# rapidsai/cugraph-gnn

Hardware: AMD Instinct MI355X
Metric: sampled-edges/sec (sample+renumber+feature-gather+SAGEConv fwd), ogbn-products-like fan-out [25, 10] (higher is better)
Workload: dtype int64 ids (int32 timed as a variant) + f32 features (SAGE lin_l/lin_r product: bf16x3-split MFMA, f32 accumulate); 1 GPU; ogbn-products-like RMAT: V=2449029, E=118462496 directed (CSR row_ptr i64 / col i64 replicated per GPU), feat fp32 [V,100], batch 1024/GPU, fan-out [25, 10], 2-layer SAGEConv(mean) 100-256-47 fwd, step = 8 call groups of 188 mini-batches; parallelism=dp1 (seeds sharded, no data-path collective)

## Files before the change

### cugraph-gnn_amd/csrc/wg_common.hpp

```cpp
#pragma once
#include <hip/hip_runtime.h>

#include <cstdarg>
#include <cstdint>
#include <cstdio>
#include <stdexcept>
#include <vector>
#include <mutex>
#include <string>
#include <unordered_map>

#include "wgamd_ops.h"
#include "wgamd_tensor.h"
#include "wgamd_types.h"

struct wholememory_tensor_ {
  void* storage_ptr;
  wholememory_tensor_description_t desc;
  wholememory_tensor_* root;
  wholememory_handle_t handle;
  bool owns_handle = false;
  uint64_t handle_serial = 0;
};

extern "C" uint64_t wgamd_handle_serial(wholememory_handle_t h);
extern "C" wholememory_error_code_t wgamd_free_if_serial(wholememory_handle_t h, uint64_t serial);

namespace wgamd {

struct hip_error : std::runtime_error {
  using std::runtime_error::runtime_error;
};
struct logic_error : std::runtime_error {
  using std::runtime_error::runtime_error;
};
struct invalid_input : std::runtime_error {
  using std::runtime_error::runtime_error;
};
struct comm_error : std::runtime_error {
  using std::runtime_error::runtime_error;
};

inline std::string fmt(const char* f, ...)
{
  char buf[1024];
  va_list ap;
  va_start(ap, f);
  vsnprintf(buf, sizeof(buf), f, ap);
  va_end(ap);
  return buf;
}

#define WG_HIP_CHECK(expr)                                                                   \
  do {                                                                                       \
    hipError_t e__ = (expr);                                                                 \
    if (e__ != hipSuccess) {                                                                 \
      throw ::wgamd::hip_error(::wgamd::fmt("%s:%d HIP error %d (%s) in %s", __FILE__,       \
                                            __LINE__, (int)e__, hipGetErrorString(e__), #expr)); \
    }                                                                                        \
  } while (0)

#define WG_EXPECTS(cond, ...)                                                              \
  do {                                                                                     \
    if (!(cond)) throw ::wgamd::logic_error(::wgamd::fmt(__VA_ARGS__));                    \
  } while (0)

#define WG_REQUIRE_INPUT(cond, ...)                                                        \
  do {                                                                                     \
    if (!(cond)) throw ::wgamd::invalid_input(::wgamd::fmt(__VA_ARGS__));                  \
  } while (0)

template <typename F>
inline wholememory_error_code_t guarded(const char* op, F&& body)
{
  try {
    body();
  } catch (const invalid_input& e) {
    fprintf(stderr, "[wholegraph_amd] %s: invalid input: %s\n", op, e.what());
    return WHOLEMEMORY_INVALID_INPUT;
  } catch (const logic_error& e) {
    fprintf(stderr, "[wholegraph_amd] %s: logic error: %s\n", op, e.what());
    return WHOLEMEMORY_LOGIC_ERROR;
  } catch (const hip_error& e) {
    fprintf(stderr, "[wholegraph_amd] %s: device error: %s\n", op, e.what());
    return WHOLEMEMORY_CUDA_ERROR;
  } catch (const comm_error& e) {
    fprintf(stderr, "[wholegraph_amd] %s: communication error: %s\n", op, e.what());
    return WHOLEMEMORY_COMMUNICATION_ERROR;
  } catch (const std::bad_alloc&) {
    fprintf(stderr, "[wholegraph_amd] %s: out of memory\n", op);
    return WHOLEMEMORY_OUT_OF_MEMORY;
  } catch (...) {
    fprintf(stderr, "[wholegraph_amd] %s: unknown error\n", op);
    return WHOLEMEMORY_UNKNOW_ERROR;
// ... 52 lines not shown
  wholememory_env_func_t* env_;
  void* ctx_ = nullptr;
  void* ptr_ = nullptr;
};

class temp_arena {
 public:
  explicit temp_arena(wholememory_env_func_t* env) : buf_(env) {}
  size_t add(size_t bytes)
  {
    const size_t off = total_;
    total_ += (bytes + 255) / 256 * 256;
    return off;
  }
  void commit() { base_ = static_cast<char*>(buf_.bytes((int64_t)(total_ ? total_ : 1))); }
  template <typename T>
  T* at(size_t off) const
  {
    return reinterpret_cast<T*>(base_ + off);
  }

 private:
  temp_buffer buf_;
  size_t total_ = 0;
  char* base_   = nullptr;
};

inline void* output_alloc(wholememory_env_func_t* env, void* memory_context, int64_t elt_count,
                          wholememory_dtype_t dtype)
{
  wholememory_tensor_description_t d;
  wholememory_initialize_tensor_desc(&d);
  d.dim        = 1;
  d.sizes[0]   = elt_count;
  d.strides[0] = 1;
  d.dtype      = dtype;
  void* p = env->output_fns.malloc_fn(&d, WHOLEMEMORY_MA_DEVICE, memory_context,
                                      env->output_fns.global_context);
  if (elt_count > 0 && p == nullptr) throw std::bad_alloc();
  return p;
}

inline int ceil_div(int64_t a, int64_t b) { return (int)((a + b - 1) / b); }

inline int stream_cu_count(hipStream_t stream)
{
  static std::mutex m;
  static std::unordered_map<int, int> device_cus;
  int dev = 0, cus = 0;
  (void)hipGetDevice(&dev);
  {
    std::lock_guard<std::mutex> g(m);
    auto it = device_cus.find(dev);
    if (it != device_cus.end()) cus = it->second;
  }
  if (cus == 0) {
    cus = 256;
    (void)hipDeviceGetAttribute(&cus, hipDeviceAttributeMultiprocessorCount, dev);
    std::lock_guard<std::mutex> g(m);
    device_cus[dev] = cus;
  }
  if (stream == nullptr) return cus;
  uint32_t mask[32] = {0};
  if (hipExtStreamGetCUMask(stream, 32, mask) != hipSuccess) {
    (void)hipGetLastError();
    return cus;
  }
  int bits = 0;
  for (uint32_t w : mask) bits += __builtin_popcount(w);
  return (bits > 0 && bits < cus) ? bits : cus;
}

struct dev_count {
  int host;
  const int* dev;
  __device__ __forceinline__ int get() const { return dev ? *dev : host; }
};

struct rng_plan {
  uint64_t seed;
  const unsigned long long* seeds_dev;
  const int* target_batch;
  const int* target_seg;
  __device__ __forceinline__ void resolve(int i, uint64_t& s, int& i_local) const
  {
    s       = seed;
    i_local = i;
    if (target_batch) {
      const int b = target_batch[i];
      i_local     = i - target_seg[b];
      s           = seeds_dev[b];
    } else if (seeds_dev) {
      s = seeds_dev[0];
    }
  }
};

int64_t scan_tmp_ints(int64_t n);
constexpr int kScanTile = 2048;
void exclusive_scan_i32(const int* in, int* out, int64_t n, int* tmp, hipStream_t stream,
                        const int* n_live_dev = nullptr);
void exclusive_scan_i32_presummed(const int* in, int* out, int64_t n, const int* sums, hipStream_t stream,
                                  const int* n_live_dev = nullptr);
struct scan_chain {
  unsigned long long* tiles;
  unsigned int* counters;
  unsigned int epoch;
};
constexpr int64_t kScanChainTiles = (int64_t)1 << 20;
scan_chain scan_chain_acquire(hipStream_t stream);


struct sample_locality {
  int* hist;
  void* recs;
  int shift;
};
int64_t sample_locality_hist_ints();
int sample_locality_shift(int64_t id_bound);
void uniform_sample_enqueue(const int64_t* row_ptr, const void* col, bool col64, const void* seeds, bool seeds64,
                            dev_count n, int M, rng_plan random_seed, const int* offsets, void* dst, int* src_lid,
                            int64_t* edge_gid, hipStream_t stream,
                            const int64_t* row_start = nullptr, const int* row_deg = nullptr,
                            const sample_locality* loc = nullptr);
void sample_count_enqueue(const int64_t* row_ptr, const void* seeds, bool seeds64, dev_count n, int M, int* cnt,
                          int* big_deg, hipStream_t stream, int64_t* row_start = nullptr, int* row_deg = nullptr);
constexpr int kWeightedBlocks  = 1024;
constexpr int kWeightedLdsKeys = 12288;
constexpr int kWeightedLists    = 9;
constexpr int kWeightedListHead = 16;
constexpr int kWeightedRedoList  = 9;
constexpr int kWeightedRedoCount = 11;
constexpr int kWeightedRedoHead  = 12;
inline int64_t weighted_list_ints(int64_t cap)
{
  return kWeightedListHead + (int64_t)(kWeightedLists + 1) * (cap > 0 ? cap : 1);
}
void weighted_count_enqueue(const int64_t* row_ptr, const void* seeds, bool seeds64, dev_count n, int M, int* cnt,
                            int* big_list, hipStream_t stream);
void weighted_sample_enqueue(const int64_t* row_ptr, const void* col, bool col64, const void* weights, bool weights64,
                             const void* seeds, bool seeds64, dev_count n, int M, rng_plan random_seed, const int* offsets,
                             int* big_list, uint32_t* slab, int64_t slab_len, void* dst, int* src_lid,
                             int64_t* edge_gid, hipStream_t stream);
int64_t append_unique_slots(int64_t capacity);
struct batch_view {
  const int* target_batch;
  const int* target_seg;
  const int* edge_row;
  const int* edge_offsets;
  int G;
  int64_t id_bound;
  int* unique_batch;
  int* unique_seg;
  const int* sample_batch;
  const int* sample_seg;
  const int* sample_local0;
  void* frontier_out;
  int* frontier_batch_out;
  int* frontier_seg_out;
  int* frontier_local0_out;
  int* neighbor_local_out;
  int* center_local_out;
  int no_pad;
  __host__ __device__ const int* sbatch() const { return sample_batch ? sample_batch : target_batch; }
  __host__ __device__ const int* sseg() const { return sample_seg ? sample_seg : target_seg; }
};
void append_unique_prepare_enqueue(const void* targets, dev_count T, bool tgt64, const void* neighbors, dev_count E, bool nbr64,
                                   batch_view bv, void* keys, int* minpos, int64_t slots, int* slot_of, int* rank,
                                   int* scan_tmp, hipStream_t stream);
void append_unique_emit_enqueue(const void* targets, dev_count T, bool tgt64, const void* neighbors, dev_count E, bool nbr64,
                                batch_view bv, const int* minpos, const int* slot_of, const int* rank, int64_t slots,
                                void* unique_out, int* map_out, int* counts_out ,
                                hipStream_t stream);


void local_rows_gather(const char* table, wholememory_matrix_description_t tm, const void* idx,
                       wholememory_dtype_t idx_dtype, int64_t n, char* out, wholememory_matrix_description_t om,
                       hipStream_t stream);
void local_rows_scatter(const char* in, wholememory_matrix_description_t im, const void* idx,
                        wholememory_dtype_t idx_dtype, int64_t n, char* table, wholememory_matrix_description_t tm,
                        hipStream_t stream);
void local_rows_permute(const char* src, wholememory_matrix_description_t sm, const int64_t* src_idx, const int64_t* dst_idx,
                        int64_t n, char* dst, wholememory_matrix_description_t dm, hipStream_t stream);
struct id_exchange {
  wholememory_comm_t comm = nullptr;
  int W = 1, me = 0;
  int64_t local_start = 0, local_rows = 0;
  std::vector<size_t> send_cnt, recv_cnt;
  std::vector<int64_t> bucket_start;
  std::vector<size_t> send_n, recv_n, send_at, recv_at;
  int64_t n = 0, n_remote = 0, self_cnt = 0, recv_total = 0;
  bool self_direct = false;
  int64_t *d_grouped = nullptr, *d_pos = nullptr, *d_recv_ids = nullptr, *d_self_ids = nullptr, *d_self_pos = nullptr;
  temp_arena scratch;
  std::vector<size_t> so, sb, ro, rb;

  explicit id_exchange(wholememory_env_func_t* env) : scratch(env) {}
  void plan(wholememory_handle_t h, size_t entry_bytes, int64_t row0, const void* idx, wholememory_dtype_t idx_dtype,
            int64_t n_, bool self_direct_, hipStream_t stream);
  void exchange_ids(int64_t* recv_ids, hipStream_t stream);
  void rows_to_owners(const char* send, char* recv, size_t row_bytes, hipStream_t stream);
  void rows_to_askers(const char* send, char* recv, size_t row_bytes, hipStream_t stream);

 private:
  void scaled(size_t unit_send, size_t unit_recv, const std::vector<size_t>& s_n, const std::vector<size_t>& s_at,
              const std::vector<size_t>& r_n, const std::vector<size_t>& r_at);
};

void distributed_rows_op(bool scatter, wholememory_handle_t handle, wholememory_matrix_description_t tm, const void* idx,
// ... 5 lines not shown
```

### cugraph-gnn_amd/csrc/wg_fused.hip

```cpp
#include <atomic>

#include "wg_common.hpp"
#include "wgamd_ext.h"

namespace wgamd {
namespace {

inline size_t align_up(size_t v) { return (v + 255) & ~(size_t)255; }

struct hop_workspace {
  size_t cnt, scan_tmp, nbr, keys, minpos, slot_of, rank, big_list, slab, row_start, row_deg, loc_hist, total;
  int64_t slots, slab_len;
};

hop_workspace plan(int64_t target_cap, int64_t edge_cap, size_t id_bytes, bool batched, int64_t max_row_len = 0)
{
  hop_workspace w{};
  size_t off = 0;
  auto take  = [&](size_t bytes) {
    size_t at = off;
    off += align_up(bytes);
    return at;
  };
  w.slots        = append_unique_slots(target_cap + edge_cap);
// ... 16 lines not shown
  w.total        = off;
  return w;
}

inline std::atomic<int64_t>& sample_locality_min()
{
  static std::atomic<int64_t> v{[] {
    const char* e = getenv("WGAMD_SAMPLE_LOCALITY");
    return e && atoll(e) > 0 ? (int64_t)atoll(e) : INT64_MAX;
  }()};
  return v;
}

struct hop_args {
  const void* csr_weight  = nullptr;
  bool weight64           = false;
  int64_t max_row_len     = 0;
  const void* sample_targets = nullptr;
  const int* n_sample_dev    = nullptr;
  int64_t sample_cap         = 0;
  const int64_t* csr_row_ptr;
  const void* csr_col;
  wholememory_dtype_t id_dtype;
  bool col32 = false;
  const void* targets;
  const int* n_targets_dev;
  int64_t target_cap;
  int M;
  rng_plan rng;
  batch_view bv;
  int* offsets;
  int* neighbor_row;
  int* center_row;
  int64_t* edge_gid;
  int64_t edge_cap;
  void* unique;
  int* counts_dev;
  void* workspace;
  size_t workspace_bytes;
  hipStream_t stream;
};

void run_hop(hop_args a)
{
  WG_REQUIRE_INPUT(a.id_dtype == WHOLEMEMORY_DT_INT || a.id_dtype == WHOLEMEMORY_DT_INT64, "id dtype must be INT|INT64");
  WG_REQUIRE_INPUT(a.csr_row_ptr && a.csr_col && a.targets && a.n_targets_dev && a.offsets && a.neighbor_row &&
                     a.unique && a.workspace,
                   "null pointer");
  WG_REQUIRE_INPUT(a.M > 0, "the no-sync walk needs a positive fan-out (capacity = targets * M)");
  const void* s_targets = a.sample_targets ? a.sample_targets : a.targets;
  const int* s_n_dev    = a.sample_targets ? a.n_sample_dev : a.n_targets_dev;
  const int64_t s_cap   = a.sample_targets ? a.sample_cap : a.target_cap;
  WG_REQUIRE_INPUT(a.target_cap > 0 && s_cap > 0 && a.edge_cap >= s_cap * (int64_t)a.M, "edge_cap < sampled_cap * M");
  WG_REQUIRE_INPUT(a.target_cap + a.edge_cap < ((int64_t)1 << 30), "capacities too large for one call");
  const bool i64     = a.id_dtype == WHOLEMEMORY_DT_INT64;
  const bool col64   = i64 && !a.col32;
  const bool batched = a.bv.target_batch != nullptr;
  WG_REQUIRE_INPUT(a.csr_weight == nullptr || a.max_row_len > 0, "a biased hop needs max_row_len (the graph's maximum degree)");
  hop_workspace w    = plan(std::max(a.target_cap, s_cap), a.edge_cap, i64 ? 8 : 4, batched, a.csr_weight ? a.max_row_len : 0);
  WG_REQUIRE_INPUT(a.workspace_bytes >= w.total, "workspace too small: need %zu bytes", w.total);
  WG_REQUIRE_INPUT((reinterpret_cast<uintptr_t>(a.workspace) & 255) == 0, "workspace must be 256-byte aligned");
  char* base    = static_cast<char*>(a.workspace);
  int* cnt      = reinterpret_cast<int*>(base + w.cnt);
  int* scan_tmp = reinterpret_cast<int*>(base + w.scan_tmp);
  void* nbr     = base + w.nbr;
  void* keys    = base + w.keys;
  int* minpos   = reinterpret_cast<int*>(base + w.minpos);
  int* slot_of  = reinterpret_cast<int*>(base + w.slot_of);
  int* rank     = reinterpret_cast<int*>(base + w.rank);
  hipStream_t st = a.stream;

  dev_count T{(int)a.target_cap, a.n_targets_dev};
  dev_count S{(int)s_cap, s_n_dev};
  if (a.csr_weight != nullptr) {
    int* big_list = reinterpret_cast<int*>(base + w.big_list);
    weighted_count_enqueue(a.csr_row_ptr, s_targets, i64, S, a.M, cnt, big_list, st);
    exclusive_scan_i32(cnt, a.offsets, s_cap, scan_tmp, st, s_n_dev);
    weighted_sample_enqueue(a.csr_row_ptr, a.csr_col, col64, a.csr_weight, a.weight64, s_targets, i64, S, a.M, a.rng, a.offsets,
                            big_list, reinterpret_cast<uint32_t*>(base + w.slab), w.slab_len, nbr, a.center_row, a.edge_gid,
                            st);
  } else {
    int64_t* row_start = reinterpret_cast<int64_t*>(base + w.row_start);
    int* row_deg       = reinterpret_cast<int*>(base + w.row_deg);
    sample_count_enqueue(a.csr_row_ptr, s_targets, i64, S, a.M, cnt, nullptr, st, row_start, row_deg);
    exclusive_scan_i32(cnt, a.offsets, s_cap, scan_tmp, st, s_n_dev);
    const int64_t loc_min = sample_locality_min().load(std::memory_order_relaxed);
    sample_locality loc{reinterpret_cast<int*>(base + w.loc_hist), keys, sample_locality_shift(a.bv.id_bound)};
    const bool use_loc = a.M <= 32 && s_cap >= loc_min && a.bv.id_bound > 0 && batched && 8 * w.slots >= 32 * s_cap;
    uniform_sample_enqueue(a.csr_row_ptr, a.csr_col, col64, s_targets, i64, S, a.M, a.rng, a.offsets, nbr, a.center_row,
                           a.edge_gid, st, row_start, row_deg, use_loc ? &loc : nullptr);
  }
  dev_count E{(int)a.edge_cap, a.offsets + s_cap};
  batch_view bv   = a.bv;
  bv.edge_row     = a.center_row;
  bv.edge_offsets = a.offsets;
  append_unique_prepare_enqueue(a.targets, T, i64, nbr, E, col64, bv, keys, minpos, w.slots, slot_of, rank, scan_tmp, st);
  append_unique_emit_enqueue(a.targets, T, i64, nbr, E, col64, bv, minpos, slot_of, rank, w.slots, a.unique, a.neighbor_row,
                             a.counts_dev, st);
}

__global__ void __launch_bounds__(256)
target_rows_kernel(const int* __restrict__ unique_seg, const int* __restrict__ target_seg, const int* __restrict__ target_batch,
                   int n, int64_t* __restrict__ rows)
{
  const int i = blockIdx.x * blockDim.x + threadIdx.x;
  if (i >= n) return;
  const int b = target_batch[i];
  rows[i]     = (int64_t)i + unique_seg[b] - target_seg[b];
}

__global__ void __launch_bounds__(256)
hetero_hop_rows_kernel(const int* __restrict__ offsets, const int* __restrict__ f_batch, const int* __restrict__ f_seg,
                       const int* __restrict__ f_local0, const int* __restrict__ row_local, int n_f,
                       const int* __restrict__ seg_dst, const int64_t* __restrict__ cseg_dst, const int* __restrict__ seg_src,
                       const int64_t* __restrict__ cseg_src, int64_t* __restrict__ dst_full, int64_t* __restrict__ dst_compact,
                       int* __restrict__ col_full, int* __restrict__ col_compact)
{
  const int64_t tid = (int64_t)blockIdx.x * blockDim.x + threadIdx.x;
  const int64_t j   = tid >> 4;
  const int sub     = (int)(tid & 15);
  if (j >= n_f) return;
  const int b     = f_batch[j];
  const int local = f_local0[b] + ((int)j - f_seg[b]);
  if (sub == 0) {
    dst_full[j] = (int64_t)seg_dst[b] + local;
    if (dst_compact) dst_compact[j] = cseg_dst[b] + local;
  }
  const int s = offsets[j], e = offsets[j + 1];
  const int add_full = seg_src[b];
  const int add_c    = col_compact ? (int)cseg_src[b] : 0;
  for (int i = s + sub; i < e; i += 16) {
    const int r = row_local[i];
    col_full[i] = r + add_full;
    if (col_compact) col_compact[i] = r + add_c;
  }
}

__global__ void __launch_bounds__(256)
hetero_hop_rows_batched_kernel(const int* __restrict__ offsets, const int* __restrict__ f_seg, const int* __restrict__ f_local0,
                               const int* __restrict__ row_local, int chunks, const int* __restrict__ seg_dst,
                               const int64_t* __restrict__ cseg_dst, const int* __restrict__ seg_src,
                               const int64_t* __restrict__ cseg_src, int64_t* __restrict__ dst_full,
                               int64_t* __restrict__ dst_compact, int* __restrict__ col_full, int* __restrict__ col_compact)
{
  const int b = blockIdx.x / chunks, c = blockIdx.x % chunks, t = threadIdx.x;
  const int f0 = f_seg[b], f1 = f_seg[b + 1];
  const int j0 = f0 + (int)((int64_t)(f1 - f0) * c / chunks), j1 = f0 + (int)((int64_t)(f1 - f0) * (c + 1) / chunks);
  if (j0 >= j1) return;
  const int e0 = offsets[j0], e1 = offsets[j1];
  const int64_t d_full = (int64_t)seg_dst[b] + f_local0[b] - f0;
  const int64_t d_c    = dst_compact ? cseg_dst[b] + f_local0[b] - f0 : 0;
  const int add_full   = seg_src[b];
  const int add_c      = col_compact ? (int)cseg_src[b] : 0;
  for (int j = j0 + t; j < j1; j += 256) {
    dst_full[j] = d_full + j;
    if (dst_compact) dst_compact[j] = d_c + j;
  }
  for (int i = e0 + t; i < e1; i += 256) {
    const int r = row_local[i];
    col_full[i] = r + add_full;
    if (col_compact) col_compact[i] = r + add_c;
  }
}

constexpr int kLayerSegMax = 16;
__global__ void __launch_bounds__(256)
layer_cols_kernel(const int* __restrict__ offsets, const int* __restrict__ f_seg, const int* __restrict__ f_local0,
                  const int* __restrict__ row_local, int G, int chunks, int n_seg, const int* __restrict__ seg_tab,
                  const int64_t* __restrict__ seg_base, int64_t* __restrict__ self_rows, int* __restrict__ col)
{
  __shared__ int s_l0[kLayerSegMax];
  __shared__ int64_t s_add[kLayerSegMax];
  const int b = blockIdx.x / chunks, c = blockIdx.x % chunks;
// ... 425 lines not shown
```

### cugraph-gnn_amd/csrc/wg_rng.hpp

```cpp
#pragma once
#include <hip/hip_runtime.h>

#include <cstdint>

namespace wgamd {

struct PcgJump {
  uint64_t a;
  uint64_t s;
};

struct PcgJumpTables {
  PcgJump t[4][256];
  constexpr PcgJumpTables() : t{}
  {
    uint64_t base_a = 6364136223846793005ULL, base_s = 1;
    for (int k = 0; k < 4; k++) {
      t[k][0].a = 1;
      t[k][0].s = 0;
      for (int c = 1; c < 256; c++) {
        t[k][c].a = t[k][c - 1].a * base_a;
        t[k][c].s = t[k][c - 1].s * base_a + base_s;
      }
      for (int d = 0; d < 8; d++) {
        uint64_t na = base_a * base_a, ns = base_s * base_a + base_s;
        base_a = na;
        base_s = ns;
      }
    }
  }
};

__device__ __constant__ const PcgJumpTables g_pcg_jump{};

struct Pcg32 {
  uint64_t state;
  uint64_t inc;

  static constexpr uint64_t kMult = 6364136223846793005ULL;

  __host__ __device__ __forceinline__ uint32_t next_u32()
  {
    uint64_t old = state;
    state        = old * kMult + inc;
    uint32_t x   = (uint32_t)(((old >> 18u) ^ old) >> 27u);
    uint32_t rot = (uint32_t)(old >> 59u);
    return (x >> rot) | (x << ((0u - rot) & 31u));
  }

  __host__ __device__ __forceinline__ void skipahead(uint64_t delta)
  {
    uint64_t acc_mult = 1u, acc_plus = 0u, cur_mult = kMult, cur_plus = inc;
    while (delta) {
      if (delta & 1u) {
        acc_mult *= cur_mult;
        acc_plus = acc_plus * cur_mult + cur_plus;
      }
      cur_plus = (cur_mult + 1u) * cur_plus;
      cur_mult *= cur_mult;
      delta >>= 1u;
    }
    state = acc_mult * state + acc_plus;
  }

  __host__ __device__ __forceinline__ Pcg32(uint64_t seed, uint64_t subsequence)
  {
    state = 0u;
    inc   = (subsequence << 1u) | 1u;
    (void)next_u32();
    state += seed;
    (void)next_u32();
    skipahead(subsequence);
  }

  __device__ __forceinline__ void jump_table(uint32_t n)
  {
    PcgJump j = g_pcg_jump.t[0][n & 255u];
#pragma unroll
    for (int k = 1; k < 4; k++) {
      const uint32_t c = (n >> (8 * k)) & 255u;
      if (c) {
        const PcgJump m = g_pcg_jump.t[k][c];
        j.s             = j.s * m.a + m.s;
        j.a             = j.a * m.a;
      }
    }
    state = j.a * state + inc * j.s;
  }

  struct table_tag {};
  __device__ __forceinline__ Pcg32(uint64_t seed, uint32_t subsequence, table_tag, uint32_t extra_draws = 0)
  {
    inc   = ((uint64_t)subsequence << 1u) | 1u;
    state = (inc + seed) * kMult + inc;
    jump_table(subsequence + extra_draws);
  }

  __host__ __device__ __forceinline__ int32_t next_i31() { return (int32_t)(next_u32() & 0x7fffffffu); }
  __host__ __device__ __forceinline__ uint64_t next_u64()
  {
    uint64_t lo = next_u32();
    uint64_t hi = next_u32();
    return lo | (hi << 32u);
  }
  __host__ __device__ __forceinline__ int64_t next_i63() { return (int64_t)(next_u64() & 0x7fffffffffffffffULL); }
  __host__ __device__ __forceinline__ float next_f32() { return (float)(next_u32() >> 8u) / 16777216.0f; }
};

}
```

### cugraph-gnn_amd/csrc/wg_sample.hip

```cpp
#include <algorithm>
#include <cmath>

#include "wg_common.hpp"
#include "wg_rng.hpp"

namespace wgamd {
namespace {

template <typename T>
struct dtype_of;
template <>
struct dtype_of<int32_t> {
  static constexpr wholememory_dtype_t value = WHOLEMEMORY_DT_INT;
};
template <>
struct dtype_of<int64_t> {
  static constexpr wholememory_dtype_t value = WHOLEMEMORY_DT_INT64;
};

__host__ __device__ constexpr int ref_block_threads(int M)
{
  int f = (M - 1) / 32;
  return f < 3 ? 32 : f < 6 ? 64 : f < 12 ? 128 : 256;
}
__host__ __device__ constexpr int ref_items_per_thread(int M)
{
  constexpr int t[32] = {1, 2, 3, 2, 3, 3, 2, 2, 3, 3, 3, 3, 2, 2, 2, 2,
                         3, 3, 3, 3, 3, 3, 3, 3, 4, 4, 4, 4, 4, 4, 4, 4};
  return t[(M - 1) / 32];
}

__device__ __forceinline__ uint64_t stream_id(int64_t seed_index, int B, int lane)
{
  return (uint64_t)(int64_t)(int32_t)(seed_index * B + lane);
}

__device__ __forceinline__ Pcg32 stream_generator(uint64_t random_seed, int64_t seed_index, int B, int lane)
{
  const int64_t sid = seed_index * B + lane;
  if (sid < (1ll << 31)) return Pcg32(random_seed, (uint32_t)sid, Pcg32::table_tag{});
  return Pcg32(random_seed, stream_id(seed_index, B, lane));
}

constexpr int kWaveRowCapDecl = 1024;
constexpr int kHugeRow = 16384;

template <typename SeedT>
__global__ void __launch_bounds__(256) sample_count_kernel(const int64_t* __restrict__ row_ptr,
                                                           const SeedT* __restrict__ seeds,
                                                           dev_count n_,
                                                           int M,
                                                           int* __restrict__ cnt,
                                                           int* __restrict__ big_deg ,
                                                           int* __restrict__ lists = nullptr ,
                                                           int list_cap            = 0,
                                                           int scratch_threshold   = 0,
                                                           int64_t* __restrict__ row_start = nullptr,
                                                           int* __restrict__ row_deg       = nullptr)
{
  const int n_live = n_.get();
  if (lists == nullptr) {
    const int end = min(n_.host, (n_live / kScanTile + 1) * kScanTile);
    for (int i = blockIdx.x * blockDim.x + threadIdx.x; i < end; i += gridDim.x * blockDim.x) {
      int deg = 0;
      if (i < n_live) {
        const int64_t nid   = (int64_t)seeds[i];
        const int64_t first = row_ptr[nid];
        deg                 = (int)(row_ptr[nid + 1] - first);
        if (row_start) {
          row_start[i] = first;
          row_deg[i]   = deg;
        }
        deg = (M > 0 && deg > M) ? M : deg;
      }
      cnt[i] = deg;
      if (big_deg) big_deg[i] = 0;
    }
    return;
  }
  int i = blockIdx.x * blockDim.x + threadIdx.x;
  int cls          = -1;
  int deg          = 0;
  if (i < n_.host) {
    if (i >= n_live) {
      if (i < (n_live / kScanTile + 1) * kScanTile) {
        cnt[i] = 0;
        if (big_deg) big_deg[i] = 0;
      }
    } else {
      int64_t nid         = (int64_t)seeds[i];
      const int64_t first = row_ptr[nid];
      deg                 = (int)(row_ptr[nid + 1] - first);
      cnt[i]              = (M > 0 && deg > M) ? M : deg;
      if (row_start) {
        row_start[i] = first;
        row_deg[i]   = deg;
      }
      if (big_deg) big_deg[i] = 0;
      if (lists != nullptr && M > 0 && deg > M) {
        cls = deg <= 16 ? 0 : deg <= 32 ? 1 : deg <= 64 ? 2 : deg <= 128 ? 3 : deg <= 256 ? 4 : deg <= 512 ? 5
              : deg <= kWaveRowCapDecl ? 6 : deg <= kHugeRow ? 7 : 8;
        if (cls >= 7 && deg > scratch_threshold) atomicMax(lists + 10, deg);
      }
    }
  }
  if (lists == nullptr) return;
  __shared__ int blk_cnt[kWeightedLists], blk_base[kWeightedLists];
  if (threadIdx.x < kWeightedLists) blk_cnt[threadIdx.x] = 0;
  __syncthreads();
  const int lane = threadIdx.x & 63;
  int my_rank    = 0;
#pragma unroll
  for (int c = 0; c < kWeightedLists; c++) {
    const uint64_t m = __ballot(cls == c);
    if (m == 0ull) continue;
    const int leader = __ffsll((long long)m) - 1;
    int base         = 0;
    if (lane == leader) base = atomicAdd(&blk_cnt[c], __popcll(m));
    base = __shfl(base, leader, 64);
    if (cls == c) my_rank = base + __popcll(m & ((1ull << lane) - 1ull));
  }
  __syncthreads();
  if (threadIdx.x < kWeightedLists && blk_cnt[threadIdx.x] > 0) blk_base[threadIdx.x] = atomicAdd(lists + threadIdx.x, blk_cnt[threadIdx.x]);
  __syncthreads();
  if (cls >= 0) lists[kWeightedListHead + (int64_t)cls * list_cap + blk_base[cls] + my_rank] = i;
}

template <typename ColT>
__device__ __forceinline__ ColT col_at(const ColT* __restrict__ col, int64_t at)
{
  return col ? col[at] : (ColT)0;
}

constexpr int kWalkGrid = 256 * 16;

template <typename ColT>
__device__ __forceinline__ void emit(ColT* dst, int* src_lid, int64_t* edge_gid, int64_t out, ColT v,
                                     int seed_index, int64_t gid)
{
  if (dst) dst[out] = v;
  if (src_lid) src_lid[out] = seed_index;
  if (edge_gid) edge_gid[out] = gid;
}

struct loc_rec {
  int64_t start;
  int i;
  int deg;
  int base;
  int i_local;
  int batch;
  int pad;
};
static_assert(sizeof(loc_rec) == 32, "one 32-byte sector per record");
// ... 32 lines not shown
  for (int b = 0; b < kLocBlocks; b++) {
    const int4 v = h4[(int64_t)b * (kLocBuckets / 4) + threadIdx.x];
    tot[0] += v.x; tot[1] += v.y; tot[2] += v.z; tot[3] += v.w;
    if (b < (int)blockIdx.x) { before[0] += v.x; before[1] += v.y; before[2] += v.z; before[3] += v.w; }
  }
  const int sum = tot[0] + tot[1] + tot[2] + tot[3];
  int inc = sum;
  const int lane = threadIdx.x & 63, wave = threadIdx.x >> 6;
#pragma unroll
  for (int d = 1; d < 64; d <<= 1) {
    const int up = __shfl_up(inc, d, 64);
    if (lane >= d) inc += up;
  }
  if (lane == 63) wave_tot[wave] = inc;
  __syncthreads();
  int run = inc - sum;
  for (int w = 0; w < wave; w++) run += wave_tot[w];
#pragma unroll
  for (int k = 0; k < 4; k++) {
    cursor[4 * threadIdx.x + k] = run + before[k];
    run += tot[k];
  }
  __syncthreads();
  for (int i = lo + threadIdx.x; i < hi; i += kLocThreads) {
    const int j = atomicAdd(&cursor[min((int)((uint64_t)seeds[i] >> shift), kLocBuckets - 1)], 1);
    loc_rec r;
    r.start = row_start[i];
    r.i     = i;
    r.deg   = row_deg[i];
    r.base  = offsets[i];
    r.i_local = i;
    r.batch   = 0;
    if (rng.target_batch) {
      r.batch   = rng.target_batch[i];
      r.i_local = i - rng.target_seg[r.batch];
    }
    r.pad   = 0;
    recs[j] = r;
  }
}

template <typename SeedT, typename ColT, int LANES>
__global__ void __launch_bounds__(256) sample_uniform_halfwave_kernel(const int64_t* __restrict__ row_ptr,
                                                                      const ColT* __restrict__ col,
                                                                      const SeedT* __restrict__ seeds,
                                                                      dev_count n_,
                                                                      int M,
                                                                      rng_plan rng,
                                                                      const int* __restrict__ offsets,
                                                                      ColT* __restrict__ dst,
                                                                      int* __restrict__ src_lid,
                                                                      int64_t* __restrict__ edge_gid,
                                                                      const int64_t* __restrict__ row_start,
                                                                      const int* __restrict__ row_deg,
                                                                      const loc_rec* __restrict__ recs = nullptr)
{
  const int n    = n_.get();
  const int lane = threadIdx.x & 63;
  const int hl   = lane & (LANES - 1);
  const int hb   = lane & ~(LANES - 1);
  int i          = (int)(((int64_t)blockIdx.x * blockDim.x + threadIdx.x) / LANES);
  loc_rec rec{};
  if (recs) {
    constexpr int kGroups = 256 / LANES;
    const int per_x = ((n + 7) / 8 + kGroups - 1) / kGroups * kGroups;
    const int k     = (int)(blockIdx.x >> 3) * kGroups + (int)threadIdx.x / LANES;
    const int j     = (int)(blockIdx.x & 7) * per_x + k;
    i               = n;
    if (k < per_x && j < n) {
      rec = recs[j];
      i   = rec.i;
    }
  }
  int32_t r_draw = 0;
  if (i < n && hl < M) {
    uint64_t random_seed;
    int i_local;
    if (recs) {
      i_local     = rec.i_local;
      random_seed = rng.seeds_dev ? rng.seeds_dev[rec.batch] : rng.seed;
    } else
      rng.resolve(i, random_seed, i_local);
    if (i_local < (1 << 26)) {
      Pcg32 g(random_seed, (uint32_t)(i_local * 32 + hl), Pcg32::table_tag{});
      r_draw = g.next_i31();
    } else {
      Pcg32 g(random_seed, stream_id(i_local, 32, hl));
      r_draw = g.next_i31();
    }
  }
  int64_t start = 0;
  int N = 0, base = 0;
  if (i < n && recs) {
    start = rec.start;
    N     = rec.deg;
    base  = rec.base;
  } else if (i < n) {
    if (row_start) {
      start = row_start[i];
      N     = row_deg[i];
    } else {
      int64_t nid = (int64_t)seeds[i];
      start       = row_ptr[nid];
      N           = (int)(row_ptr[nid + 1] - start);
    }
    base = offsets[i];
  }
  const bool pick = N > M;
  if (__ballot(pick) == 0ull) {
    if (hl < N) emit<ColT>(dst, src_lid, edge_gid, (int64_t)base + hl, col_at<ColT>(col, start + hl), i, start + hl);
    return;
  }
  int r = 0;
  if (pick && hl < M) r = r_draw % (N - hl);
  const int tail = N - hl - 1;
  int p1 = -1, p2 = -1;
  for (int s = 0; s + 1 < M; s++) {
    const int rs    = __shfl(r, hb | s, 64);
    const bool prev = s < hl;
    p1 = (prev && rs == r) ? s : p1;
    p2 = (prev && rs == tail) ? s : p2;
  }
  int root = p2 >= 0 ? p2 : hl;
#pragma unroll
  for (int round = 0; round < (LANES == 32 ? 5 : 4); round++) root = __shfl(root, hb | root, 64);
  const int val = N - root - 1;
  const int vp1 = __shfl(val, hb | (p1 & (LANES - 1)), 64);
  const int a   = p1 >= 0 ? vp1 : r;
  if (pick) {
    if (hl < M) emit<ColT>(dst, src_lid, edge_gid, (int64_t)base + hl, col_at<ColT>(col, start + a), i, start + a);
  } else if (hl < N) {
    emit<ColT>(dst, src_lid, edge_gid, (int64_t)base + hl, col_at<ColT>(col, start + hl), i, start + hl);
  }
}

template <typename SeedT, typename ColT, int GW, int K, bool EXACT>
__global__ void __launch_bounds__(256)
sample_uniform_multi_kernel(const ColT* __restrict__ col, dev_count n_, int M_rt, rng_plan rng, const int* __restrict__ offsets,
                            ColT* __restrict__ dst, int* __restrict__ src_lid, int64_t* __restrict__ edge_gid,
                            const int64_t* __restrict__ row_start, const int* __restrict__ row_deg,
                            const loc_rec* __restrict__ recs)
{
  constexpr int kGPW    = 64 / GW;
  constexpr int kGroups = 4 * kGPW;
  constexpr int kRounds = GW <= 2 ? 1 : GW <= 4 ? 2 : GW <= 8 ? 3 : GW <= 16 ? 4 : 5;
  const int M    = EXACT ? GW : M_rt;
  const int n    = n_.get();
  const int lane = threadIdx.x & 63;
  const int grp  = lane / GW;
  const int hl   = lane - grp * GW;
  const int hb   = grp * GW;
  const bool live_group = grp < kGPW;
  const int wg_group    = (int)(threadIdx.x >> 6) * kGPW + grp;
  const int per_x = ((n + 7) / 8 + kGroups * K - 1) / (kGroups * K) * (kGroups * K);
  const int64_t n_chunks = recs ? (int64_t)(per_x / (kGroups * K)) * 8 : ((int64_t)n + kGroups * K - 1) / (kGroups * K);
  for (int64_t chunk = blockIdx.x; chunk < n_chunks; chunk += gridDim.x) {
  int i[K], N[K], base[K], i_local[K], batch[K];
  int64_t start[K];
  if (recs) {
    const int k0    = ((int)(chunk >> 3) * kGroups + wg_group) * K;
#pragma unroll
    for (int k = 0; k < K; k++) {
      const int j = (int)(chunk & 7) * per_x + k0 + k;
      i[k] = n, N[k] = 0, base[k] = 0, start[k] = 0, i_local[k] = 0, batch[k] = 0;
      if (live_group && k0 + k < per_x && j < n) {
        const loc_rec r = recs[j];
        i[k] = r.i, N[k] = r.deg, base[k] = r.base, start[k] = r.start, i_local[k] = r.i_local, batch[k] = r.batch;
      }
    }
  } else {
    const int64_t g = chunk * kGroups + wg_group;
#pragma unroll
    for (int k = 0; k < K; k++) {
      i[k] = live_group ? (int)min(g * K + k, (int64_t)n) : n;
      N[k] = 0, base[k] = 0, start[k] = 0, i_local[k] = i[k], batch[k] = 0;
      if (i[k] < n) {
        start[k] = row_start[i[k]];
        N[k]     = row_deg[i[k]];
        base[k]  = offsets[i[k]];
        if (rng.target_batch) batch[k] = rng.target_batch[i[k]];
      }
    }
    if (rng.target_batch) {
#pragma unroll
      for (int k = 0; k < K; k++)
        if (i[k] < n) i_local[k] = i[k] - rng.target_seg[batch[k]];
    }
  }
  int32_t r_draw[K];
#pragma unroll
  for (int k = 0; k < K; k++) {
    r_draw[k] = 0;
    if (i[k] < n && hl < M) {
      const uint64_t random_seed = rng.seeds_dev ? rng.seeds_dev[rng.target_batch ? batch[k] : 0] : rng.seed;
      if (i_local[k] < (1 << 26)) {
        Pcg32 g(random_seed, (uint32_t)(i_local[k] * 32 + hl), Pcg32::table_tag{});
        r_draw[k] = g.next_i31();
      } else {
        Pcg32 g(random_seed, stream_id(i_local[k], 32, hl));
        r_draw[k] = g.next_i31();
      }
    }
  }
  int a[K];
#pragma unroll
  for (int k = 0; k < K; k++) {
    const bool pick = N[k] > M;
    a[k]            = hl;
    if (__ballot(pick) != 0ull) {
      int r = 0;
      if (pick && hl < M) r = r_draw[k] % (N[k] - hl);
      const int tail = N[k] - hl - 1;
      int p1 = -1, p2 = -1;
      auto step = [&](int s) {
        const int rs    = __shfl(r, hb + s, 64);
        const bool prev = s < hl;
        p1 = (prev && rs == r) ? s : p1;
        p2 = (prev && rs == tail) ? s : p2;
      };
      if constexpr (EXACT) {
#pragma unroll
        for (int s = 0; s + 1 < GW; s++) step(s);
      } else {
        for (int s = 0; s + 1 < M; s++) step(s);
      }
      int root = p2 >= 0 ? p2 : hl;
#pragma unroll
      for (int round = 0; round < kRounds; round++) root = __shfl(root, hb + root, 64);
      const int val = N[k] - root - 1;
      const int vp1 = __shfl(val, hb + max(p1, 0), 64);
      if (pick) a[k] = p1 >= 0 ? vp1 : r;
    }
  }
  ColT v[K];
  bool on[K];
#pragma unroll
  for (int k = 0; k < K; k++) {
    on[k] = live_group && hl < (N[k] > M ? M : N[k]);
    v[k]  = on[k] ? col_at<ColT>(col, start[k] + a[k]) : (ColT)0;
  }
#pragma unroll
  for (int k = 0; k < K; k++)
    if (on[k]) emit<ColT>(dst, src_lid, edge_gid, (int64_t)base[k] + hl, v[k], i[k], start[k] + a[k]);
  }
}

constexpr int kHashSlots = 4096;

__device__ __forceinline__ int lds_hash_find(const int* keys, int pos)
{
  uint32_t h = ((uint32_t)pos * 2654435761u) & (kHashSlots - 1);
  while (true) {
    int k = keys[h];
    if (k == pos || k == -1) return (int)h;
    h = (h + 1) & (kHashSlots - 1);
  }
}

template <typename SeedT, typename ColT>
__global__ void __launch_bounds__(256) sample_uniform_block_kernel(const int64_t* __restrict__ row_ptr,
                                                                   const ColT* __restrict__ col,
                                                                   const SeedT* __restrict__ seeds,
                                                                   dev_count n_,
                                                                   int M,
                                                                   int B,
                                                                   int items,
                                                                   rng_plan rng,
                                                                   const int* __restrict__ offsets,
                                                                   ColT* __restrict__ dst,
                                                                   int* __restrict__ src_lid,
                                                                   int64_t* __restrict__ edge_gid)
{
  __shared__ int r[1024];
  __shared__ int a[1024];
  __shared__ int hkeys[kHashSlots];
  __shared__ int hvals[kHashSlots];
  const int i = blockIdx.x;
  if (i >= n_.get()) return;
  const int64_t nid   = (int64_t)seeds[i];
// ... 106 lines not shown
constexpr int kWaveRowCap = 1024;
static_assert(kWaveRowCap == kWaveRowCapDecl, "keep the two in step");

__device__ __forceinline__ uint32_t key_bits(float k)
{
  uint32_t b = __float_as_uint(k);
  return (b & 0x80000000u) ? ~b : (b | 0x80000000u);
}

constexpr int kLdsKeys = kWeightedLdsKeys;

template <typename SeedT, typename ColT, typename WeightT, int B, int T>
__global__ void __launch_bounds__(T) sample_weighted_kernel(const int64_t* __restrict__ row_ptr,
                                                            const ColT* __restrict__ col,
                                                            const WeightT* __restrict__ weight,
                                                            const SeedT* __restrict__ seeds,
                                                            dev_count n_,
                                                            int M,
                                                            rng_plan rng,
                                                            const int* __restrict__ offsets,
                                                            uint32_t* __restrict__ slab,
                                                            int64_t slab_len,
                                                            ColT* __restrict__ dst,
                                                            int* __restrict__ src_lid,
                                                            int64_t* __restrict__ edge_gid,
                                                            int* __restrict__ lists ,
                                                            int list_cap,
                                                            int redo = 0 )
{
  static_assert(T % B == 0 && T % 64 == 0, "threads must be a multiple of the stream layout and of the wave");
  __shared__ uint32_t lds_keys[kLdsKeys];
  __shared__ int hist[256];
  __shared__ int sh_digit, sh_need, sh_redo;
  __shared__ int wave_cnt[2][T / 64];
  __shared__ int sh_li;
  const int n_live  = n_.get();
  const int n_huge  = lists && !redo ? lists[8] : 0;
  const int count   = lists ? (redo ? lists[kWeightedRedoCount] : n_huge + lists[7]) : n_live;
  uint32_t* gkeys   = slab + (int64_t)blockIdx.x * slab_len;
  int li            = blockIdx.x;
  while (true) {
  __syncthreads();
  if (lists) {
    if (threadIdx.x == 0) sh_li = atomicAdd(lists + (redo ? kWeightedRedoHead : 9), 1);
    __syncthreads();
    li = sh_li;
  }
  if (li >= count) break;
  const int i = lists ? (redo ? lists[kWeightedListHead + (int64_t)kWeightedRedoList * list_cap + li]
                         : li < n_huge ? lists[kWeightedListHead + 8 * (int64_t)list_cap + li]
                                       : lists[kWeightedListHead + 7 * (int64_t)list_cap + (li - n_huge)])
                      : li;
  if (!lists) li += gridDim.x;
  if (i >= n_live) continue;
  uint64_t random_seed;
  int i_rng;
  rng.resolve(i, random_seed, i_rng);
  const int64_t nid   = (int64_t)seeds[i];
  const int64_t start = row_ptr[nid];
  const int N         = (int)(row_ptr[nid + 1] - start);
  if (N <= 0) continue;
  const int64_t base = offsets[i];
  if (M <= 0 || N <= M) {
    for (int j = threadIdx.x; j < N; j += T)
      emit<ColT>(dst, src_lid, edge_gid, base + j, col_at<ColT>(col, start + j), i, start + j);
    continue;
  }
  const bool in_lds = N <= kLdsKeys;
  auto put = [&](int id, uint32_t k) { if (in_lds) lds_keys[id] = k; else gkeys[id] = k; };
  auto get = [&](int id) -> uint32_t {
    return in_lds ? lds_keys[id] : __hip_atomic_load(gkeys + id, __ATOMIC_RELAXED, __HIP_MEMORY_SCOPE_AGENT);
  };
  if (threadIdx.x == 0) sh_redo = 0;
  __syncthreads();
  {
    constexpr int hop = T / B;
    const int lane = threadIdx.x % B, part = threadIdx.x / B;
    const int L     = lane < N ? (N - lane + B - 1) / B : 0;
    const int share = (L + hop - 1) / hop;
    const int m0 = part * share, m1 = min(L, m0 + share);
    bool redrawn = false;
    if (m0 < m1) {
      const int64_t sid = (int64_t)i_rng * B + lane;
      Pcg32 g = (sid < (1ll << 31)) ? Pcg32(random_seed, (uint32_t)sid, Pcg32::table_tag{}, 3u * (uint32_t)m0)
                                    : Pcg32(random_seed, stream_id(i_rng, B, lane));
      if (sid >= (1ll << 31)) g.skipahead(3u * (uint64_t)m0);
      for (int m = m0; m < m1; m++) {
        const int id = lane + m * B;
        put(id, key_bits(ares_key((float)weight[start + id], g, &redrawn)));
      }
    }
    if (redrawn) sh_redo = 1;
  }
  __syncthreads();
  if (T > B && sh_redo) {
    if (threadIdx.x < B) {
      Pcg32 g = stream_generator(random_seed, i_rng, B, threadIdx.x);
      for (int id = threadIdx.x; id < N; id += B) put(id, key_bits(ares_key((float)weight[start + id], g)));
    }
    __syncthreads();
  }
  uint32_t prefix = 0, prefix_mask = 0;
  int need = M;
  for (int shift = 24; shift >= 0; shift -= 8) {
    for (int h = threadIdx.x; h < 256; h += T) hist[h] = 0;
    __syncthreads();
    for (int id = threadIdx.x; id < N; id += T) {
      uint32_t k = get(id);
      if ((k & prefix_mask) == prefix) atomicAdd(&hist[(k >> shift) & 255], 1);
    }
    __syncthreads();
    if (threadIdx.x < 64) {
      const int l  = threadIdx.x;
      const int h0 = hist[4 * l], h1 = hist[4 * l + 1], h2 = hist[4 * l + 2], h3 = hist[4 * l + 3];
      const int own = h0 + h1 + h2 + h3;
      int inc = own;
      for (int off = 1; off < 64; off <<= 1) {
        int v = __shfl_down(inc, off);
        if (l + off < 64) inc += v;
      }
      int acc = inc - own;
      if (acc < need && need <= inc) {
        int d = 4 * l + 3;
        if (acc + h3 < need) {
          acc += h3;
          d = 4 * l + 2;
          if (acc + h2 < need) {
            acc += h2;
            d = 4 * l + 1;
            if (acc + h1 < need) {
              acc += h1;
              d = 4 * l;
            }
          }
        }
        sh_digit = d;
        sh_need  = need - acc;
      }
    }
    __syncthreads();
    prefix |= (uint32_t)sh_digit << shift;
    prefix_mask |= 255u << shift;
    need = sh_need;
    __syncthreads();
  }
  const uint32_t thr = prefix;
  int out_run = 0, tie_run = 0;
  const int lane = threadIdx.x & 63, wave = threadIdx.x >> 6;
  for (int chunk = 0; chunk < N; chunk += T) {
    int id     = chunk + threadIdx.x;
    uint32_t k = id < N ? get(id) : 0u;
    bool gt    = id < N && k > thr;
    bool eq    = id < N && k == thr;
    uint64_t meq = __ballot(eq);
    int eq_before_in_wave = __popcll(meq & ((1ull << lane) - 1ull));
    if (lane == 0) wave_cnt[1][wave] = __popcll(meq);
    __syncthreads();
    int eq_before = tie_run + eq_before_in_wave, eq_total = 0;
    for (int w = 0; w < T / 64; w++) {
      if (w < wave) eq_before += wave_cnt[1][w];
      eq_total += wave_cnt[1][w];
    }
    bool take      = gt || (eq && eq_before < need);
    uint64_t mtake = __ballot(take);
    int before_in_wave = __popcll(mtake & ((1ull << lane) - 1ull));
    if (lane == 0) wave_cnt[0][wave] = __popcll(mtake);
    __syncthreads();
    int before = out_run + before_in_wave, total = 0;
    for (int w = 0; w < T / 64; w++) {
      if (w < wave) before += wave_cnt[0][w];
      total += wave_cnt[0][w];
    }
    if (take) emit<ColT>(dst, src_lid, edge_gid, base + before, col_at<ColT>(col, start + id), i, start + id);
    out_run += total;
    tie_run += eq_total;
    __syncthreads();
  }
  }
}

template <typename SeedT, typename ColT, typename WeightT, int LANES>
__global__ void __launch_bounds__(256) sample_weighted_group_kernel(const int64_t* __restrict__ row_ptr,
                                                                    const ColT* __restrict__ col,
                                                                    const WeightT* __restrict__ weight,
                                                                    const SeedT* __restrict__ seeds,
                                                                    int M,
                                                                    rng_plan rng,
                                                                    const int* __restrict__ offsets,
                                                                    ColT* __restrict__ dst,
                                                                    int* __restrict__ src_lid,
                                                                    int64_t* __restrict__ edge_gid,
                                                                    const int* __restrict__ lists,
                                                                    int list_cap,
                                                                    int cls)
{
  const int lane = threadIdx.x & 63;
  const int hl = lane & (LANES - 1), hb = lane & ~(LANES - 1);
  const int64_t li  = (((int64_t)blockIdx.x * blockDim.x + threadIdx.x) / LANES);
  const bool active = li < (int64_t)lists[cls];
  if (__ballot(active) == 0ull) return;
  int i = 0, N = 0;
  int64_t start = 0, base = 0;
  uint32_t k = 0u;
  if (active) {
    i = lists[kWeightedListHead + (int64_t)cls * list_cap + li];
    uint64_t random_seed;
    int i_rng;
    rng.resolve(i, random_seed, i_rng);
    const int64_t nid = (int64_t)seeds[i];
    start             = row_ptr[nid];
    N                 = (int)(row_ptr[nid + 1] - start);
    base              = offsets[i];
    if (hl < N) {
      Pcg32 g = stream_generator(random_seed, i_rng, 128, hl);
      k       = key_bits(ares_key((float)weight[start + hl], g));
    }
  }
  const uint64_t gm = LANES == 64 ? ~0ull : (((1ull << LANES) - 1ull) << hb);
  uint32_t prefix = 0;
  int need        = M;
  for (int bit = 31; bit >= 0; bit--) {
    const uint32_t cand = prefix | (1u << bit);
    const uint32_t hi   = ~((1u << bit) - 1u);
    const int cnt       = __popcll(__ballot((k & hi) == cand) & gm);
    if (cnt >= need) prefix = cand; else need -= cnt;
  }
  const uint64_t below = ((1ull << lane) - 1ull) & gm;
  const bool eq        = active && hl < N && k == prefix;
  const uint64_t meq   = __ballot(eq) & gm;
  const bool take      = active && hl < N && (k > prefix || (eq && __popcll(meq & below) < need));
  const uint64_t mt    = __ballot(take) & gm;
  if (take) emit<ColT>(dst, src_lid, edge_gid, base + __popcll(mt & below), col_at<ColT>(col, start + hl), i, start + hl);
}

template <typename SeedT, typename ColT, typename WeightT, int KMAX>
__global__ void __launch_bounds__(256) sample_weighted_wave_kernel(const int64_t* __restrict__ row_ptr,
                                                                   const ColT* __restrict__ col,
                                                                   const WeightT* __restrict__ weight,
                                                                   const SeedT* __restrict__ seeds,
                                                                   int M,
                                                                   rng_plan rng,
                                                                   const int* __restrict__ offsets,
                                                                   ColT* __restrict__ dst,
                                                                   int* __restrict__ src_lid,
                                                                   int64_t* __restrict__ edge_gid,
                                                                   const int* __restrict__ lists,
                                                                   int list_cap,
                                                                   int cls)
{
  const int lane   = threadIdx.x & 63;
  const int64_t li = (int64_t)blockIdx.x * 4 + (threadIdx.x >> 6);
  if (li >= (int64_t)lists[cls]) return;
  const int i = lists[kWeightedListHead + (int64_t)cls * list_cap + li];
  uint64_t random_seed;
  int i_rng;
  rng.resolve(i, random_seed, i_rng);
  const int64_t nid   = (int64_t)seeds[i];
  const int64_t start = row_ptr[nid];
  const int N         = __builtin_amdgcn_readfirstlane((int)(row_ptr[nid + 1] - start));
  const int64_t base  = offsets[i];
  uint32_t k[KMAX];
  {
    Pcg32 ga = stream_generator(random_seed, i_rng, 128, lane);
    Pcg32 gb = stream_generator(random_seed, i_rng, 128, lane + 64);
#pragma unroll
    for (int s = 0; s < KMAX; s++) {
      const int id = (s >> 1) * 128 + (s & 1) * 64 + lane;
      k[s]         = 0u;
      if (s * 64 < N) {
        if (id < N) k[s] = key_bits(ares_key((float)weight[start + id], (s & 1) ? gb : ga));
      }
    }
  }
  uint32_t k_or = 0u, k_and = ~0u;
#pragma unroll
  for (int s = 0; s < KMAX; s++) {
    k_or |= k[s];
    k_and &= k[s] != 0u ? k[s] : ~0u;
  }
#pragma unroll
  for (int d = 32; d >= 1; d >>= 1) {
    k_or |= __shfl_xor(k_or, d, 64);
    k_and &= __shfl_xor(k_and, d, 64);
  }
  k_or  = __builtin_amdgcn_readfirstlane(k_or);
  k_and = __builtin_amdgcn_readfirstlane(k_and);
  const uint32_t differ = k_or ^ k_and;
  const int top         = differ ? 31 - __clz(differ) : -1;
  uint32_t hi     = top < 0 ? ~0u : top >= 31 ? 0u : ~((2u << top) - 1u);
  uint32_t prefix = k_and & hi;
  int need        = M;
  int match       = N;
#pragma unroll 1
  for (int bit = top; bit >= 0 && match != need; bit--) {
    const uint32_t cand = prefix | (1u << bit);
    hi |= 1u << bit;
    int cnt = 0;
#pragma unroll
    for (int s = 0; s < KMAX; s++) cnt += __popcll(__ballot((k[s] & hi) == cand));
    if (cnt >= need) {
      prefix = cand;
      match  = cnt;
    } else {
      need -= cnt;
      match -= cnt;
    }
  }
  const uint64_t below = (1ull << lane) - 1ull;
  int out_run = 0, tie_run = 0;
#pragma unroll
  for (int s = 0; s < KMAX; s++) {
    const int id       = (s >> 1) * 128 + (s & 1) * 64 + lane;
    const uint32_t kd  = k[s] & hi;
    const bool eq      = k[s] != 0u && kd == prefix;
    const uint64_t meq = __ballot(eq);
    const bool take    = (k[s] != 0u && kd > prefix) || (eq && tie_run + __popcll(meq & below) < need);
    const uint64_t mt  = __ballot(take);
    if (take) emit<ColT>(dst, src_lid, edge_gid, base + out_run + __popcll(mt & below), col_at<ColT>(col, start + id), i, start + id);
    out_run += __popcll(mt);
    tie_run += __popcll(meq);
    __builtin_amdgcn_sched_barrier(0);
  }
}

constexpr uint64_t kPcgA  = Pcg32::kMult;
constexpr uint64_t kPcgA2 = kPcgA * kPcgA;
constexpr uint64_t kPcgA3 = kPcgA2 * kPcgA;
constexpr float kMagScale = 1.4426950408889634f * (1.0f - 1.0f / 65536.0f);

__device__ __forceinline__ uint32_t pcg_output(uint64_t old)
{
  const uint32_t x   = (uint32_t)(((old >> 18u) ^ old) >> 27u);
  const uint32_t rot = (uint32_t)(old >> 59u);
  return (x >> rot) | (x << ((0u - rot) & 31u));
}

struct KeyStream {
  uint64_t s, c2, c3;
  __device__ __forceinline__ explicit KeyStream(const Pcg32& g)
    : s(g.state), c2(g.inc * (kPcgA + 1u)), c3(g.inc * (kPcgA2 + kPcgA + 1u))
  {
  }
  __device__ __forceinline__ float next_mag(bool& rare)
  {
    const uint64_t s0 = s;
    const uint64_t s2 = s0 * kPcgA2 + c2;
    s                 = s0 * kPcgA3 + c3;
    const uint32_t d1 = pcg_output(s0), d3 = pcg_output(s2);
    rare |= d3 == 0u;
    return ldexpf((float)((d1 >> 8u) + (1u << 24)), -25 - __clz((int)d3));
  }
};

__device__ __forceinline__ float ares_key_exact(float a, float w) { return (log1pf(-a) / logf(2.0f)) * (1.0f / w); }
__device__ __forceinline__ bool weight_is_odd(float w) { return ((__float_as_uint(w) >> 23u) - 27u) > 200u; }

__device__ __forceinline__ void redo_append(int* lists, int list_cap, int i)
{
  const int p = atomicAdd(lists + kWeightedRedoCount, 1);
  lists[kWeightedListHead + (int64_t)kWeightedRedoList * list_cap + p] = i;
}

__device__ __forceinline__ void lane_select(uint32_t kb, int n_keys, int M, uint32_t& prefix, uint32_t& hi, int& need)
{
  prefix    = 0u;
  hi        = 0u;
  need      = M;
  int match = n_keys;
#pragma unroll 1
  for (int bit = 31; bit >= 0 && match != need; bit--) {
    const uint32_t cand = prefix | (1u << bit);
    hi |= 1u << bit;
    const int cnt = __popcll(__ballot(kb != 0u && (kb & hi) == cand));
    if (cnt >= need) {
      prefix = cand;
      match  = cnt;
    } else {
      need -= cnt;
      match -= cnt;
    }
  }
}

template <typename SeedT, typename ColT, typename WeightT, int KMAX>
__global__ void __launch_bounds__(256) sample_weighted_wave_pruned_kernel(const int64_t* __restrict__ row_ptr,
                                                                          const ColT* __restrict__ col,
                                                                          const WeightT* __restrict__ weight,
                                                                          const SeedT* __restrict__ seeds,
                                                                          int M,
                                                                          rng_plan rng,
                                                                          const int* __restrict__ offsets,
                                                                          ColT* __restrict__ dst,
                                                                          int* __restrict__ src_lid,
                                                                          int64_t* __restrict__ edge_gid,
                                                                          int* __restrict__ lists,
                                                                          int list_cap,
                                                                          int cls,
                                                                          int force_redo)
{
  __shared__ int sh_id[4][64];
  __shared__ float sh_a[4][64];
  const int lane = threadIdx.x & 63, wv = threadIdx.x >> 6;
  const int64_t li = (int64_t)blockIdx.x * 4 + wv;
  if (li >= (int64_t)lists[cls]) return;
  const int i = lists[kWeightedListHead + (int64_t)cls * list_cap + li];
  uint64_t random_seed;
  int i_rng;
  rng.resolve(i, random_seed, i_rng);
  const int64_t nid   = (int64_t)seeds[i];
  const int64_t start = row_ptr[nid];
  const int N         = __builtin_amdgcn_readfirstlane((int)(row_ptr[nid + 1] - start));
  const int64_t base  = offsets[i];
  uint32_t k[KMAX];
  float av[KMAX];
  bool rare = force_redo != 0;
  {
    float wv[KMAX];
#pragma unroll
    for (int s = 0; s < KMAX; s++) wv[s] = (float)weight[start + min(s * 64 + lane, N - 1)];
    KeyStream ga(stream_generator(random_seed, i_rng, 128, lane));
    KeyStream gb(stream_generator(random_seed, i_rng, 128, lane + 64));
#pragma unroll
    for (int s = 0; s < KMAX; s++) {
      const int id = s * 64 + lane;
      k[s]         = ~0u;
      av[s]        = 0.f;
      if (s * 64 < N) {
        if (id < N) {
          const float w = wv[s];
          const float a = ((s & 1) ? gb : ga).next_mag(rare);
          rare |= weight_is_odd(w);
          av[s] = a;
          k[s]  = __float_as_uint(a * __builtin_amdgcn_rcpf(w) * kMagScale);
        }
      }
    }
  }
  if (__ballot(rare) != 0ull) {
    if (lane == 0) redo_append(lists, list_cap, i);
    return;
  }
  const uint64_t below = (1ull << lane) - 1ull;
  uint32_t k_or = 0u, k_and = ~0u;
#pragma unroll
  for (int s = 0; s < KMAX; s++) {
    k_or |= k[s] != ~0u ? k[s] : 0u;
    k_and &= k[s];
  }
#pragma unroll
  for (int d = 32; d >= 1; d >>= 1) {
    k_or |= __shfl_xor(k_or, d, 64);
    k_and &= __shfl_xor(k_and, d, 64);
  }
  k_or  = __builtin_amdgcn_readfirstlane(k_or);
  k_and = __builtin_amdgcn_readfirstlane(k_and);
  const uint32_t differ = k_or ^ k_and;
  const int top         = differ ? 31 - __clz(differ) : -1;
  uint32_t hi     = top < 0 ? ~0u : top >= 31 ? 0u : ~((2u << top) - 1u);
  uint32_t prefix = k_and & hi;
  int need = M, match = N, under = 0;
#pragma unroll 1
  for (int bit = top; bit >= 0 && match != need && under + match > 64; bit--) {
    hi |= 1u << bit;
    int cnt0 = 0;
#pragma unroll
    for (int s = 0; s < KMAX; s++) cnt0 += __popcll(__ballot((k[s] & hi) == prefix));
    if (cnt0 >= need) {
      match = cnt0;
    } else {
      need -= cnt0;
      under += cnt0;
      match -= cnt0;
      prefix |= 1u << bit;
    }
  }
  if (under + match > 64) {
    if (lane == 0) redo_append(lists, list_cap, i);
    return;
  }
  uint32_t bound = prefix | ~hi;
  uint32_t kb = 0u, sel_prefix = 0u, sel_hi = 0u;
  int cid = 0, sel_need = 0, n_sel = 0;
#pragma unroll 1
  for (int round = 0; round < 2; round++) {
    n_sel = 0;
#pragma unroll
    for (int s = 0; s < KMAX; s++) {
      const bool in    = k[s] <= bound && k[s] != ~0u;
      const uint64_t m = __ballot(in);
      if (in) {
        const int p  = n_sel + __popcll(m & below);
        sh_id[wv][p] = s * 64 + lane;
        sh_a[wv][p]  = av[s];
      }
      n_sel += __popcll(m);
    }
    asm volatile("s_waitcnt lgkmcnt(0)" ::: "memory");
    kb = 0u;
    if (lane < n_sel) {
      cid           = sh_id[wv][lane];
      const float a = sh_a[wv][lane];
      kb            = key_bits(ares_key_exact(a, (float)weight[start + cid]));
    }
    asm volatile("s_waitcnt lgkmcnt(0)" ::: "memory");
// ... 153 lines not shown
            }
            int acc = inc - own;
            if (acc < need && need <= inc) {
              int d = 4 * l + 3;
              if (acc + h3 < need) {
                acc += h3;
                d = 4 * l + 2;
                if (acc + h2 < need) {
                  acc += h2;
                  d = 4 * l + 1;
                  if (acc + h1 < need) {
                    acc += h1;
                    d = 4 * l;
                  }
                }
              }
              sh_digit = d;
              sh_need  = need - acc;
            }
          }
          __syncthreads();
          prefix |= (uint32_t)sh_digit << shift;
          hi |= 255u << shift;
          need = sh_need;
          __syncthreads();
        }
      }
      for (int e = tid; e < n; e += T) {
        const uint32_t kk = c_kb[e], kd = kk & hi;
        if (kk != 0u && kd > prefix) {
          const int p = atomicAdd(&sh_keep, 1);
          keep_id[p]  = c_id[e];
          keep_a[p]   = c_a[e];
          atomicMin(&sh_kmin, kk);
        } else if (kk != 0u && kd == prefix) {
          const int q = atomicAdd(&sh_eq, 1);
          if (q < kEqCap) {
            eq_id[q] = c_id[e];
            eq_a[q]  = c_a[e];
            atomicMin(&sh_kmin, kk);
          } else {
            sh_rare = 1;
          }
        }
      }
      __syncthreads();
      const int eqc = min(sh_eq, kEqCap);
      if (tid < eqc) {
        int rank = 0;
        for (int j = 0; j < eqc; j++) rank += eq_id[j] < eq_id[tid] ? 1 : 0;
        if (rank < need) {
          const int p = atomicAdd(&sh_keep, 1);
          keep_id[p]  = eq_id[tid];
          keep_a[p]   = eq_a[tid];
        }
      }
      __syncthreads();
      if (last) {
        if (tid < M && !sh_rare) {
          const int mine = keep_id[tid];
          int rank = 0;
          for (int j = 0; j < M; j++) rank += keep_id[j] < mine ? 1 : 0;
          emit<ColT>(dst, src_lid, edge_gid, base + rank, col_at<ColT>(col, start + mine), i, start + mine);
        }
      } else {
        if (tid < M) {
          c_id[tid] = keep_id[tid];
          c_a[tid]  = keep_a[tid];
        }
        if (tid == 0) {
          sh_count = M;
          sh_thr   = (~sh_kmin) & 0x7fffffffu;
        }
      }
      __syncthreads();
    };

    const int sl = tid % B, part = tid / B;
    const int L     = (N - sl + B - 1) / B;
    const int share = (L + 3) / 4;
    const int m0 = part * share, m1 = min(L, m0 + share);
    const int rounds = (((N + B - 1) / B) + 3) / 4;
    const int64_t sid = (int64_t)i_rng * B + sl;
    Pcg32 g0 = (sid < (1ll << 31)) ? Pcg32(random_seed, (uint32_t)sid, Pcg32::table_tag{}, 3u * (uint32_t)m0)
                                   : Pcg32(random_seed, stream_id(i_rng, B, sl));
    if (sid >= (1ll << 31)) g0.skipahead(3u * (uint64_t)m0);
    KeyStream g(g0);
    bool rare = false;
    auto next = [&](float w, float& a, uint32_t& k) {
      a = g.next_mag(rare);
      rare |= weight_is_odd(w);
      k = __float_as_uint(a * __builtin_amdgcn_rcpf(w) * kMagScale);
    };
    auto weight_of = [&](int m) { return (float)weight[start + sl + (int64_t)min(m, m1 - 1) * B]; };
    const bool has0 = m0 < m1;
    float a0    = 0.f;
    uint32_t k0 = ~0u;
    if (has0) next(weight_of(m0), a0, k0);
    {
      const int nvalid = __popcll(__ballot(has0));
      uint32_t v = 0x7f800000u;
      if (nvalid >= M) {
        uint32_t prefix = 0u, hi = 0u;
        int need = M, match = nvalid;
#pragma unroll 1
        for (int bit = 31; bit >= 0 && match != need; bit--) {
          hi |= 1u << bit;
          const int cnt0 = __popcll(__ballot(has0 && (k0 & hi) == prefix));
          if (cnt0 >= need) {
            match = cnt0;
          } else {
            need -= cnt0;
            match -= cnt0;
            prefix |= 1u << bit;
          }
        }
        v = prefix | ~hi;
      }
      if (lane == 0) sh_wthr[wave] = v;
    }
    __syncthreads();
    uint32_t thr0 = sh_wthr[0];
#pragma unroll
    for (int w = 1; w < W; w++) thr0 = min(thr0, sh_wthr[w]);
    if (has0 && k0 <= thr0) append(m0 * B + sl, a0);
    compress(false);
    uint32_t thr = sh_thr;
    if (has0 && k0 > thr0 && k0 <= thr) append(m0 * B + sl, a0);
    for (int r = 1; r < rounds;) {
      if (__syncthreads_or(sh_count > kCandCap / 2)) compress(false);
      thr = sh_thr;
      float wv[kChunkRounds];
#pragma unroll
      for (int c = 0; c < kChunkRounds; c++) wv[c] = weight_of(m0 + r + c);
#pragma unroll
      for (int c = 0; c < kChunkRounds; c++) {
        const int m = m0 + r + c;
        if (m < m1) {
          float a;
          uint32_t k;
          next(wv[c], a, k);
          if (k <= thr) append(m * B + sl, a);
        }
      }
      r += kChunkRounds;
    }
    if (rare) sh_rare = 1;
    compress(true);
    if (tid == 0 && sh_rare) redo_append(lists, list_cap, i);
  }
}

template <typename SeedT, typename ColT>
__global__ void __launch_bounds__(256) copy_short_rows_kernel(const int64_t* __restrict__ row_ptr, const ColT* __restrict__ col,
                                                              const SeedT* __restrict__ seeds, dev_count n_, int M,
                                                              const int* __restrict__ offsets, ColT* __restrict__ dst,
                                                              int* __restrict__ src_lid, int64_t* __restrict__ edge_gid)
{
  const int64_t t = (int64_t)blockIdx.x * blockDim.x + threadIdx.x;
  const int i = (int)(t >> 4), hl = (int)(t & 15);
  if (i >= n_.get()) return;
  const int64_t nid   = (int64_t)seeds[i];
  const int64_t start = row_ptr[nid];
  const int N         = (int)(row_ptr[nid + 1] - start);
  if (N <= 0 || N > M) return;
  const int64_t base = offsets[i];
  for (int j = hl; j < N; j += 16) emit<ColT>(dst, src_lid, edge_gid, base + j, col_at<ColT>(col, start + j), i, start + j);
}

template <typename SeedT, typename ColT>
void uniform_launch(const int64_t* row_ptr, const ColT* col, const SeedT* seeds, dev_count n, int M,
                    rng_plan random_seed, const int* offsets, ColT* dst, int* lid, int64_t* gid, hipStream_t stream,
                    const int64_t* row_start = nullptr, const int* row_deg = nullptr, const sample_locality* loc = nullptr)
{
  const int cap = n.host;
  if (cap <= 0) return;
  if (M > 0 && M <= 32 && row_start != nullptr) {
    static const int K = [] {
      const char* e = getenv("WGAMD_SAMPLE_K");
      const int k   = e ? atoi(e) : 4;
      return k == 1 || k == 2 ? k : 4;
    }();
    const loc_rec* recs = nullptr;
    if (loc != nullptr) {
      auto* r = static_cast<loc_rec*>(loc->recs);
      locality_hist_kernel<SeedT><<<kLocBlocks, kLocThreads, 0, stream>>>(seeds, n, loc->shift, loc->hist);
      locality_scatter_kernel<SeedT><<<kLocBlocks, kLocThreads, 0, stream>>>(seeds, n, loc->shift, loc->hist, row_start, row_deg,
                                                                            offsets, random_seed, r);
      recs = r;
    }
#define WG_MULTI(GW, KK)                                                                                             \
  sample_uniform_multi_kernel<SeedT, ColT, GW, KK, WG_EXACT>                                                          \
    <<<(int)std::min<int64_t>((ceil_div((int64_t)cap, 4 * (64 / GW) * KK) + 15) / 8 * 8, kWalkGrid), 256, 0, stream>>>(           \
      col, n, M, random_seed, offsets, dst, lid, gid, row_start, row_deg, recs)
#define WG_MULTI_K(GW)                                                                                               \
  do {                                                                                                               \
    if (K == 1) WG_MULTI(GW, 1); else if (K == 2) WG_MULTI(GW, 2); else WG_MULTI(GW, 4);                              \
  } while (0)
    static const bool exact = getenv("WGAMD_SAMPLE_EXACT_WIDTH") == nullptr || atoi(getenv("WGAMD_SAMPLE_EXACT_WIDTH")) != 0;
#define WG_EXACT true
    if (exact && M == 5) WG_MULTI_K(5);
    else if (exact && M == 10) WG_MULTI_K(10);
    else if (exact && M == 15) WG_MULTI_K(15);
    else if (exact && M == 25) WG_MULTI_K(25);
    else {
#undef WG_EXACT
#define WG_EXACT false
      if (M <= 8) WG_MULTI_K(8);
      else if (M <= 16) WG_MULTI_K(16);
      else WG_MULTI_K(32);
    }
#undef WG_EXACT
#undef WG_MULTI_K
#undef WG_MULTI
    WG_HIP_CHECK(hipGetLastError());
    return;
  }
  if (M <= 0) {
    sample_uniform_block_kernel<SeedT, ColT><<<cap, 64, 0, stream>>>(row_ptr, col, seeds, n, 0x7fffffff, 32, 1,
                                                                     random_seed, offsets, dst, lid, gid);
  } else if (M <= 16) {
    sample_uniform_halfwave_kernel<SeedT, ColT, 16><<<ceil_div((int64_t)cap * 16, 256), 256, 0, stream>>>(
      row_ptr, col, seeds, n, M, random_seed, offsets, dst, lid, gid, row_start, row_deg);
  } else if (M <= 32) {
    sample_uniform_halfwave_kernel<SeedT, ColT, 32><<<ceil_div((int64_t)cap * 32, 256), 256, 0, stream>>>(
      row_ptr, col, seeds, n, M, random_seed, offsets, dst, lid, gid, row_start, row_deg);
  } else if (M <= 1024) {
    const int B = ref_block_threads(M);
    sample_uniform_block_kernel<SeedT, ColT><<<cap, B < 64 ? 64 : B, 0, stream>>>(
      row_ptr, col, seeds, n, M, B, ref_items_per_thread(M), random_seed, offsets, dst, lid, gid);
  } else {
    sample_uniform_reservoir_kernel<SeedT, ColT><<<cap, 64, 0, stream>>>(row_ptr, col, seeds, n, M, random_seed,
                                                                         offsets, dst, lid, gid);
  }
  WG_HIP_CHECK(hipGetLastError());
}

inline int& weighted_mode(int which)
{
  static int mode[2] = {[] { const char* e = getenv("WGAMD_WEIGHTED_PRUNING"); return e && e[0] == '0' ? 0 : 1; }(),
                        [] { const char* e = getenv("WGAMD_WEIGHTED_FORCE_REDO"); return e && e[0] == '1' ? 1 : 0; }()};
  return mode[which];
}
inline bool weighted_pruning_off() { return weighted_mode(0) == 0; }
inline int weighted_force_redo() { return weighted_mode(1); }

struct side_stream {
  int device         = -1;
  hipStream_t stream = nullptr;
  hipEvent_t fork = nullptr, join = nullptr;
  void ensure()
  {
    int dev = 0;
    WG_HIP_CHECK(hipGetDevice(&dev));
    if (stream != nullptr && dev == device) return;
    device = dev;
    WG_HIP_CHECK(hipStreamCreateWithFlags(&stream, hipStreamNonBlocking));
    WG_HIP_CHECK(hipEventCreateWithFlags(&fork, hipEventDisableTiming));
    WG_HIP_CHECK(hipEventCreateWithFlags(&join, hipEventDisableTiming));
  }
};
inline side_stream& weighted_side_stream()
{
  static thread_local side_stream s;
  s.ensure();
  return s;
}

template <typename SeedT, typename ColT, typename WeightT>
void weighted_sample_launch(const int64_t* row_ptr, const ColT* col, const WeightT* weights, const SeedT* seeds, dev_count n,
                            int M, rng_plan rng, const int* offsets, int* lists, int blocks, uint32_t* slab,
                            int64_t slab_len, ColT* dst, int* lid, int64_t* gid, hipStream_t stream)
{
  if (n.host <= 0) return;
  const int cap = n.host;
  if (M <= 0 || M > 256) {
    sample_weighted_kernel<SeedT, ColT, WeightT, 256, 256><<<std::max(blocks, 1), 256, 0, stream>>>(
      row_ptr, col, weights, seeds, n, M, rng, offsets, slab, slab_len, dst, lid, gid, nullptr, 0);
    return;
  }
  const bool pruned = M <= 32 && !weighted_pruning_off();
  bool forked = false;
  side_stream* side = nullptr;
  if (blocks > 0 && pruned) {
    side = &weighted_side_stream();
    WG_HIP_CHECK(hipEventRecord(side->fork, stream));
    WG_HIP_CHECK(hipStreamWaitEvent(side->stream, side->fork, 0));
    sample_weighted_block_pruned_kernel<SeedT, ColT, WeightT><<<blocks, 512, 0, side->stream>>>(
      row_ptr, col, weights, seeds, n, M, rng, offsets, dst, lid, gid, lists, cap, weighted_force_redo());
    WG_HIP_CHECK(hipEventRecord(side->join, side->stream));
    forked = true;
  } else if (blocks > 0)
    sample_weighted_kernel<SeedT, ColT, WeightT, 128, 512><<<blocks, 512, 0, stream>>>(
      row_ptr, col, weights, seeds, n, M, rng, offsets, slab, slab_len, dst, lid, gid, lists, cap);
  if (M < 16)
    sample_weighted_group_kernel<SeedT, ColT, WeightT, 16><<<ceil_div((int64_t)cap * 16, 256), 256, 0, stream>>>(
      row_ptr, col, weights, seeds, M, rng, offsets, dst, lid, gid, lists, cap, 0);
  if (M < 32)
    sample_weighted_group_kernel<SeedT, ColT, WeightT, 32><<<ceil_div((int64_t)cap * 32, 256), 256, 0, stream>>>(
      row_ptr, col, weights, seeds, M, rng, offsets, dst, lid, gid, lists, cap, 1);
  if (M < 64)
    sample_weighted_group_kernel<SeedT, ColT, WeightT, 64><<<ceil_div((int64_t)cap * 64, 256), 256, 0, stream>>>(
      row_ptr, col, weights, seeds, M, rng, offsets, dst, lid, gid, lists, cap, 2);
#define WG_WAVE(KM, CLS)                                                                                               \
  do {                                                                                                                 \
    if (pruned)                                                                                                        \
      sample_weighted_wave_pruned_kernel<SeedT, ColT, WeightT, KM><<<ceil_div(cap, 4), 256, 0, stream>>>(              \
        row_ptr, col, weights, seeds, M, rng, offsets, dst, lid, gid, lists, cap, CLS, weighted_force_redo());          \
    else                                                                                                               \
      sample_weighted_wave_kernel<SeedT, ColT, WeightT, KM><<<ceil_div(cap, 4), 256, 0, stream>>>(                     \
        row_ptr, col, weights, seeds, M, rng, offsets, dst, lid, gid, lists, cap, CLS);                                \
  } while (0)
  if (M < 128) WG_WAVE(2, 3);
  WG_WAVE(4, 4);
  WG_WAVE(8, 5);
  WG_WAVE(16, 6);
#undef WG_WAVE
  copy_short_rows_kernel<SeedT, ColT><<<ceil_div((int64_t)cap * 16, 256), 256, 0, stream>>>(row_ptr, col, seeds, n, M, offsets,
                                                                                          dst, lid, gid);
  if (forked) WG_HIP_CHECK(hipStreamWaitEvent(stream, side->join, 0));
  if (pruned)
    sample_weighted_kernel<SeedT, ColT, WeightT, 128, 512><<<blocks > 0 ? std::min(blocks, 128) : 64, 512, 0, stream>>>(
      row_ptr, col, weights, seeds, n, M, rng, offsets, slab, slab_len, dst, lid, gid, lists, cap, 1);
}

struct sample_args {
  wholememory_tensor_t row_ptr, col, weight, seeds, out_offsets;
  int M;
  void *dst_ctx, *lid_ctx, *gid_ctx;
  uint64_t random_seed;
  wholememory_env_func_t* env;
  hipStream_t stream;
};

void validate(const sample_args& a, bool weighted)
{
  WG_REQUIRE_INPUT(a.row_ptr && a.col && a.seeds && a.out_offsets && a.env, "null tensor / env");
  WG_REQUIRE_INPUT(a.dst_ctx != nullptr, "output_dest_memory_context must not be NULL");
  auto rd = a.row_ptr->desc, cd = a.col->desc, sd = a.seeds->desc, od = a.out_offsets->desc;
  WG_REQUIRE_INPUT(rd.dim == 1 && cd.dim == 1 && sd.dim == 1 && od.dim == 1, "all tensors must be 1-D");
  WG_REQUIRE_INPUT(!weighted || (!a.row_ptr->handle && !a.col->handle),
                   "weighted sampling needs CSR tensors that wrap device pointers (a partitioned CSR is served for the "
                   "unweighted op only, as in the reference)");
  WG_EXPECTS(rd.dtype == WHOLEMEMORY_DT_INT64, "csr_row_ptr dtype must be INT64, got %d", (int)rd.dtype);
  WG_EXPECTS(od.dtype == WHOLEMEMORY_DT_INT, "output_sample_offset dtype must be INT, got %d", (int)od.dtype);
  WG_REQUIRE_INPUT(cd.dtype == WHOLEMEMORY_DT_INT || cd.dtype == WHOLEMEMORY_DT_INT64, "csr_col dtype must be INT|INT64");
  WG_REQUIRE_INPUT(sd.dtype == WHOLEMEMORY_DT_INT || sd.dtype == WHOLEMEMORY_DT_INT64, "center_nodes dtype must be INT|INT64");
  WG_REQUIRE_INPUT(od.sizes[0] == sd.sizes[0] + 1, "output_sample_offset must have center_node_count+1 entries");
  WG_REQUIRE_INPUT(sd.sizes[0] < (int64_t)1 << 31, "too many center nodes");
  if (weighted) {
    WG_REQUIRE_INPUT(a.weight && !a.weight->handle && a.weight->desc.dim == 1, "csr_weight must be a 1-D device tensor");
    WG_REQUIRE_INPUT(a.weight->desc.dtype == WHOLEMEMORY_DT_FLOAT || a.weight->desc.dtype == WHOLEMEMORY_DT_DOUBLE,
                     "csr_weight dtype must be FLOAT|DOUBLE");
    WG_REQUIRE_INPUT(a.weight->desc.sizes[0] == cd.sizes[0], "csr_weight and csr_col sizes differ");
  }
}

// ... 94 lines not shown
}

struct borrowed_tensor {
  wholememory_tensor_t t = nullptr;
  borrowed_tensor(void* p, int64_t n, wholememory_dtype_t dt)
  {
    wholememory_tensor_description_t d;
    wholememory_initialize_tensor_desc(&d);
    d.dim        = 1;
    d.dtype      = dt;
    d.sizes[0]   = n;
    d.strides[0] = 1;
    WG_EXPECTS(wholememory_make_tensor_from_pointer(&t, p, &d) == WHOLEMEMORY_SUCCESS, "tensor over scratch");
  }
  ~borrowed_tensor() { wholememory_destroy_tensor(t); }
  borrowed_tensor(const borrowed_tensor&)            = delete;
  borrowed_tensor& operator=(const borrowed_tensor&) = delete;
};

template <typename ColT>
void run_partitioned(const sample_args& a)
{
  const int n        = (int)a.seeds->desc.sizes[0];
  const int M        = a.M;
  hipStream_t stream = a.stream;
  const bool seeds64 = a.seeds->desc.dtype == WHOLEMEMORY_DT_INT64;
  int* offsets       = static_cast<int*>(tensor_data(a.out_offsets));
  auto fetch = [&](wholememory_tensor_t table, wholememory_tensor_t idx, wholememory_tensor_t out, const char* what) {
    const auto rc = wholememory_gather(table, idx, out, a.env, stream, -1);
    if (rc != WHOLEMEMORY_SUCCESS) throw logic_error(fmt("gather of %s failed (%d)", what, (int)rc));
  };
  temp_arena arena(a.env);
  const size_t o_ids = arena.add(sizeof(int64_t) * 2 * n), o_ptr = arena.add(sizeof(int64_t) * 2 * n),
               o_twice = arena.add(sizeof(int) * n), o_cnt = arena.add(sizeof(int) * (n + 1)),
               o_scan = arena.add(sizeof(int) * scan_tmp_ints(n + 1));
  arena.commit();
  int64_t* ids  = arena.at<int64_t>(o_ids);
  int64_t* ptrs = arena.at<int64_t>(o_ptr);
  int* twice    = arena.at<int>(o_twice);
  int* cnt      = arena.at<int>(o_cnt);
  if (n > 0) {
    centre_pairs_kernel<<<ceil_div(n, 256), 256, 0, stream>>>(tensor_data(a.seeds), seeds64, n, ids, twice);
    WG_HIP_CHECK(hipGetLastError());
  }
  {
    borrowed_tensor t_ids(ids, 2 * (int64_t)n, WHOLEMEMORY_DT_INT64), t_ptrs(ptrs, 2 * (int64_t)n, WHOLEMEMORY_DT_INT64);
    fetch(a.row_ptr, t_ids.t, t_ptrs.t, "csr_row_ptr");
  }
  sample_count_enqueue(ptrs, twice, false, dev_count{n, nullptr}, M, cnt, nullptr, stream);
  exclusive_scan_i32(cnt, offsets, n, arena.at<int>(o_scan), stream);
  int total = 0;
  WG_HIP_CHECK(hipMemcpyAsync(&total, offsets + n, sizeof(int), hipMemcpyDeviceToHost, stream));
  WG_HIP_CHECK(hipStreamSynchronize(stream));
  auto* dst = static_cast<ColT*>(output_alloc(a.env, a.dst_ctx, total, dtype_of<ColT>::value));
  int* lid  = a.lid_ctx ? static_cast<int*>(output_alloc(a.env, a.lid_ctx, total, WHOLEMEMORY_DT_INT)) : nullptr;
  temp_buffer gid_buf(a.env);
  auto* gid = a.gid_ctx ? static_cast<int64_t*>(output_alloc(a.env, a.gid_ctx, total, WHOLEMEMORY_DT_INT64))
                        : gid_buf.device<int64_t>(total, WHOLEMEMORY_DT_INT64);
  if (n > 0 && total > 0)
    uniform_sample_enqueue(ptrs, nullptr, sizeof(ColT) == 8, twice, false, dev_count{n, nullptr}, M,
                           rng_plan{a.random_seed, nullptr, nullptr, nullptr}, offsets, nullptr, lid, gid, stream);
  {
    borrowed_tensor t_gid(gid, total, WHOLEMEMORY_DT_INT64), t_dst(dst, total, dtype_of<ColT>::value);
    fetch(a.col, t_gid.t, t_dst.t, "csr_col");
  }
  WG_HIP_CHECK(hipStreamSynchronize(stream));
}

template <typename WeightT>
void dispatch(const sample_args& a, bool weighted)
{
  const bool s64 = a.seeds->desc.dtype == WHOLEMEMORY_DT_INT64;
  const bool c64 = a.col->desc.dtype == WHOLEMEMORY_DT_INT64;
  if (!weighted && (a.row_ptr->handle || a.col->handle)) return c64 ? run_partitioned<int64_t>(a) : run_partitioned<int32_t>(a);
  if (s64 && c64) return run<int64_t, int64_t, WeightT>(a, weighted);
  if (s64 && !c64) return run<int64_t, int32_t, WeightT>(a, weighted);
  if (!s64 && c64) return run<int32_t, int64_t, WeightT>(a, weighted);
  return run<int32_t, int32_t, WeightT>(a, weighted);
}

}

void sample_count_enqueue(const int64_t* row_ptr, const void* seeds, bool seeds64, dev_count n, int M, int* cnt,
                          int* big_deg, hipStream_t stream, int64_t* row_start, int* row_deg)
{
  if (n.host <= 0) return;
  if (seeds64)
    sample_count_kernel<int64_t><<<std::min(ceil_div(n.host, 256), kWalkGrid), 256, 0, stream>>>(
      row_ptr, static_cast<const int64_t*>(seeds), n, M, cnt, big_deg, nullptr, 0, 0, row_start, row_deg);
  else
    sample_count_kernel<int32_t><<<std::min(ceil_div(n.host, 256), kWalkGrid), 256, 0, stream>>>(
      row_ptr, static_cast<const int32_t*>(seeds), n, M, cnt, big_deg, nullptr, 0, 0, row_start, row_deg);
  WG_HIP_CHECK(hipGetLastError());
}

void weighted_count_enqueue(const int64_t* row_ptr, const void* seeds, bool seeds64, dev_count n, int M, int* cnt,
                            int* big_list, hipStream_t stream)
{
  if (n.host <= 0) return;
  WG_HIP_CHECK(hipMemsetAsync(big_list, 0, kWeightedListHead * sizeof(int), stream));
  if (seeds64)
    sample_count_kernel<int64_t><<<ceil_div(n.host, 256), 256, 0, stream>>>(row_ptr, static_cast<const int64_t*>(seeds), n, M,
                                                                           cnt, nullptr, big_list, n.host, kLdsKeys);
  else
    sample_count_kernel<int32_t><<<ceil_div(n.host, 256), 256, 0, stream>>>(row_ptr, static_cast<const int32_t*>(seeds), n, M,
                                                                           cnt, nullptr, big_list, n.host, kLdsKeys);
  WG_HIP_CHECK(hipGetLastError());
}

void weighted_sample_enqueue(const int64_t* row_ptr, const void* col, bool col64, const void* weights, bool weights64,
                             const void* seeds, bool seeds64, dev_count n, int M, rng_plan random_seed, const int* offsets,
                             int* big_list, uint32_t* slab, int64_t slab_len, void* dst, int* src_lid,
                             int64_t* edge_gid, hipStream_t stream)
{
  WG_REQUIRE_INPUT(M > 0 && M <= 256, "the no-sync biased hop needs 0 < fan-out <= 256");
#define WG_W(ST, CT, WT)                                                                                                  \
  weighted_sample_launch<ST, CT, WT>(row_ptr, static_cast<const CT*>(col), static_cast<const WT*>(weights),              \
                                     static_cast<const ST*>(seeds), n, M, random_seed, offsets, big_list, kWeightedBlocks, \
                                     slab, slab_len, static_cast<CT*>(dst), src_lid, edge_gid, stream)
#define WG_WW(ST, CT) do { if (weights64) WG_W(ST, CT, double); else WG_W(ST, CT, float); } while (0)
  if (seeds64 && col64) WG_WW(int64_t, int64_t);
  else if (seeds64) WG_WW(int64_t, int32_t);
  else if (col64) WG_WW(int32_t, int64_t);
  else WG_WW(int32_t, int32_t);
#undef WG_WW
#undef WG_W
  WG_HIP_CHECK(hipGetLastError());
}

int64_t sample_locality_hist_ints() { return (int64_t)kLocBlocks * kLocBuckets; }
int sample_locality_shift(int64_t id_bound)
{
  int bits = 0;
  while (bits < 62 && ((int64_t)1 << bits) < id_bound) bits++;
  int buckets_log2 = 0;
  while ((1 << buckets_log2) < kLocBuckets) buckets_log2++;
  return bits > buckets_log2 ? bits - buckets_log2 : 0;
}

void uniform_sample_enqueue(const int64_t* row_ptr, const void* col, bool col64, const void* seeds, bool seeds64,
                            dev_count n, int M, rng_plan random_seed, const int* offsets, void* dst, int* src_lid,
                            int64_t* edge_gid, hipStream_t stream, const int64_t* row_start,
                            const int* row_deg, const sample_locality* loc)
{
#define WG_U(ST, CT)                                                                                               \
  uniform_launch<ST, CT>(row_ptr, static_cast<const CT*>(col), static_cast<const ST*>(seeds), n, M, random_seed, \
                         offsets, static_cast<CT*>(dst), src_lid, edge_gid, stream, row_start, row_deg, loc)
  if (seeds64 && col64) WG_U(int64_t, int64_t);
  else if (seeds64) WG_U(int64_t, int32_t);
  else if (col64) WG_U(int32_t, int64_t);
  else WG_U(int32_t, int32_t);
#undef WG_U
}

}

extern "C" {

void wgamd_set_weighted_sampling_mode(int pruning, int force_redo)
{
  if (pruning >= 0) wgamd::weighted_mode(0) = pruning ? 1 : 0;
  if (force_redo >= 0) wgamd::weighted_mode(1) = force_redo ? 1 : 0;
}

wholememory_error_code_t wholegraph_csr_unweighted_sample_without_replacement(
  wholememory_tensor_t wm_csr_row_ptr_tensor, wholememory_tensor_t wm_csr_col_ptr_tensor,
  wholememory_tensor_t center_nodes_tensor, int max_sample_count,
  wholememory_tensor_t output_sample_offset_tensor, void* output_dest_memory_context,
  void* output_center_localid_memory_context, void* output_edge_gid_memory_context,
  unsigned long long random_seed, wholememory_env_func_t* p_env_fns, void* stream)
{
  return wgamd::guarded("wholegraph_csr_unweighted_sample_without_replacement", [&] {
    wgamd::sample_args a{wm_csr_row_ptr_tensor, wm_csr_col_ptr_tensor, nullptr, center_nodes_tensor,
                         output_sample_offset_tensor, max_sample_count, output_dest_memory_context,
                         output_center_localid_memory_context, output_edge_gid_memory_context,
                         (uint64_t)random_seed, p_env_fns, static_cast<hipStream_t>(stream)};
    wgamd::validate(a, false);
    wgamd::dispatch<float>(a, false);
  });
}

wholememory_error_code_t wholegraph_csr_weighted_sample_without_replacement(
  wholememory_tensor_t wm_csr_row_ptr_tensor, wholememory_tensor_t wm_csr_col_ptr_tensor,
  wholememory_tensor_t wm_csr_weight_ptr_tensor, wholememory_tensor_t center_nodes_tensor,
  int max_sample_count, wholememory_tensor_t output_sample_offset_tensor,
  void* output_dest_memory_context, void* output_center_localid_memory_context,
  void* output_edge_gid_memory_context, unsigned long long random_seed,
  wholememory_env_func_t* p_env_fns, void* stream)
{
  return wgamd::guarded("wholegraph_csr_weighted_sample_without_replacement", [&] {
    wgamd::sample_args a{wm_csr_row_ptr_tensor, wm_csr_col_ptr_tensor, wm_csr_weight_ptr_tensor,
                         center_nodes_tensor, output_sample_offset_tensor, max_sample_count,
                         output_dest_memory_context, output_center_localid_memory_context,
                         output_edge_gid_memory_context, (uint64_t)random_seed, p_env_fns,
                         static_cast<hipStream_t>(stream)};
    wgamd::validate(a, true);
    if (a.weight->desc.dtype == WHOLEMEMORY_DT_DOUBLE)
      wgamd::dispatch<double>(a, true);
    else
      wgamd::dispatch<float>(a, true);
  });
}

wholememory_error_code_t generate_random_positive_int_cpu(int64_t random_seed, int64_t subsequence,
                                                          wholememory_tensor_t output)
{
  if (output == nullptr || output->desc.dim != 1) {
    fprintf(stderr, "[wholegraph_amd] generate_random_positive_int_cpu: output should be 1D tensor.\n");
    return WHOLEMEMORY_INVALID_INPUT;
  }
  if (output->desc.dtype != WHOLEMEMORY_DT_INT && output->desc.dtype != WHOLEMEMORY_DT_INT64) {
    fprintf(stderr, "[wholegraph_amd] generate_random_positive_int_cpu: output should be int64 or int32 tensor.\n");
    return WHOLEMEMORY_INVALID_INPUT;
  }
  wgamd::Pcg32 g((uint64_t)random_seed, (uint64_t)subsequence);
  void* p = wgamd::tensor_data(output);
  for (int64_t k = 0; k < output->desc.sizes[0]; k++) {
    if (output->desc.dtype == WHOLEMEMORY_DT_INT)
      static_cast<int32_t*>(p)[k] = g.next_i31();
    else
      static_cast<int64_t*>(p)[k] = g.next_i63();
  }
  return WHOLEMEMORY_SUCCESS;
}

wholememory_error_code_t generate_exponential_distribution_negative_float_cpu(int64_t random_seed,
                                                                              int64_t subsequence,
                                                                              wholememory_tensor_t output)
{
  if (output == nullptr || output->desc.dim != 1) {
// ... 28 lines not shown
```

### cugraph-gnn_amd/csrc/wg_sample_replace.hip

```cpp
#include "wg_common.hpp"
#include "wg_rng.hpp"
#include "wgamd_ext.h"

namespace wgamd {
namespace {

template <typename SeedT>
__global__ void __launch_bounds__(256)
replace_count_kernel(const int64_t* __restrict__ row_ptr, const SeedT* __restrict__ seeds, int n, int M, int* __restrict__ cnt)
{
  const int i = blockIdx.x * blockDim.x + threadIdx.x;
  if (i >= n) return;
  const int64_t nid = (int64_t)seeds[i];
  cnt[i]            = row_ptr[nid + 1] > row_ptr[nid] ? M : 0;
}

template <typename SeedT, typename ColT>
__global__ void __launch_bounds__(256)
replace_sample_kernel(const int64_t* __restrict__ row_ptr, const ColT* __restrict__ col, const SeedT* __restrict__ seeds, int n,
                      int M, uint64_t random_seed, const int* __restrict__ offsets, ColT* __restrict__ dst,
                      int* __restrict__ src_lid, int64_t* __restrict__ edge_gid)
{
  const int64_t p = (int64_t)blockIdx.x * blockDim.x + threadIdx.x;
  if (p >= (int64_t)n * M) return;
  const int i = (int)(p / M), t = (int)(p - (int64_t)i * M);
  int32_t r;
  if (p < (1ll << 31)) {
    Pcg32 g(random_seed, (uint32_t)p, Pcg32::table_tag{});
    r = g.next_i31();
  } else {
    Pcg32 g(random_seed, (uint64_t)p);
    r = g.next_i31();
  }
  const int64_t nid   = (int64_t)seeds[i];
  const int64_t start = row_ptr[nid];
  const int64_t N     = row_ptr[nid + 1] - start;
  if (N <= 0) return;
  const int64_t a   = start + (int64_t)(r % N);
  const int64_t out = (int64_t)offsets[i] + t;
  dst[out]          = col[a];
  if (src_lid) src_lid[out] = i;
  if (edge_gid) edge_gid[out] = a;
}

template <typename SeedT, typename ColT>
void run(const int64_t* row_ptr, const void* col_, const void* seeds_, int n, int M, int* offsets, void* dst_ctx, void* lid_ctx,
         void* gid_ctx, uint64_t random_seed, wholememory_dtype_t col_dt, wholememory_env_func_t* env, hipStream_t stream)
{
  const auto* col   = static_cast<const ColT*>(col_);
  const auto* seeds = static_cast<const SeedT*>(seeds_);
  temp_buffer cnt_buf(env), scan_tmp(env);
  int* cnt  = cnt_buf.device<int>(n + 1, WHOLEMEMORY_DT_INT);
  int* stmp = scan_tmp.device<int>(scan_tmp_ints(n + 1), WHOLEMEMORY_DT_INT);
  if (n > 0) replace_count_kernel<SeedT><<<ceil_div(n, 256), 256, 0, stream>>>(row_ptr, seeds, n, M, cnt);
  WG_HIP_CHECK(hipGetLastError());
  exclusive_scan_i32(cnt, offsets, n, stmp, stream);
  int total = 0;
  WG_HIP_CHECK(hipMemcpyAsync(&total, offsets + n, sizeof(int), hipMemcpyDeviceToHost, stream));
  WG_HIP_CHECK(hipStreamSynchronize(stream));
  auto* dst = static_cast<ColT*>(output_alloc(env, dst_ctx, total, col_dt));
  int* lid  = lid_ctx ? static_cast<int*>(output_alloc(env, lid_ctx, total, WHOLEMEMORY_DT_INT)) : nullptr;
  auto* gid = gid_ctx ? static_cast<int64_t*>(output_alloc(env, gid_ctx, total, WHOLEMEMORY_DT_INT64)) : nullptr;
  if (n == 0 || total == 0) return;
  replace_sample_kernel<SeedT, ColT><<<ceil_div((int64_t)n * M, 256), 256, 0, stream>>>(row_ptr, col, seeds, n, M, random_seed,
                                                                                       offsets, dst, lid, gid);
  WG_HIP_CHECK(hipGetLastError());
  WG_HIP_CHECK(hipStreamSynchronize(stream));
}

}
}

extern "C" wholememory_error_code_t wgamd_csr_uniform_sample_with_replacement(
  wholememory_tensor_t wm_csr_row_ptr_tensor, wholememory_tensor_t wm_csr_col_ptr_tensor,
  wholememory_tensor_t center_nodes_tensor, int sample_count, wholememory_tensor_t output_sample_offset_tensor,
  void* output_dest_memory_context, void* output_center_localid_memory_context, void* output_edge_gid_memory_context,
  unsigned long long random_seed, wholememory_env_func_t* p_env_fns, void* stream)
{
  using namespace wgamd;
  return guarded("wgamd_csr_uniform_sample_with_replacement", [&] {
    WG_REQUIRE_INPUT(wm_csr_row_ptr_tensor && wm_csr_col_ptr_tensor && center_nodes_tensor && output_sample_offset_tensor &&
                       p_env_fns,
                     "null tensor / env");
    WG_REQUIRE_INPUT(output_dest_memory_context != nullptr, "output_dest_memory_context must not be NULL");
    WG_REQUIRE_INPUT(sample_count > 0, "sampling with replacement needs a positive sample count");
    auto rd = wm_csr_row_ptr_tensor->desc, cd = wm_csr_col_ptr_tensor->desc, sd = center_nodes_tensor->desc,
         od = output_sample_offset_tensor->desc;
    WG_REQUIRE_INPUT(rd.dim == 1 && cd.dim == 1 && sd.dim == 1 && od.dim == 1, "all tensors must be 1-D");
    WG_REQUIRE_INPUT(!wm_csr_row_ptr_tensor->handle && !wm_csr_col_ptr_tensor->handle, "CSR tensors must wrap device pointers");
    WG_EXPECTS(rd.dtype == WHOLEMEMORY_DT_INT64, "csr_row_ptr dtype must be INT64, got %d", (int)rd.dtype);
    WG_EXPECTS(od.dtype == WHOLEMEMORY_DT_INT, "output_sample_offset dtype must be INT, got %d", (int)od.dtype);
    WG_REQUIRE_INPUT(cd.dtype == WHOLEMEMORY_DT_INT || cd.dtype == WHOLEMEMORY_DT_INT64, "csr_col dtype must be INT|INT64");
    WG_REQUIRE_INPUT(sd.dtype == WHOLEMEMORY_DT_INT || sd.dtype == WHOLEMEMORY_DT_INT64, "center_nodes dtype must be INT|INT64");
    WG_REQUIRE_INPUT(od.sizes[0] == sd.sizes[0] + 1, "output_sample_offset must have center_node_count+1 entries");
    WG_REQUIRE_INPUT(sd.sizes[0] * (int64_t)sample_count < ((int64_t)1 << 31), "too many samples for one call");
    const int n       = (int)sd.sizes[0];
    const auto* rp    = static_cast<const int64_t*>(tensor_data(wm_csr_row_ptr_tensor));
    const void* col   = tensor_data(wm_csr_col_ptr_tensor);
    const void* seeds = tensor_data(center_nodes_tensor);
    int* offsets      = static_cast<int*>(tensor_data(output_sample_offset_tensor));
    auto st           = static_cast<hipStream_t>(stream);
    const bool s64 = sd.dtype == WHOLEMEMORY_DT_INT64, c64 = cd.dtype == WHOLEMEMORY_DT_INT64;
#define WG_GO(S, C)                                                                                                        \
  run<S, C>(rp, col, seeds, n, sample_count, offsets, output_dest_memory_context, output_center_localid_memory_context,    \
            output_edge_gid_memory_context, (uint64_t)random_seed, cd.dtype, p_env_fns, st)
    if (s64 && c64) WG_GO(int64_t, int64_t);
    else if (s64) WG_GO(int64_t, int32_t);
    else if (c64) WG_GO(int32_t, int64_t);
    else WG_GO(int32_t, int32_t);
#undef WG_GO
  });
}
```

### cugraph-gnn_amd/csrc/wg_unique.hip

```cpp
#include "wg_common.hpp"
#include "wgamd_ext.h"

namespace wgamd {
namespace {

template <typename IdT>
__global__ void __launch_bounds__(256) unique_mark_kernel(const IdT* __restrict__ ids, int64_t n, int64_t bound, uint8_t* __restrict__ flags,
                                                          int* __restrict__ bad, const int* __restrict__ n_live)
{
  if (n_live) n = min(n, (int64_t)*n_live);
  const int64_t T = (int64_t)gridDim.x * blockDim.x;
  for (int64_t i = (int64_t)blockIdx.x * blockDim.x + threadIdx.x; i < n; i += 4 * T) {
    int64_t id[4];
    uint8_t f[4];
#pragma unroll
    for (int k = 0; k < 4; k++) id[k] = i + k * T < n ? (int64_t)ids[i + k * T] : -1;
#pragma unroll
    for (int k = 0; k < 4; k++) {
      if (id[k] >= bound) {
        *bad  = 1;
        id[k] = -1;
      }
      f[k] = id[k] >= 0 ? flags[id[k]] : 1;
    }
#pragma unroll
    for (int k = 0; k < 4; k++)
      if (f[k] == 0) flags[id[k]] = 1;
  }
}

__global__ void __launch_bounds__(256) unique_pack_kernel(const uint8_t* __restrict__ flags, int64_t n_words, uint2* __restrict__ rank,
                                                          int* __restrict__ cnt, int64_t cnt_padded)
{
  const int64_t w = (int64_t)blockIdx.x * blockDim.x + threadIdx.x;
  if (w < n_words) {
    const uint4* p = reinterpret_cast<const uint4*>(flags + w * 32);
    const uint4 a = p[0], b = p[1];
    const uint32_t v[8] = {a.x, a.y, a.z, a.w, b.x, b.y, b.z, b.w};
    uint32_t word = 0;
#pragma unroll
    for (int k = 0; k < 8; k++) {
      const uint32_t x = v[k];
      word |= ((x & 1u) | ((x >> 7) & 2u) | ((x >> 14) & 4u) | ((x >> 21) & 8u)) << (4 * k);
    }
    rank[w].x = word;
    cnt[w]    = __popc(word);
  } else if (w < cnt_padded) {
    cnt[w] = 0;
  }
}

__global__ void __launch_bounds__(256) unique_compact_kernel(uint2* __restrict__ rank, const int* __restrict__ prefix, int64_t n_words,
                                                             int64_t* __restrict__ distinct, int* __restrict__ n_distinct)
{
  const int64_t w = (int64_t)blockIdx.x * blockDim.x + threadIdx.x;
  if (w == 0 && n_distinct) *n_distinct = prefix[n_words];
  if (w >= n_words) return;
  uint32_t word = rank[w].x;
  int at        = prefix[w];
  rank[w].y     = (uint32_t)at;
  while (word) {
    const int k    = __ffs(word) - 1;
    distinct[at++] = w * 32 + k;
    word &= word - 1;
  }
}

template <typename IdT>
__global__ void __launch_bounds__(256) unique_inverse_kernel(const IdT* __restrict__ ids, int64_t n, int64_t bound, const uint2* __restrict__ rank,
                                                             int* __restrict__ inverse,
                                                             const int* __restrict__ n_live)
{
  if (n_live) n = min(n, (int64_t)*n_live);
  const int64_t T = (int64_t)gridDim.x * blockDim.x;
  for (int64_t i = (int64_t)blockIdx.x * blockDim.x + threadIdx.x; i < n; i += 4 * T) {
    int64_t id[4];
    uint2 r[4];
#pragma unroll
    for (int k = 0; k < 4; k++) id[k] = i + k * T < n ? (int64_t)ids[i + k * T] : -1;
#pragma unroll
    for (int k = 0; k < 4; k++) {
      const bool ok = id[k] >= 0 && id[k] < bound;
      r[k]          = ok ? rank[id[k] >> 5] : make_uint2(0u, 0xffffffffu);
    }
#pragma unroll
    for (int k = 0; k < 4; k++)
      if (i + k * T < n) inverse[i + k * T] = (int)r[k].y + __popc(r[k].x & ((1u << (id[k] & 31)) - 1u));
  }
}

struct unique_plan {
  size_t flags, bits, cnt, tmp, bad, total;
  int64_t n_words, cnt_padded;
};
unique_plan plan_unique(int64_t bound)
{
  unique_plan p{};
  size_t at = 0;
  auto add  = [&](size_t bytes) {
    const size_t o = at;
    at += (bytes + 255) / 256 * 256;
    return o;
  };
  p.n_words    = (bound + 31) / 32;
  p.cnt_padded = (p.n_words + kScanTile) / kScanTile * kScanTile;
  p.flags = add((size_t)p.n_words * 32);
  p.bits  = add(sizeof(uint2) * (size_t)p.n_words);
  p.cnt   = add(sizeof(int) * (size_t)(p.cnt_padded + 1));
  p.tmp   = add(sizeof(int) * (size_t)scan_tmp_ints(p.n_words));
  p.bad   = add(sizeof(int));
  p.total = at;
  return p;
}

}
}

extern "C" {

size_t wgamd_unique_bounded_workspace_bytes(int64_t id_bound)
{
  if (id_bound <= 0 || id_bound >= ((int64_t)1 << 31) - 4096) return 0;
  return wgamd::plan_unique(id_bound).total;
}

wholememory_error_code_t wgamd_unique_bounded(const void* ids, wholememory_dtype_t id_dtype, int64_t n, int64_t id_bound,
                                              int64_t* distinct, int* inverse, int* n_distinct_dev, int* out_of_bound_dev,
                                              void* workspace, size_t workspace_bytes, void* stream)
{
  return wgamd_unique_bounded_live(ids, id_dtype, n, nullptr, id_bound, distinct, inverse, n_distinct_dev, out_of_bound_dev,
                                   workspace, workspace_bytes, stream);
}

wholememory_error_code_t wgamd_unique_bounded_live(const void* ids, wholememory_dtype_t id_dtype, int64_t n, const int* n_live_dev,
                                                   int64_t id_bound, int64_t* distinct, int* inverse, int* n_distinct_dev,
                                                   int* out_of_bound_dev, void* workspace, size_t workspace_bytes, void* stream)
{
  using namespace wgamd;
  return guarded("wgamd_unique_bounded", [&] {
    WG_REQUIRE_INPUT(id_dtype == WHOLEMEMORY_DT_INT || id_dtype == WHOLEMEMORY_DT_INT64, "id dtype must be INT|INT64");
    WG_REQUIRE_INPUT(n >= 0 && n < ((int64_t)1 << 31), "bad id count");
    WG_REQUIRE_INPUT(id_bound > 0 && id_bound < ((int64_t)1 << 31) - 4096, "id_bound must be in (0, 2^31)");
    WG_REQUIRE_INPUT(n_distinct_dev && workspace && (n == 0 || (ids && distinct && inverse)), "null pointer");
    const unique_plan p = plan_unique(id_bound);
    WG_REQUIRE_INPUT(workspace_bytes >= p.total, "workspace too small: need %zu bytes", p.total);
    WG_REQUIRE_INPUT((reinterpret_cast<uintptr_t>(workspace) & 255) == 0, "workspace must be 256-byte aligned");
    hipStream_t st = static_cast<hipStream_t>(stream);
    char* base     = static_cast<char*>(workspace);
    uint8_t* flags = reinterpret_cast<uint8_t*>(base + p.flags);
    uint2* rank    = reinterpret_cast<uint2*>(base + p.bits);
    int* cnt       = reinterpret_cast<int*>(base + p.cnt);
    int* tmp       = reinterpret_cast<int*>(base + p.tmp);
    int* bad       = reinterpret_cast<int*>(base + p.bad);
    WG_HIP_CHECK(hipMemsetAsync(flags, 0, (size_t)p.n_words * 32, st));
    WG_HIP_CHECK(hipMemsetAsync(bad, 0, sizeof(int), st));
    if (n > 0) {
      const int grid = (int)std::min<int64_t>(ceil_div(n, 256), 256 * 32);
      if (id_dtype == WHOLEMEMORY_DT_INT) unique_mark_kernel<int32_t><<<grid, 256, 0, st>>>(static_cast<const int32_t*>(ids), n, id_bound, flags, bad, n_live_dev);
      else unique_mark_kernel<int64_t><<<grid, 256, 0, st>>>(static_cast<const int64_t*>(ids), n, id_bound, flags, bad, n_live_dev);
      WG_HIP_CHECK(hipGetLastError());
    }
    unique_pack_kernel<<<(int)ceil_div(p.cnt_padded, 256), 256, 0, st>>>(flags, p.n_words, rank, cnt, p.cnt_padded);
    exclusive_scan_i32(cnt, cnt, p.n_words, tmp, st);
    unique_compact_kernel<<<(int)ceil_div(p.n_words, 256), 256, 0, st>>>(rank, cnt, p.n_words, distinct, n_distinct_dev);
    WG_HIP_CHECK(hipGetLastError());
    if (n > 0) {
      const int grid = (int)std::min<int64_t>(ceil_div(n, 256), 256 * 32);
      if (id_dtype == WHOLEMEMORY_DT_INT) unique_inverse_kernel<int32_t><<<grid, 256, 0, st>>>(static_cast<const int32_t*>(ids), n, id_bound, rank, inverse, n_live_dev);
      else unique_inverse_kernel<int64_t><<<grid, 256, 0, st>>>(static_cast<const int64_t*>(ids), n, id_bound, rank, inverse, n_live_dev);
      WG_HIP_CHECK(hipGetLastError());
    }
    if (out_of_bound_dev) WG_HIP_CHECK(hipMemcpyAsync(out_of_bound_dev, bad, sizeof(int), hipMemcpyDeviceToDevice, st));
  });
}

}
```

### cugraph-gnn_amd/wholegraph_amd/_lib.py

```python
import ctypes
import os
from ctypes import (CFUNCTYPE, POINTER, Structure, c_bool, c_float, c_int, c_int64, c_size_t,
                    c_ulonglong, c_void_p)

_HERE = os.path.dirname(os.path.abspath(__file__))
LIB_PATH = os.environ.get("WGAMD_LIBRARY_PATH") or os.path.normpath(os.path.join(_HERE, "..", "lib", "libwholegraph_amd.so"))

WHOLEMEMORY_MAX_TENSOR_DIM = 8

(WHOLEMEMORY_SUCCESS, WHOLEMEMORY_UNKNOW_ERROR, WHOLEMEMORY_NOT_IMPLEMENTED, WHOLEMEMORY_LOGIC_ERROR,
 WHOLEMEMORY_CUDA_ERROR, WHOLEMEMORY_COMMUNICATION_ERROR, WHOLEMEMORY_INVALID_INPUT,
 WHOLEMEMORY_INVALID_VALUE, WHOLEMEMORY_OUT_OF_MEMORY, WHOLEMEMORY_NOT_SUPPORTED,
 WHOLEMEMORY_SYSTEM_ERROR) = range(11)

_ERROR_NAMES = ["SUCCESS", "UNKNOW_ERROR", "NOT_IMPLEMENTED", "LOGIC_ERROR", "CUDA_ERROR",
                "COMMUNICATION_ERROR", "INVALID_INPUT", "INVALID_VALUE", "OUT_OF_MEMORY",
                "NOT_SUPPORTED", "SYSTEM_ERROR"]

(DT_UNKNOWN, DT_FLOAT, DT_HALF, DT_DOUBLE, DT_BF16, DT_INT, DT_INT64, DT_INT16, DT_INT8,
 DT_COUNT) = range(10)

IDS_BYTE_OFFSETS = 64
HETERO_SAGE_MAX_RELATIONS, HETERO_SAGE_RELU = 8, 1

# ... 250 lines not shown
                                    c_void_p, c_int, c_void_p, c_size_t, c_void_p]),
    "wgamd_rgcn_layer_supported": (c_int, [c_int, c_int, c_int, c_int]),
    "wgamd_rgcn_edge_coef": (c_int, [c_void_p, c_int64, c_void_p, c_int, c_int, c_int, c_void_p, c_void_p, c_void_p]),
    "wgamd_rgcn_layer_f32": (c_int, [c_void_p, c_void_p, c_int64, c_void_p, c_int64, c_int, c_void_p, c_int, c_void_p, c_void_p,
                                     c_void_p, c_void_p, c_int, c_int, c_void_p, c_int64, c_int, c_void_p, c_int, c_void_p, c_int64,
                                     c_void_p]),
    "wgamd_rgcn_wgrad_workspace_bytes": (c_size_t, [c_int64, c_int, c_int]),
    "wgamd_rgcn_wgrad_f32": (c_int, [c_void_p, c_int64, c_int, c_void_p, c_int, c_void_p, c_void_p, c_void_p, c_void_p, c_int64,
                                     c_int, c_void_p, c_void_p, c_int, c_int64, c_int64, c_void_p, c_void_p, c_size_t, c_void_p]),
    "wgamd_transformer_layer_supported": (c_int, [c_int, c_int, c_int, c_int, c_int]),
    "wgamd_transformer_block_width": (c_int, [c_int, c_int]),
    "wgamd_transformer_layer_f32": (c_int, [c_void_p, c_void_p, c_int64, c_void_p, c_int64, c_int, c_void_p, c_int, c_void_p, c_int64,
                                            c_int, c_void_p, c_int, c_void_p, c_int, c_void_p, c_int64, c_void_p, c_int64, c_int,
                                            c_void_p, c_int64, c_int, c_void_p, c_int, c_void_p, c_int64, c_void_p, c_void_p, c_void_p]),
    "wgamd_transformer_bwd_dst_f32": (c_int, [c_void_p, c_void_p, c_int64, c_void_p, c_int64, c_int, c_void_p, c_int, c_void_p, c_int,
                                              c_int, c_void_p, c_void_p, c_int64, c_void_p, c_int64, c_void_p, c_void_p, c_void_p,
                                              c_void_p]),
    "wgamd_transformer_bwd_src_f32": (c_int, [c_void_p, c_void_p, c_void_p, c_void_p, c_int64, c_int64, c_int, c_int, c_int, c_int, c_void_p,
                                              c_void_p, c_void_p, c_int64, c_void_p, c_int64, c_void_p, c_int64, c_int, c_void_p]),
    "wgamd_hetero_sage_layer_supported": (c_int, [POINTER(c_int), c_int, c_int, c_int]),
    "wgamd_hetero_sage_layer_f32": (c_int, [c_void_p, c_int, c_int64, c_void_p, c_int64, c_int, c_void_p, c_void_p, c_int, c_void_p,
                                            c_int64, c_int, c_void_p, c_int, c_void_p, c_int64, c_void_p, c_void_p, c_int64,
                                            c_void_p]),
    "wgamd_hetero_sage_layer_f32_train": (c_int, [c_void_p, c_int, c_int64, c_void_p, c_int64, c_int, c_void_p, c_void_p, c_int,
                                                  c_void_p, c_int64, c_int, c_void_p, c_int, c_void_p, c_int64, c_void_p, c_void_p,
                                                  c_int64, c_void_p, c_int64, c_void_p]),
    "wgamd_gin_layer_supported": (c_int, [c_int, c_int, c_int]),
    "wgamd_gin_layer_f32": (c_int, [c_void_p, c_void_p, c_int64, c_void_p, c_int64, c_int, c_void_p, c_int, c_void_p, c_void_p,
                                    c_int64, c_void_p, c_void_p, c_int64, c_int, c_void_p, c_void_p, c_int64, c_int, c_void_p, c_int,
                                    c_void_p, c_int64, c_void_p]),
    "wgamd_gin_layer_f32_train": (c_int, [c_void_p, c_void_p, c_int64, c_void_p, c_int64, c_int, c_void_p, c_int, c_void_p, c_void_p,
                                          c_int64, c_void_p, c_void_p, c_int64, c_int, c_void_p, c_void_p, c_int64, c_int, c_void_p,
                                          c_int, c_void_p, c_int64, c_void_p, c_int64, c_void_p, c_int64, c_void_p]),
    "wgamd_gin_aggregate_f32": (c_int, [c_void_p, c_void_p, c_int64, c_void_p, c_int64, c_int, c_void_p, c_int, c_void_p, c_void_p,
                                        c_int64, c_void_p, c_void_p, c_int64, c_void_p]),
    "wgamd_segment_sum_f32": (c_int, [c_void_p, c_int64, c_int, c_void_p, c_int64, c_void_p, c_int64, c_void_p]),
    "wgamd_bias_act_rows_f32": (c_int, [c_void_p, c_int64, c_int64, c_int, c_void_p, c_int, c_void_p, c_void_p, c_int64, c_void_p]),
    "wgamd_gat_transform_heads_supported": (c_int, [c_int, c_int, c_int]),
    "wgamd_gat_transform_weight_bytes": (c_size_t, [c_int, c_int, c_int]),
    "wgamd_gat_transform_weight_tiles": (c_int, [c_void_p, c_int64, c_int, c_int, c_int, c_void_p, c_void_p]),
    "wgamd_gat_transform_heads_bf16x3": (c_int, [c_void_p, c_int64, c_int64, c_int, c_int, c_int, c_void_p, c_void_p, c_int64,
                                                 c_void_p, c_int, c_void_p, c_void_p, c_int64, c_void_p]),
    "wgamd_gat_layer_fused_supported": (c_int, [c_int, c_int, c_int]),
    "wgamd_gat_layer_fused_bf16x3": (c_int, [c_void_p, c_void_p, c_int64, c_void_p, c_int64, c_int, c_void_p, c_void_p, c_int, c_int,
                                             c_float, c_void_p, c_void_p, c_void_p, c_int64, c_void_p, c_int, c_void_p, c_void_p,
                                             c_int64, c_void_p]),
    "wgamd_gat_aggregate_heads_f32": (c_int, [c_void_p, c_void_p, c_int64, c_void_p, c_int64, c_int, c_void_p, c_void_p, c_int,
                                              c_float, c_void_p, c_void_p, c_int64, c_void_p]),
    "wgamd_rows_terms_bwd_f32": (c_int, [c_void_p, c_int64, c_int64, c_int, c_void_p, c_int, c_void_p, c_void_p]),
    "wgamd_gather_term_slabs_f32": (c_int, [c_void_p, c_int64, c_int, c_void_p, c_int, c_int64, c_void_p, c_void_p]),
    "wgamd_gat_aggregate_heads_bwd_f32": (c_int, [c_void_p, c_void_p, c_int64, c_void_p, c_int64, c_void_p, c_void_p, c_int, c_int,
                                                  c_void_p, c_void_p, c_int, c_float, c_void_p, c_void_p, c_int64, c_void_p, c_void_p,
                                                  c_void_p, c_void_p, c_int64, c_void_p, c_void_p]),
    "wgamd_gat_aggregate_heads_bwd_gx_f32": (c_int, [c_void_p, c_void_p, c_int64, c_int64, c_int, c_void_p, c_void_p, c_int, c_float,
                                                     c_void_p, c_void_p, c_void_p, c_int64, c_void_p, c_int64, c_void_p]),
    "wgamd_gat_aggregate_heads_ids_f32": (c_int, [c_void_p, c_void_p, c_int64, c_void_p, c_int64, c_void_p, c_void_p, c_int, c_int,
                                                  c_void_p, c_void_p, c_int, c_float, c_void_p, c_void_p, c_int64, c_void_p]),
    "wgamd_gat_layer_fused_ids_bf16x3": (c_int, [c_void_p, c_void_p, c_int64, c_void_p, c_int64, c_void_p, c_void_p, c_int, c_int,
                                                 c_void_p, c_void_p, c_int, c_int, c_float, c_void_p, c_void_p, c_void_p, c_int64,
                                                 c_void_p, c_int, c_void_p, c_void_p, c_int64, c_void_p]),
    "wgamd_gat_csr_rows_f32": (c_int, [c_void_p, c_void_p, c_int64, c_void_p, c_int64, c_void_p, c_void_p, c_int, c_int, c_float,
                                       c_void_p, c_int, c_void_p, c_void_p, c_int64, c_void_p]),
    "wgamd_set_weighted_sampling_mode": (None, [c_int, c_int]),
    "wgamd_set_sample_locality_min": (None, [c_int64]),
    "wgamd_sample_hop_workspace_bytes": (c_size_t, [c_int64, c_int64, c_int]),
    "wgamd_sample_hop_weighted_workspace_bytes": (c_size_t, [c_int64, c_int64, c_int, c_int64]),
    "wgamd_sample_hop_nosync": (c_int, [c_void_p, c_void_p, c_int, c_void_p, c_void_p, c_int64, c_int,
                                        c_ulonglong, c_void_p, c_void_p, c_void_p, c_void_p, c_int64, c_void_p,
                                        c_void_p, c_void_p, c_size_t, c_void_p]),
    "wgamd_sample_hop_pyg_nosync": (c_int, [c_void_p, c_void_p]),
    "wgamd_call_group_target_rows": (c_int, [c_void_p, c_void_p, c_void_p, c_int64, c_void_p, c_void_p]),
    "wgamd_sample_hop_batched_nosync": (c_int, [c_void_p, c_void_p, c_int, c_void_p, c_void_p, c_void_p, c_int,
                                                c_int64, c_int, c_void_p, c_void_p, c_void_p, c_void_p, c_void_p,
                                                c_int64, c_void_p, c_void_p, c_void_p, c_void_p, c_void_p, c_size_t,
                                                c_int64, c_void_p]),
    "wgamd_gather_terms_supported": (c_int, [c_int, c_int]),
    "wgamd_gather_terms_f32": (c_int, [c_void_p, c_int64, c_void_p, c_int, c_int64, c_int, c_void_p, c_int, c_void_p, c_int64,
                                       c_void_p, c_int64, c_int, c_void_p]),
    "wgamd_unique_bounded_workspace_bytes": (c_size_t, [c_int64]),
    "wgamd_unique_bounded": (c_int, [c_void_p, c_int, c_int64, c_int64, c_void_p, c_void_p, c_void_p, c_void_p, c_void_p,
                                     c_size_t, c_void_p]),
    "wgamd_unique_bounded_live": (c_int, [c_void_p, c_int, c_int64, c_void_p, c_int64, c_void_p, c_void_p, c_void_p, c_void_p,
                                          c_void_p, c_size_t, c_void_p]),
    "wgamd_sample_hop_batched_nosync_ex": (c_int, [c_void_p, c_void_p, c_int, c_void_p, c_void_p, c_void_p, c_int,
                                                   c_int64, c_int, c_void_p, c_void_p, c_void_p, c_void_p, c_void_p,
                                                   c_int64, c_void_p, c_void_p, c_void_p, c_void_p, c_void_p, c_size_t,
                                                   c_int64, ctypes.c_uint, c_void_p]),
}

_lib = None


def lib():
    global _lib
    if _lib is None:
        if not os.path.exists(LIB_PATH):
            raise WholeGraphLibraryError(
                f"{LIB_PATH} not found: build the HIP library first "
                "(python -c 'import __graft_entry__ as g; g.build()' or make -C cugraph-gnn_amd/csrc). "
                "There is no CPU fallback.")
        handle = ctypes.CDLL(LIB_PATH)
        for name, sig in SYMBOLS.items():
            fn = getattr(handle, name)
            if sig is not None:
                fn.restype, fn.argtypes = sig
        _lib = handle
    return _lib


def check(code, what):
    if code != WHOLEMEMORY_SUCCESS:
        raise WholeMemoryError(code, what)
```

### cugraph-gnn_amd/wholegraph_amd/fused.py

```python
from dataclasses import dataclass, field
from typing import List, Sequence, Union

import torch

from . import _lib as L
from .env import get_stream, torch_dtype_to_wm


HOP_NO_UNIQUE_PAD = 1
HOP_COL_INT32 = 2

_COL32 = {}


def compact_columns(col: torch.Tensor, n_vertices: int):
    import weakref
    if col.dtype != torch.int64 or not (0 < int(n_vertices) < (1 << 31)) or not col.is_cuda:
        return None
    key = (col.data_ptr(), col.numel())
    hit = _COL32.get(key)
    if hit is not None and hit[0]() is col:
        return hit[1]
    for k in [k for k, v in _COL32.items() if v[0]() is None]:
        del _COL32[k]
# ... 29 lines not shown

    def target_rows_in_unique(self, k: int, n_targets: int) -> torch.Tensor:
        rows = torch.empty((n_targets,), dtype=torch.int64, device=self.unique_seg[k].device)
        L.check(L.lib().wgamd_call_group_target_rows(self.unique_seg[k].data_ptr(), self.target_seg[k].data_ptr(),
                                                     self.target_batch[k].data_ptr(), int(n_targets), rows.data_ptr(),
                                                     get_stream()), "wgamd_call_group_target_rows")
        return rows

    def finalize_batches(self):
        hops, G = self.hops, self.n_batches
        tseg = [t.cpu().tolist() for t in self.target_seg]
        useg = [t.cpu().tolist() for t in self.unique_seg]
        eseg = [self.offsets[k][torch.as_tensor(tseg[k], device=self.offsets[k].device).long()].cpu().tolist()
                for k in range(hops)]
        out = []
        for b in range(G):
            target_gids = [None] * (hops + 1)
            edge_indice, csr_row_ptr, csr_col_ind = [None] * hops, [None] * hops, [None] * hops
            target_gids[hops] = self.seeds[b * self.batch_size:(b + 1) * self.batch_size]
            for k in range(hops):
                i = hops - 1 - k
                t0, t1 = tseg[k][b], tseg[k][b + 1]
                e0, e1 = eseg[k][b], eseg[k][b + 1]
                csr_row_ptr[i] = self.offsets[k][t0:t1 + 1] - e0
                csr_col_ind[i] = self.neighbor_row[k][e0:e1] - useg[k][b]
                edge_indice[i] = torch.stack([csr_col_ind[i], self.center_row[k][e0:e1] - t0])
                target_gids[i] = self.unique[k][useg[k][b]:useg[k][b + 1]]
            out.append((target_gids, edge_indice, csr_row_ptr, csr_col_ind))
        return out

    def finalize(self):
        assert self.n_batches == 1
        return self.finalize_batches()[0]

    def finalize_single(self, copy: bool = False):
        assert self.n_batches == 1
        hops = self.hops
        sz = self.counts.cpu().tolist()
        keep = (lambda t: t.clone()) if copy else (lambda t: t)
        target_gids = [None] * hops + [self.seeds]
        edge_indice, csr_row_ptr, csr_col_ind = [None] * hops, [None] * hops, [None] * hops
        n_t = int(self.seeds.shape[0])
        for k in range(hops):
            i = hops - 1 - k
            n_e, n_u = sz[k]
            csr_row_ptr[i] = keep(self.offsets[k][:n_t + 1])
            csr_col_ind[i] = keep(self.neighbor_row[k][:n_e])
            edge_indice[i] = torch.stack([csr_col_ind[i], self.center_row[k][:n_e]])
            target_gids[i] = keep(self.unique[k][:n_u])
            n_t = n_u
        return target_gids, edge_indice, csr_row_ptr, csr_col_ind


def _merge_hops_batch_major(fields_per_hop, segs_per_hop, G, dev):
    H = len(fields_per_hop)
    n_fields = len(fields_per_hop[0]) if H else 0
    tot, offs = [0] * G, [0] * (G + 1)
    for s_ in segs_per_hop:
        for b in range(G):
            tot[b] += s_[b + 1] - s_[b]
    for b in range(G):
        offs[b + 1] = offs[b] + tot[b]
    if H == 0:
        return [], offs
    live = [[f[s_[0]:s_[G]] for f in fs] for fs, s_ in zip(fields_per_hop, segs_per_hop)]
    if H == 1:
        return live[0], offs
    shift, before = [], [0] * G
    for s_ in segs_per_hop:
        shift.append([offs[b] + before[b] - s_[b] for b in range(G)])
        before = [before[b] + s_[b + 1] - s_[b] for b in range(G)]
    meta = torch.tensor([[s_[b + 1] - s_[b] for b in range(G)] for s_ in segs_per_hop] + shift, dtype=torch.int64).to(dev)
    batches = torch.arange(G, device=dev)
    merged = [torch.empty(offs[G], dtype=live[0][i].dtype, device=dev) for i in range(n_fields)]
    for h in range(H):
        n_h = segs_per_hop[h][G] - segs_per_hop[h][0]
        if n_h == 0:
            continue
        b_of = torch.repeat_interleave(batches, meta[h], output_size=n_h)
        dest = torch.arange(segs_per_hop[h][0], segs_per_hop[h][G], device=dev) + meta[H + h][b_of]
        for i in range(n_fields):
            merged[i][dest] = live[h][i]
    return merged, offs


class NoSyncWalk:
    def __init__(self, csr_row_ptr: torch.Tensor, csr_col_ind: torch.Tensor, batch_size: int,
                 max_neighbors: List[int], id_dtype=torch.int64, n_batches: int = 1, pad_unique: bool = True,
                 compact_col: bool = True):
        assert csr_row_ptr.is_cuda and csr_col_ind.is_cuda
        assert all(m > 0 for m in max_neighbors), "the no-sync walk needs positive fan-outs"
        self.flags = 0 if pad_unique else HOP_NO_UNIQUE_PAD
        assert csr_col_ind.dtype == id_dtype, "no-sync walk: seeds and csr_col must share a dtype"
        self.row_ptr, self.col = csr_row_ptr, csr_col_ind
        self.n_vertices = int(csr_row_ptr.shape[0]) - 1
        c32 = compact_columns(csr_col_ind, self.n_vertices) if compact_col else None
        if c32 is not None:
            self.col, self.flags = c32, self.flags | HOP_COL_INT32
        self.fanouts = list(max_neighbors)
        self.id_dtype = id_dtype
        self.wm_dtype = torch_dtype_to_wm(id_dtype)
        self.G, self.B = int(n_batches), int(batch_size)
        dev = csr_row_ptr.device
        self.target_caps, self.edge_caps = [], []
        t = self.G * self.B
        for m in self.fanouts:
            self.target_caps.append(t)
            self.edge_caps.append(t * m)
            t = t + t * m
        assert t < (1 << 30), "call group too large: lower n_batches"
        lib = L.lib()
        ws = max(lib.wgamd_sample_hop_workspace_bytes(tc, ec, self.wm_dtype)
                 for tc, ec in zip(self.target_caps, self.edge_caps))
        self.workspace = torch.empty(ws + 256, dtype=torch.uint8, device=dev)
        self.ws_off = (-self.workspace.data_ptr()) % 256
        self.ws_bytes = ws
        self.dev = dev
        self.seed_seg = (torch.arange(self.G + 1, dtype=torch.int32, device=dev) * self.B).contiguous()
        self.seed_batch = torch.arange(self.G, dtype=torch.int32, device=dev).repeat_interleave(self.B).contiguous()

    def _seeds_tensor(self, random_seeds) -> torch.Tensor:
        if isinstance(random_seeds, torch.Tensor):
            t = random_seeds.to(device=self.dev, dtype=torch.int64)
        else:
            rows = []
            for per_hop in random_seeds:
                vals = [per_hop] * self.G if isinstance(per_hop, int) else list(per_hop)
                rows.append([(int(v) & 0xFFFFFFFFFFFFFFFF) - (1 << 64) if (int(v) & (1 << 63)) else int(v) & 0xFFFFFFFFFFFFFFFF
                             for v in vals])
            t = torch.tensor(rows, dtype=torch.int64, device=self.dev)
        assert t.shape == (len(self.fanouts), self.G), f"random_seeds must be [hops={len(self.fanouts)}, G={self.G}]"
        return t.contiguous()

    def run(self, seeds: torch.Tensor, random_seeds: Union[torch.Tensor, Sequence]) -> WalkResult:
        assert seeds.dtype == self.id_dtype and seeds.shape[0] == self.G * self.B
        lib, dev = L.lib(), self.dev
        hops = len(self.fanouts)
        rs = self._seeds_tensor(random_seeds)
        counts = torch.empty((hops, 2), dtype=torch.int32, device=dev)
        res = WalkResult(hops, self.G, self.B, seeds, counts=counts, target_caps=self.target_caps)
        res._keepalive = [rs]
        targets, t_batch, t_seg = seeds, self.seed_batch, self.seed_seg
        stream = get_stream()
        ws_ptr = self.workspace.data_ptr() + self.ws_off
        for k, (m, tc, ec) in enumerate(zip(self.fanouts, self.target_caps, self.edge_caps)):
            offsets = torch.empty(tc + 1, dtype=torch.int32, device=dev)
            nbr_row = torch.empty(ec, dtype=torch.int32, device=dev)
            ctr_row = torch.empty(ec, dtype=torch.int32, device=dev)
            unique = torch.empty(tc + ec, dtype=self.id_dtype, device=dev)
            u_batch = torch.empty(tc + ec, dtype=torch.int32, device=dev) if k + 1 < hops else None
            u_seg = torch.empty(self.G + 1, dtype=torch.int32, device=dev)
            L.check(lib.wgamd_sample_hop_batched_nosync_ex(
                self.row_ptr.data_ptr(), self.col.data_ptr(), self.wm_dtype, targets.data_ptr(), t_batch.data_ptr(),
                t_seg.data_ptr(), self.G, tc, m, rs[k].data_ptr(), offsets.data_ptr(), nbr_row.data_ptr(),
                ctr_row.data_ptr(), None, ec, unique.data_ptr(), None if u_batch is None else u_batch.data_ptr(),
                u_seg.data_ptr(),
                counts[k].data_ptr(), ws_ptr, self.ws_bytes, self.n_vertices, self.flags, stream),
                "wgamd_sample_hop_batched_nosync_ex")
            res.unique.append(unique)
            res.unique_seg.append(u_seg)
            res.target_seg.append(t_seg)
            res.target_batch.append(t_batch)
            res.offsets.append(offsets)
            res.neighbor_row.append(nbr_row)
            res.center_row.append(ctr_row)
            targets, t_batch, t_seg = unique, u_batch, u_seg
        return res


class CapturedWalk:

    def __init__(self, walk: NoSyncWalk):
        self.walk = walk
        self._graph = self._res = None
        hops = len(walk.fanouts)
        self._seeds = torch.zeros(walk.G * walk.B, dtype=walk.id_dtype, device=walk.dev)
        self._rs = torch.zeros((hops, walk.G), dtype=torch.int64, device=walk.dev)
        self._rs_host = torch.zeros((hops, walk.G), dtype=torch.int64).pin_memory()

    def run(self, seeds: torch.Tensor, random_seeds) -> WalkResult:
        w = self.walk
        if isinstance(random_seeds, torch.Tensor):
            self._rs.copy_(random_seeds.to(torch.int64).view_as(self._rs), non_blocking=True)
        else:
            for k, per_hop in enumerate(random_seeds):
                vals = [per_hop] * w.G if isinstance(per_hop, int) else list(per_hop)
                for b, v in enumerate(vals):
                    v = int(v) & 0xFFFFFFFFFFFFFFFF
                    self._rs_host[k, b] = v - (1 << 64) if v & (1 << 63) else v
            self._rs.copy_(self._rs_host, non_blocking=True)
        self._seeds.copy_(seeds, non_blocking=True)
        if self._graph is None:
            cur = torch.cuda.current_stream()
            side = torch.cuda.Stream(device=w.dev)
            side.wait_stream(cur)
            with torch.cuda.stream(side):
                w.run(self._seeds, self._rs)
            cur.wait_stream(side)
            g = torch.cuda.CUDAGraph()
            with torch.cuda.graph(g):
                self._res = w.run(self._seeds, self._rs)
            self._graph = g
        self._graph.replay()
        return self._res


class SingleBatchNoSyncWalk:

    def __init__(self, csr_row_ptr, csr_col_ind, batch_size, max_neighbors, id_dtype=torch.int64):
        self.inner = NoSyncWalk(csr_row_ptr, csr_col_ind, batch_size, max_neighbors, id_dtype, 1, compact_col=False)

    def run(self, seeds, random_seeds: Sequence[int]) -> WalkResult:
        w = self.inner
        lib, dev = L.lib(), w.dev
        hops = len(w.fanouts)
        counts = torch.empty((hops, 2), dtype=torch.int32, device=dev)
        n_seeds = torch.full((1,), seeds.shape[0], dtype=torch.int32, device=dev)
        res = WalkResult(hops, 1, w.B, seeds, counts=counts, target_caps=w.target_caps)
        res._keepalive = [n_seeds]
        targets, n_ptr = seeds, n_seeds.data_ptr()
        zero = torch.zeros(1, dtype=torch.int32, device=dev)
        t_seg = torch.cat([zero, n_seeds])
        for k, (m, tc, ec) in enumerate(zip(w.fanouts, w.target_caps, w.edge_caps)):
            offsets = torch.empty(tc + 1, dtype=torch.int32, device=dev)
            nbr = torch.empty(ec, dtype=torch.int32, device=dev)
            ctr = torch.empty(ec, dtype=torch.int32, device=dev)
            unique = torch.empty(tc + ec, dtype=w.id_dtype, device=dev)
            L.check(lib.wgamd_sample_hop_nosync(
                w.row_ptr.data_ptr(), w.col.data_ptr(), w.wm_dtype, targets.data_ptr(), n_ptr, tc, m,
                int(random_seeds[k]) & 0xFFFFFFFFFFFFFFFF, offsets.data_ptr(), nbr.data_ptr(), ctr.data_ptr(), None, ec,
                unique.data_ptr(), counts[k].data_ptr(), w.workspace.data_ptr() + w.ws_off, w.ws_bytes, get_stream()),
                "wgamd_sample_hop_nosync")
            res.unique.append(unique)
            res.offsets.append(offsets)
            res.neighbor_row.append(nbr)
            res.center_row.append(ctr)
            res.target_seg.append(t_seg)
            u_seg = torch.cat([zero, counts[k, 1:2]])
            res.unique_seg.append(u_seg)
            targets, n_ptr, t_seg = unique, counts[k].data_ptr() + 4, u_seg
        return res


import ctypes as _ct


class _PygHop(_ct.Structure):
    _fields_ = [("csr_row_ptr", _ct.c_void_p), ("csr_col", _ct.c_void_p), ("id_dtype", _ct.c_int),
                ("n_batches", _ct.c_int), ("max_sample_count", _ct.c_int), ("random_seeds_dev", _ct.c_void_p),
                ("nodes", _ct.c_void_p), ("node_batch", _ct.c_void_p), ("node_seg", _ct.c_void_p),
                ("node_cap", _ct.c_int64),
                ("frontier", _ct.c_void_p), ("frontier_batch", _ct.c_void_p), ("frontier_seg", _ct.c_void_p),
                ("frontier_local0", _ct.c_void_p), ("frontier_cap", _ct.c_int64),
                ("offsets", _ct.c_void_p), ("neighbor_local", _ct.c_void_p), ("center_local", _ct.c_void_p),
                ("edge_gid", _ct.c_void_p), ("edge_cap", _ct.c_int64),
                ("nodes_out", _ct.c_void_p), ("nodes_out_batch", _ct.c_void_p), ("nodes_out_seg", _ct.c_void_p),
# ... 20 lines not shown
    frontier_batch: List[torch.Tensor] = field(default_factory=list)
    frontier_local0: List[torch.Tensor] = field(default_factory=list)
    counts: torch.Tensor = None

    def finalize_batches(self, edge_id: torch.Tensor = None):
        G, hops = self.n_batches, self.hops
        pieces = list(self.frontier_seg) + [self.node_seg] + [self.offsets[k][self.frontier_seg[k].long()] for k in range(hops)]
        flat = torch.cat([p_.reshape(-1).to(torch.int64) for p_ in pieces]).cpu().tolist()
        host, at = [], 0
        for p_ in pieces:
            host.append(flat[at:at + p_.numel()])
            at += p_.numel()
        fseg = host[:hops + 1]
        nseg = host[hops + 1]
        eseg = host[hops + 2:]
        fields = []
        for k in range(hops):
            lo, hi = eseg[k][0], eseg[k][G]
            gid = self.edge_gid[k]
            fields.append([self.row_local[k][:hi].long(), self.col_local[k][:hi].long(),
                           edge_id[gid[:hi]] if edge_id is not None else gid[:hi]])
        (rows, cols, edges), offs = _merge_hops_batch_major(fields, eseg, G, self.nodes.device)
        sizes_b = [offs[b + 1] - offs[b] for b in range(G)]
        node_v = torch.split(self.nodes[nseg[0]:nseg[G]], [nseg[b + 1] - nseg[b] for b in range(G)])
        row_v, col_v, edge_v = (torch.split(t[:offs[G]], sizes_b) for t in (rows, cols, edges))
        self.group_context = dict(nodes=self.nodes[nseg[0]:nseg[G]], node_sizes=[nseg[b + 1] - nseg[b] for b in range(G)],
                                  edges=edges[:offs[G]], edge_sizes=sizes_b)
        E, dev = offs[G], self.nodes.device
        if E > 0 and rows.dtype == torch.int64:
            n_b = [nseg[b + 1] - nseg[b] for b in range(G)]
            Nn = nseg[G] - nseg[0]
            meta = torch.tensor([sizes_b, n_b, [v + 1 for v in n_b], [nseg[b] - nseg[0] for b in range(G)], offs[:G]],
                                dtype=torch.int64).to(dev)
            ar = torch.arange(G, device=dev)
            ei_all = torch.stack([rows[:E], cols[:E]])
            b_of_e = torch.repeat_interleave(ar, meta[0], output_size=E)
            keys = cols[:E] + meta[3][b_of_e]
            rp_all = torch.searchsorted(keys, torch.arange(Nn + 1, device=dev))
            b_of_p = torch.repeat_interleave(ar, meta[2], output_size=Nn + G)
            rp_cat = (rp_all[torch.arange(Nn + G, device=dev) - b_of_p] - meta[4][b_of_p]).to(torch.int32)
            col32 = rows[:E].to(torch.int32)
            self.group_context["edge_index"] = torch.split(ei_all, sizes_b, dim=1)
            self.group_context["csr"] = list(zip(torch.split(rp_cat, [v + 1 for v in n_b]), torch.split(col32, sizes_b)))
        out, nn_all, ne_all = [], [], []
        for b in range(G):
            nn = [fseg[0][b + 1] - fseg[0][b]] + [fseg[k + 1][b + 1] - fseg[k + 1][b] for k in range(hops)]
            ne = [eseg[k][b + 1] - eseg[k][b] for k in range(hops)]
            nn_all.append(nn), ne_all.append(ne)
            out.append((node_v[b], row_v[b], col_v[b], edge_v[b], nn, ne))
        self.group_context["num_sampled_nodes"] = torch.tensor(nn_all).unbind(0)
        self.group_context["num_sampled_edges"] = torch.tensor(ne_all).unbind(0)
        return out


class PygNoSyncWalk:

    def __init__(self, csr_row_ptr, csr_col_ind, batch_size: int, fanout: List[int], n_batches: int = 1,
                 csr_weight: torch.Tensor = None, pad_unique: bool = True, compact_col: bool = True):
        self.flags = 0 if pad_unique else HOP_NO_UNIQUE_PAD
        assert csr_row_ptr.is_cuda and csr_col_ind.is_cuda and csr_col_ind.dtype in (torch.int32, torch.int64)
        assert all(0 < f for f in fanout), "the no-sync walk needs positive fan-outs"
        self.weight, self.max_row_len = None, 0
        if csr_weight is not None:
            assert csr_weight.is_cuda and csr_weight.dtype in (torch.float32, torch.float64) and all(f <= 256 for f in fanout)
            assert csr_weight.shape[0] == csr_col_ind.shape[0]
            self.weight = csr_weight.contiguous()
            self.max_row_len = max(int((csr_row_ptr[1:] - csr_row_ptr[:-1]).max()), 1) if csr_row_ptr.shape[0] > 1 else 1
        self.row_ptr, self.col = csr_row_ptr, csr_col_ind
        self.id_dtype, self.wm_dtype = csr_col_ind.dtype, torch_dtype_to_wm(csr_col_ind.dtype)
        c32 = compact_columns(csr_col_ind, int(csr_row_ptr.shape[0]) - 1) if compact_col else None
        if c32 is not None:
            self.col, self.flags = c32, self.flags | HOP_COL_INT32
        self.G, self.B, self.fanout = int(n_batches), int(batch_size), [int(f) for f in fanout]
        dev = csr_row_ptr.device
        self.frontier_caps, self.edge_caps, self.node_caps = [], [], []
        f, n = self.G * self.B, self.G * self.B
        for m in self.fanout:
            self.frontier_caps.append(f)
            self.node_caps.append(n)
            self.edge_caps.append(f * m)
            n, f = n + f * m, f * m
        assert n < (1 << 30), "call group too large: lower n_batches"
        lib = L.lib()
        if self.weight is None:
            ws = max(lib.wgamd_sample_hop_workspace_bytes(max(nc, fc), ec, self.wm_dtype)
                     for nc, fc, ec in zip(self.node_caps, self.frontier_caps, self.edge_caps))
        else:
            ws = max(lib.wgamd_sample_hop_weighted_workspace_bytes(max(nc, fc), ec, self.wm_dtype, self.max_row_len)
                     for nc, fc, ec in zip(self.node_caps, self.frontier_caps, self.edge_caps))
        self.workspace = torch.empty(ws + 256, dtype=torch.uint8, device=dev)
        self.ws_off, self.ws_bytes, self.dev = (-self.workspace.data_ptr()) % 256, ws, dev
        self.seed_seg = (torch.arange(self.G + 1, dtype=torch.int32, device=dev) * self.B).contiguous()
        self.seed_batch = torch.arange(self.G, dtype=torch.int32, device=dev).repeat_interleave(self.B).contiguous()
        self.zeros_g = torch.zeros(self.G, dtype=torch.int32, device=dev)

    def run(self, seeds: torch.Tensor, random_seeds, seed_seg: torch.Tensor = None, seed_batch: torch.Tensor = None) -> PygWalkResult:
        assert seeds.dtype == self.id_dtype and seeds.shape[0] == self.G * self.B
        assert (seed_seg is None) == (seed_batch is None)
        lib, dev, G = L.lib(), self.dev, self.G
        hops = len(self.fanout)
        if isinstance(random_seeds, torch.Tensor):
            rs = random_seeds.to(device=dev, dtype=torch.int64).contiguous()
        else:
            rs = torch.tensor([[v - (1 << 64) if v & (1 << 63) else v for v in (int(x) & 0xFFFFFFFFFFFFFFFF for x in row)]
                               for row in random_seeds], dtype=torch.int64, device=dev)
        assert rs.shape == (hops, G)
        res = PygWalkResult(hops, G, self.B, counts=torch.empty((hops, 2), dtype=torch.int32, device=dev))
        res._keepalive = [rs]
        if seed_seg is None:
            seed_seg, seed_batch = self.seed_seg, self.seed_batch
        else:
            assert seed_seg.dtype == torch.int32 and seed_seg.shape[0] == G + 1 and seed_seg.is_contiguous()
            assert seed_batch.dtype == torch.int32 and seed_batch.shape[0] == G * self.B and seed_batch.is_contiguous()
        nodes, n_batch, n_seg = seeds, seed_batch, seed_seg
        front, f_batch, f_seg, f_local0 = seeds, seed_batch, seed_seg, self.zeros_g
        i32 = dict(dtype=torch.int32, device=dev)
        for k, (m, fc, nc, ec) in enumerate(zip(self.fanout, self.frontier_caps, self.node_caps, self.edge_caps)):
            offsets = torch.empty(fc + 1, **i32)
            row_l, col_l = torch.empty(ec, **i32), torch.empty(ec, **i32)
            scratch_r, scratch_c = torch.empty(ec, **i32), torch.empty(ec, **i32)
            gid = torch.empty(ec, dtype=torch.int64, device=dev)
            nodes_out = torch.empty(nc + ec, dtype=self.id_dtype, device=dev)
            nodes_out_batch, nodes_out_seg = torch.empty(nc + ec, **i32), torch.empty(G + 1, **i32)
            f_out = torch.empty(ec, dtype=self.id_dtype, device=dev)
            f_out_batch, f_out_seg, f_out_l0 = torch.empty(ec, **i32), torch.empty(G + 1, **i32), torch.empty(G, **i32)
            p = _PygHop(self.row_ptr.data_ptr(), self.col.data_ptr(), self.wm_dtype, G, m, rs[k].data_ptr(),
                        nodes.data_ptr(), n_batch.data_ptr(), n_seg.data_ptr(), nc,
                        front.data_ptr(), f_batch.data_ptr(), f_seg.data_ptr(), f_local0.data_ptr(), fc,
                        offsets.data_ptr(), row_l.data_ptr(), col_l.data_ptr(), gid.data_ptr(), ec,
                        nodes_out.data_ptr(), nodes_out_batch.data_ptr(), nodes_out_seg.data_ptr(),
                        f_out.data_ptr(), f_out_batch.data_ptr(), f_out_seg.data_ptr(), f_out_l0.data_ptr(),
                        res.counts[k].data_ptr(), scratch_r.data_ptr(), scratch_c.data_ptr(),
                        self.workspace.data_ptr() + self.ws_off, self.ws_bytes,
                        None if self.weight is None else self.weight.data_ptr(),
                        0 if self.weight is None else torch_dtype_to_wm(self.weight.dtype), self.max_row_len,
                        int(self.row_ptr.shape[0]) - 1, self.flags)
            L.check(lib.wgamd_sample_hop_pyg_nosync(_ct.byref(p), get_stream()), "wgamd_sample_hop_pyg_nosync")
            res.offsets.append(offsets)
            res.row_local.append(row_l)
            res.col_local.append(col_l)
            res.edge_gid.append(gid)
            res.frontier_seg.append(f_seg)
            res.frontier_batch.append(f_batch)
            res.frontier_local0.append(f_local0)
            res._keepalive += [scratch_r, scratch_c, f_batch, n_batch, front, f_local0]
            nodes, n_batch, n_seg = nodes_out, nodes_out_batch, nodes_out_seg
            front, f_batch, f_seg, f_local0 = f_out, f_out_batch, f_out_seg, f_out_l0
        res.frontier_seg.append(f_seg)
        res.nodes, res.node_seg = nodes, n_seg
        return res


class HeteroPygWalk:

    def __init__(self, graphs, batch_size: int, fanout, n_batches: int, biased: bool = False, num_nodes=None,
                 pad_unique: bool = True):
        self.flags = 0 if pad_unique else HOP_NO_UNIQUE_PAD
        self.biased = bool(biased)
        self.num_nodes = dict(num_nodes) if num_nodes else {}
        self.etypes = sorted(graphs.keys())
        self.graphs = graphs
        self.G, self.B = int(n_batches), int(batch_size)
        self.fanout = {et: [int(f) for f in fanout.get(et, [])] for et in self.etypes}
        self.hops = len(next(iter(fanout.values())))
        for et in self.etypes:
            if not self.fanout[et]:
                self.fanout[et] = [0] * self.hops
            assert len(self.fanout[et]) == self.hops and all(f >= 0 for f in self.fanout[et])
            assert graphs[et].col.dtype == torch.int64 and graphs[et].row_ptr.is_cuda
        self.ntypes = sorted({t for et in self.etypes for t in (et[0], et[2])})
        self.dev = graphs[self.etypes[0]].row_ptr.device
        self.wm_dtype = torch_dtype_to_wm(torch.int64)
        self._ws = None
        dev = self.dev
        self.seed_seg = (torch.arange(self.G + 1, dtype=torch.int32, device=dev) * self.B).contiguous()
        self.seed_batch = torch.arange(self.G, dtype=torch.int32, device=dev).repeat_interleave(self.B).contiguous()
        self.zeros_g = torch.zeros(self.G, dtype=torch.int32, device=dev)
        self.zeros_g1 = torch.zeros(self.G + 1, dtype=torch.int32, device=dev)
        self.col32 = {et: compact_columns(graphs[et].col, int(self.num_nodes.get(et[0], 0))) for et in self.etypes}
        self.max_row_len = {}
        if self.biased:
            for et in self.etypes:
                g = graphs[et]
                assert g.weight is not None and g.weight.dtype in (torch.float32, torch.float64)
                assert all(f <= 256 for f in self.fanout[et])
                self.max_row_len[et] = max(int((g.row_ptr[1:] - g.row_ptr[:-1]).max()), 1) if g.row_ptr.shape[0] > 1 else 1

    def _workspace(self, node_cap, edge_cap, max_row_len=0):
        if max_row_len > 0:
            need = L.lib().wgamd_sample_hop_weighted_workspace_bytes(node_cap, edge_cap, self.wm_dtype, max_row_len)
        else:
            need = L.lib().wgamd_sample_hop_workspace_bytes(node_cap, edge_cap, self.wm_dtype)
        if self._ws is None or self._ws.numel() < need + 256:
            self._ws = torch.empty(need + 256, dtype=torch.uint8, device=self.dev)
        off = (-self._ws.data_ptr()) % 256
        return self._ws.data_ptr() + off, self._ws.numel() - off

    def _frontier(self, st, cap):
        G, dev = self.G, self.dev
        if G <= 4095 and st["nodes"].shape[0] >= 1 and st["seg"].dtype == torch.int32 and st["begin"].dtype == torch.int32:
            nodes, seg, begin = st["nodes"].contiguous(), st["seg"].contiguous(), st["begin"].contiguous()
            ids = torch.empty(cap, dtype=torch.int64, device=dev)
            b = torch.empty(cap, dtype=torch.int32, device=dev)
            f_seg = torch.empty(G + 1, dtype=torch.int32, device=dev)
            L.check(L.lib().wgamd_frontier_list(nodes.data_ptr(), int(nodes.shape[0]), seg.data_ptr(), begin.data_ptr(), G, int(cap),
                                                ids.data_ptr(), b.data_ptr(), f_seg.data_ptr(), get_stream()), "wgamd_frontier_list")
            return ids, b, f_seg, begin
        size_b = st["seg"][1:] - st["seg"][:-1]
        cnt = (size_b - st["begin"]).to(torch.int32)
        f_seg = torch.zeros(G + 1, dtype=torch.int32, device=dev)
        f_seg[1:] = torch.cumsum(cnt, 0)
        p = torch.arange(cap, dtype=torch.int32, device=dev)
        b = torch.searchsorted(f_seg[1:].contiguous(), p, right=True).clamp_(max=G - 1)
        src = st["seg"][:-1][b].long() + st["begin"][b].long() + (p - f_seg[:-1][b]).long()
        ids = st["nodes"][src.clamp_(0, st["nodes"].shape[0] - 1)]
        return ids.contiguous(), b.to(torch.int32).contiguous(), f_seg, st["begin"].contiguous()

    def run(self, seed_type: str, seeds: torch.Tensor, random_seeds: torch.Tensor, seed_lists=None):
        lib, dev, G = L.lib(), self.dev, self.G
        assert seed_lists is not None or (seeds.dtype == torch.int64 and seeds.shape[0] == G * self.B and seeds.is_cuda)
        rs = random_seeds.to(device=dev, dtype=torch.int64).contiguous()
        assert rs.shape == (self.hops * len(self.etypes), G)
        i32 = dict(dtype=torch.int32, device=dev)
        state = {}
        for t in self.ntypes:
            state[t] = dict(nodes=torch.zeros(1, dtype=torch.int64, device=dev), batch=torch.zeros(1, **i32),
                            seg=self.zeros_g1, cap=0, begin=self.zeros_g, gained_cap=0)
        if seed_lists is None:
            state[seed_type] = dict(nodes=seeds, batch=self.seed_batch, seg=self.seed_seg, cap=G * self.B,
                                    begin=self.zeros_g, gained_cap=G * self.B)
        else:
            for t, (ids, seg, batch) in seed_lists.items():
                assert ids.dtype == torch.int64 and seg.dtype == torch.int32 and batch.dtype == torch.int32
                assert seg.shape[0] == G + 1 and batch.shape[0] == ids.shape[0]
                state[t] = dict(nodes=ids.contiguous(), batch=batch.contiguous(), seg=seg.contiguous(), cap=int(ids.shape[0]),
                                begin=self.zeros_g, gained_cap=int(ids.shape[0]))
        rec = dict(calls=[], sizes=[{t: (state[t]["seg"][1:] - state[t]["seg"][:-1]) for t in self.ntypes}])
        keep = [rs]
        for h in range(self.hops):
            fronts = {t: (self._frontier(state[t], state[t]["gained_cap"]) if state[t]["gained_cap"] > 0 else None)
                      for t in self.ntypes}
            f_caps = {t: state[t]["gained_cap"] for t in self.ntypes}
            for t in self.ntypes:
                st = state[t]
                st["begin"] = (st["seg"][1:] - st["seg"][:-1]).to(torch.int32).contiguous()
                st["gained_cap"] = 0
            for ti, et in enumerate(self.etypes):
                src_t, _, dst_t = et
                m, fr = self.fanout[et][h], fronts[dst_t]
                if m == 0 or fr is None:
                    rec["calls"].append(None)
                    continue
                g = self.graphs[et]
                f_ids, f_batch, f_seg, f_l0 = fr
                fc = f_caps[dst_t]
                ec = fc * m
                st = state[src_t]
# ... 87 lines not shown
```

### include/wgamd_ext.h

```cpp
#ifndef WGAMD_EXT_H_
#define WGAMD_EXT_H_

#include "wgamd_types.h"

#ifdef __cplusplus
extern "C" {
#endif


wholememory_error_code_t wgamd_spmm_csr_f32(const int* row_ptr,
                                            const int* col,
                                            int64_t n_rows,
                                            const float* x,
                                            int64_t ldx,
                                            int F,
                                            const void* src_ids,
                                            wholememory_dtype_t src_ids_dtype,
                                            int mean,
                                            float* out,
                                            int64_t ldo,
                                            void* stream);

wholememory_error_code_t wgamd_sage_aggregate_f32(const int* row_ptr,
                                                  const int* col,
// ... 276 lines not shown
                                                          const float* a_dst, int H, int C, float negative_slope,
                                                          const int64_t* dst_rows, const void* w_tiles, const float* acc_in,
                                                          int64_t ld_acc, const float* bias, int relu, const int64_t* out_rows,
                                                          float* out, int64_t ldo, void* stream);

size_t wgamd_gat_csr_bwd_workspace_bytes(int64_t n_entries, int H, int C);
wholememory_error_code_t wgamd_gat_csr_bwd_f32(const int* row_ptr, const int* col, int64_t n_rows, const float* x, int64_t ldx,
                                               const float* a_src, const float* a_dst, int H, int C, float negative_slope,
                                               const float* alpha, const float* grad_out, int64_t ldg, const int* row_ptr_t,
                                               const int* edge_perm, const int* edge_dst, int64_t n_src, float* de,
                                               float* grad_x, int64_t ldgx, float* grad_a_src, float* grad_a_dst,
                                               void* workspace, size_t workspace_bytes, void* stream);
wholememory_error_code_t wgamd_gat_csr_bwd_f32_v2(const int* row_ptr, const int* col, int64_t n_rows, const float* x, int64_t ldx,
                                                  const float* a_src, const float* a_dst, int H, int C, float negative_slope,
                                                  const float* alpha, const float* grad_out, int64_t ldg, const int* row_ptr_t,
                                                  const int* edge_perm, const int* edge_dst, int64_t n_src, float* de,
                                                  float* grad_x, int64_t ldgx, float* grad_a_src, float* grad_a_dst,
                                                  int64_t n_entries, void* workspace, size_t workspace_bytes, void* stream);

wholememory_error_code_t wgamd_sage_layer_fused_f32(const int* row_ptr, const int* col, int64_t n_rows, const float* x,
                                                    int64_t ldx, int64_t x_rows, int F, const void* src_ids,
                                                    wholememory_dtype_t src_ids_dtype, const int64_t* self_rows, int mean,
                                                    const float* w_t, int64_t ldw, int N, const float* bias, int relu,
                                                    float* out, int64_t ldo, void* stream);

size_t wgamd_sage_weight_planes_bytes(int K, int N);
int wgamd_sage_layer_bf16x3_supported(int F, int N);
wholememory_error_code_t wgamd_sage_layer_weight_planes(const float* w_l, int64_t ldl, const float* w_r, int64_t ldr,
                                                        const float* bias, int F, int N, int Np, void* planes,
                                                        float* bias_out, int full_tiles, void* stream);
#define WGAMD_SAGE_FULL_TILES 2
int wgamd_sage_layer_uses_half_tiles(int F);
wholememory_error_code_t wgamd_sage_split_weight_bf16x3(const float* w_t, int64_t ldw, int K, int N, void* planes,
                                                        void* stream);
wholememory_error_code_t wgamd_sage_layer_fused_bf16x3(const int* row_ptr, const int* col, int64_t n_rows, const float* x,
                                                       int64_t ldx, int64_t x_rows, int F, const void* src_ids,
                                                       wholememory_dtype_t src_ids_dtype, const int64_t* self_rows, int mean,
                                                       const void* w_planes, int N, const float* bias, int relu, float* out,
                                                       int64_t ldo, void* stream);

wholememory_error_code_t wgamd_sage_layer_fused_bf16x3_train(const int* row_ptr, const int* col, int64_t n_rows, const float* x,
                                                             int64_t ldx, int64_t x_rows, int F, const void* src_ids,
                                                             wholememory_dtype_t src_ids_dtype, const int64_t* self_rows,
                                                             int mean, const void* w_planes, int N, const float* bias, int relu,
                                                             float* out, int64_t ldo, float* agg_out, int64_t ld_agg,
                                                             void* stream);

size_t wgamd_sage_wgrad_workspace_bytes(int64_t n_rows, int F, int N);
wholememory_error_code_t wgamd_sage_wgrad_bf16x3(const float* agg, int64_t ld_agg, const float* x, int64_t ldx, int F,
                                                 const void* src_ids, wholememory_dtype_t src_ids_dtype,
                                                 const int64_t* self_rows, int64_t n_rows, const float* grad_out, int64_t ldg,
                                                 const float* act_out, int64_t ld_act, int N, float* grad_w_l,
                                                 float* grad_w_r, float* grad_bias, int accumulate, void* workspace,
                                                 size_t workspace_bytes, void* stream);

#define WGAMD_IDS_BYTE_OFFSETS ((wholememory_dtype_t)64)

void wgamd_set_weighted_sampling_mode(int pruning, int force_redo);
void wgamd_set_sample_locality_min(int64_t min_capacity);

wholememory_error_code_t wgamd_csr_uniform_sample_with_replacement(
  wholememory_tensor_t wm_csr_row_ptr_tensor, wholememory_tensor_t wm_csr_col_ptr_tensor,
  wholememory_tensor_t center_nodes_tensor, int sample_count, wholememory_tensor_t output_sample_offset_tensor,
  void* output_dest_memory_context, void* output_center_localid_memory_context, void* output_edge_gid_memory_context,
  unsigned long long random_seed, wholememory_env_func_t* p_env_fns, void* stream);

int wgamd_gather_terms_supported(int F, int T);
wholememory_error_code_t wgamd_gather_terms_f32(const float* table, int64_t ldt, const void* ids, wholememory_dtype_t id_dtype,
                                                int64_t n, int F, const float* v, int T, float* out_x, int64_t ldx,
                                                float* out_terms, int64_t ldo, int term_group, void* stream);
wholememory_error_code_t wgamd_gather_term_slabs_f32(const float* slabs_in, int64_t n_in, int n_slabs, const void* ids,
                                                     wholememory_dtype_t id_dtype, int64_t n, float* slabs_out, void* stream);
wholememory_error_code_t wgamd_rows_terms_bwd_f32(const float* x, int64_t ldx, int64_t n, int F, const float* dterms, int T,
                                                  float* dv, void* stream);

size_t wgamd_unique_bounded_workspace_bytes(int64_t id_bound);
wholememory_error_code_t wgamd_unique_bounded(const void* ids, wholememory_dtype_t id_dtype, int64_t n, int64_t id_bound,
                                              int64_t* distinct, int* inverse, int* n_distinct_dev, int* out_of_bound_dev,
                                              void* workspace, size_t workspace_bytes, void* stream);
wholememory_error_code_t wgamd_unique_bounded_live(const void* ids, wholememory_dtype_t id_dtype, int64_t n, const int* n_live_dev,
                                                   int64_t id_bound, int64_t* distinct, int* inverse, int* n_distinct_dev,
                                                   int* out_of_bound_dev, void* workspace, size_t workspace_bytes, void* stream);

size_t wgamd_softmax_xent_state_bytes(int64_t n_rows);
wholememory_error_code_t wgamd_softmax_xent_forward_f32(const float* logits, int64_t ld, int64_t n_rows, int n_classes,
                                                        const int64_t* target, const float* row_weight, float* lse, void* state,
                                                        int state_is_zeroed, float* loss_out, void* stream);
wholememory_error_code_t wgamd_softmax_xent_backward_f32(const float* logits, int64_t ld, int64_t n_rows, int n_classes,
                                                         const int64_t* target, const float* row_weight, const float* lse,
                                                         const void* state, const float* grad_loss, float* grad_logits, int64_t ldg,
                                                         void* stream);

#define WGAMD_GCN_ADD_SELF_LOOPS 1
#define WGAMD_GCN_RELU 2
#define WGAMD_GCN_MAX_HOPS 8
int wgamd_gcn_layer_supported(int F, int N);
wholememory_error_code_t wgamd_gcn_layer_f32(const int* row_ptr, const int* col, int64_t n_rows, const float* x, int64_t ldx, int F,
                                             const void* src_ids, wholememory_dtype_t src_ids_dtype, const int64_t* self_rows,
                                             const float* edge_weight, const float* dinv_src, const float* dinv_dst, float fill,
                                             const float* w, int64_t ldw, int N, const float* bias, int flags, float* out,
                                             int64_t ldo, void* stream);
wholememory_error_code_t wgamd_gcn_layer_f32_train(const int* row_ptr, const int* col, int64_t n_rows, const float* x, int64_t ldx,
                                                   int F, const void* src_ids, wholememory_dtype_t src_ids_dtype,
                                                   const int64_t* self_rows, const float* edge_weight, const float* dinv_src,
                                                   const float* dinv_dst, float fill, const float* w, int64_t ldw, int N,
                                                   const float* bias, int flags, float* out, int64_t ldo, float* agg_out,
                                                   int64_t ld_agg, void* stream);
wholememory_error_code_t wgamd_gcn_aggregate_f32(const int* row_ptr, const int* col, int64_t n_rows, const float* x, int64_t ldx,
                                                 int F, const void* src_ids, wholememory_dtype_t src_ids_dtype,
                                                 const int64_t* self_rows, const float* edge_weight, const float* dinv_src,
                                                 const float* dinv_dst, float fill, int flags, float* out, int64_t ldo,
                                                 void* stream);
wholememory_error_code_t wgamd_gcn_degrees_f32(int n_hops, const int* const* row_ptr, const int* const* col,
                                               const int64_t* const* self_rows, const float* const* edge_weight,
                                               const int64_t* n_rows, const int64_t* out_base, float fill, int add_self_loops,
                                               float* dinv, int64_t n_out, void* stream);
size_t wgamd_gcn_wgrad_workspace_bytes(int64_t n_rows, int F, int N);
wholememory_error_code_t wgamd_gcn_wgrad_f32(const float* agg, int64_t ld_agg, int64_t n_rows, int F, const float* grad_out,
                                             int64_t ldg, const float* act_out, int64_t ld_act, int N, float* grad_w,
                                             float* grad_bias, int accumulate, void* workspace, size_t workspace_bytes,
                                             void* stream);

int wgamd_rgcn_layer_supported(int F, int N, int B, int has_root);
wholememory_error_code_t wgamd_rgcn_edge_coef(const int* row_ptr, int64_t n_rows, const void* edge_type,
                                              wholememory_dtype_t edge_type_dtype, int R, int mean, int* rel, float* coef,
                                              void* stream);
wholememory_error_code_t wgamd_rgcn_layer_f32(const int* row_ptr, const int* col, int64_t n_rows, const float* x, int64_t ldx, int F,
                                              const void* src_ids, wholememory_dtype_t src_ids_dtype, const int64_t* self_rows,
                                              const int* rel, const float* coef, const float* comp, int B, int has_root,
                                              const float* wt, int64_t ldw, int N, const float* bias, int relu, float* out,
                                              int64_t ldo, void* stream);
size_t wgamd_rgcn_wgrad_workspace_bytes(int64_t max_items, int F, int N);
wholememory_error_code_t wgamd_rgcn_wgrad_f32(const float* x, int64_t ldx, int F, const void* src_ids,
                                              wholememory_dtype_t src_ids_dtype, const int64_t* pair_src, const int64_t* pair_dst,
                                              const float* pair_coef, const float* grad, int64_t ldg, int N,
                                              const int64_t* item_start, const int64_t* seg_ptr, int n_seg, int64_t pairs_per_item,
                                              int64_t max_items, float* M, void* workspace, size_t workspace_bytes, void* stream);

int wgamd_transformer_layer_supported(int F_src, int F_dst, int D, int H, int N);
int wgamd_transformer_block_width(int F_src, int D);
wholememory_error_code_t wgamd_transformer_layer_f32(const int* row_ptr, const int* col, int64_t n_rows, const float* x, int64_t ldx,
                                                     int F_src, const void* src_ids, wholememory_dtype_t src_ids_dtype,
                                                     const float* x_dst, int64_t ldx_dst, int F_dst, const int64_t* self_rows,
                                                     int x_dst_ids, const float* edge_attr, int D, const float* u, int64_t ldu,
                                                     const float* w, int64_t ldw, int H, const float* wt, int64_t ldwt, int N,
                                                     const float* bias, int relu, float* out, int64_t ldo, float* alpha, float* a_save,
                                                     void* stream);
wholememory_error_code_t wgamd_transformer_bwd_dst_f32(const int* row_ptr, const int* col, int64_t n_rows, const float* x, int64_t ldx,
                                                       int F_src, const void* src_ids, wholememory_dtype_t src_ids_dtype,
                                                       const float* edge_attr, int D, int H, const float* alpha, const float* dA,
                                                       int64_t ldda, const float* A, int64_t lda, float* du, float* dw, float* ds,
                                                       void* stream);
wholememory_error_code_t wgamd_transformer_bwd_src_f32(const int* row_ptr_t, const int* col_t, const int* perm, const int64_t* self_t,
                                                       int64_t n_rows, int64_t n_src, int F_src, int D, int H, int skip_at,
                                                       const float* alpha, const float* ds, const float* dA, int64_t ldda,
                                                       const float* u, int64_t ldu, float* gx, int64_t ldgx, int accumulate,
                                                       void* stream);

#define WGAMD_HETERO_SAGE_MAX_RELATIONS 8
#define WGAMD_HETERO_SAGE_RELU 1
typedef struct {
  const int* row_ptr;
  const int* col;
  const float* x;
  int64_t ldx;
  const void* src_ids;
// ... 46 lines not shown
```

Baseline: 5.283 billion sampled-edges/s.

## Precompute PCG stream jump table and cache per-row RNG indices in sampler

After: 5.215 billion sampled-edges/s. -1.3%, worse.

```diff
diff --git a/cugraph-gnn_amd/csrc/wg_common.hpp b/cugraph-gnn_amd/csrc/wg_common.hpp
--- a/cugraph-gnn_amd/csrc/wg_common.hpp
+++ b/cugraph-gnn_amd/csrc/wg_common.hpp
@@ -10,6 +10,7 @@
 #include <string>
 #include <unordered_map>
 
+#include "wg_pcg_stream.hpp"
 #include "wgamd_ops.h"
 #include "wgamd_tensor.h"
 #include "wgamd_types.h"
@@ -228,6 +229,7 @@
   const unsigned long long* seeds_dev;
   const int* target_batch;
   const int* target_seg;
+  pcg_stream_table tab{};
   __device__ __forceinline__ void resolve(int i, uint64_t& s, int& i_local) const
   {
     s       = seed;
@@ -268,9 +270,10 @@
                             dev_count n, int M, rng_plan random_seed, const int* offsets, void* dst, int* src_lid,
                             int64_t* edge_gid, hipStream_t stream,
                             const int64_t* row_start = nullptr, const int* row_deg = nullptr,
-                            const sample_locality* loc = nullptr);
+                            const sample_locality* loc = nullptr, const void* row_rng = nullptr);
 void sample_count_enqueue(const int64_t* row_ptr, const void* seeds, bool seeds64, dev_count n, int M, int* cnt,
-                          int* big_deg, hipStream_t stream, int64_t* row_start = nullptr, int* row_deg = nullptr);
+                          int* big_deg, hipStream_t stream, int64_t* row_start = nullptr, int* row_deg = nullptr,
+                          void* row_rng = nullptr, const int* target_batch = nullptr, const int* target_seg = nullptr);
 constexpr int kWeightedBlocks  = 1024;
 constexpr int kWeightedLdsKeys = 12288;
 constexpr int kWeightedLists    = 9;
diff --git a/cugraph-gnn_amd/csrc/wg_fused.hip b/cugraph-gnn_amd/csrc/wg_fused.hip
--- a/cugraph-gnn_amd/csrc/wg_fused.hip
+++ b/cugraph-gnn_amd/csrc/wg_fused.hip
@@ -122,13 +122,15 @@
   } else {
     int64_t* row_start = reinterpret_cast<int64_t*>(base + w.row_start);
     int* row_deg       = reinterpret_cast<int*>(base + w.row_deg);
-    sample_count_enqueue(a.csr_row_ptr, s_targets, i64, S, a.M, cnt, nullptr, st, row_start, row_deg);
+    void* row_rng = batched && a.rng.target_batch && a.rng.target_seg && a.M <= 32 && (int64_t)w.slots >= s_cap ? keys : nullptr;
+    sample_count_enqueue(a.csr_row_ptr, s_targets, i64, S, a.M, cnt, nullptr, st, row_start, row_deg, row_rng, a.rng.target_batch,
+                         a.rng.target_seg);
     exclusive_scan_i32(cnt, a.offsets, s_cap, scan_tmp, st, s_n_dev);
     const int64_t loc_min = sample_locality_min().load(std::memory_order_relaxed);
     sample_locality loc{reinterpret_cast<int*>(base + w.loc_hist), keys, sample_locality_shift(a.bv.id_bound)};
     const bool use_loc = a.M <= 32 && s_cap >= loc_min && a.bv.id_bound > 0 && batched && 8 * w.slots >= 32 * s_cap;
     uniform_sample_enqueue(a.csr_row_ptr, a.csr_col, col64, s_targets, i64, S, a.M, a.rng, a.offsets, nbr, a.center_row,
-                           a.edge_gid, st, row_start, row_deg, use_loc ? &loc : nullptr);
+                           a.edge_gid, st, row_start, row_deg, use_loc ? &loc : nullptr, use_loc ? nullptr : row_rng);
   }
   dev_count E{(int)a.edge_cap, a.offsets + s_cap};
   batch_view bv   = a.bv;
diff --git a/cugraph-gnn_amd/csrc/wg_pcg_stream.hip b/cugraph-gnn_amd/csrc/wg_pcg_stream.hip
--- /dev/null
+++ b/cugraph-gnn_amd/csrc/wg_pcg_stream.hip
@@ -0,0 +1,106 @@
+#include <atomic>
+#include <map>
+
+#include "wg_common.hpp"
+#include "wg_rng.hpp"
+#include "wgamd_ext.h"
+
+namespace wgamd {
+namespace {
+
+__global__ void __launch_bounds__(256) pcg_stream_table_kernel(PcgStreamEntry* __restrict__ t, uint32_t n)
+{
+  const uint32_t J = blockIdx.x * blockDim.x + threadIdx.x;
+  if (J >= n) return;
+  PcgJump j = g_pcg_jump.t[0][J & 255u];
+#pragma unroll
+  for (int k = 1; k < 4; k++) {
+    const PcgJump m = g_pcg_jump.t[k][(J >> (8 * k)) & 255u];
+    j.s             = j.s * m.a + m.s;
+    j.a             = j.a * m.a;
+  }
+  const uint64_t a1 = j.a * Pcg32::kMult;
+  PcgStreamEntry e;
+  e.a  = a1;
+  e.s  = j.s + j.a + a1;
+  t[J] = e;
+}
+
+struct device_table {
+  PcgStreamEntry* entries = nullptr;
+  uint32_t built          = 0;
+};
+std::mutex g_mutex;
+std::map<int, device_table> g_tables;
+std::atomic<uint32_t> g_limit{[] {
+  const char* e = getenv("WGAMD_PCG_STREAM_TABLE");
+  return e && e[0] == '0' ? 0u : kPcgStreamTableEntries;
+}()};
+
+}
+
+pcg_stream_table pcg_stream_table_current()
+{
+  const uint32_t limit = g_limit.load(std::memory_order_relaxed);
+  if (limit == 0) return {};
+  int dev = 0;
+  if (hipGetDevice(&dev) != hipSuccess) {
+    (void)hipGetLastError();
+    return {};
+  }
+  std::lock_guard<std::mutex> g(g_mutex);
+  auto it = g_tables.find(dev);
+  if (it == g_tables.end()) return {};
+  return {it->second.entries, std::min(limit, it->second.built)};
+}
+
+}
+
+extern "C" {
+
+wholememory_error_code_t wgamd_pcg_stream_table_prepare(void* stream)
+{
+  using namespace wgamd;
+  return guarded("wgamd_pcg_stream_table_prepare", [&] {
+    int dev = 0;
+    WG_HIP_CHECK(hipGetDevice(&dev));
+    std::lock_guard<std::mutex> g(g_mutex);
+    if (g_tables.find(dev) != g_tables.end()) return;
+    hipStream_t st                   = static_cast<hipStream_t>(stream);
+    hipStreamCaptureStatus capturing = hipStreamCaptureStatusNone;
+    if (hipStreamIsCapturing(st, &capturing) != hipSuccess) (void)hipGetLastError();
+    WG_REQUIRE_INPUT(capturing == hipStreamCaptureStatusNone, "prepare the PCG stream table before the stream capture begins");
+    void* p = nullptr;
+    WG_HIP_CHECK(hipMalloc(&p, sizeof(PcgStreamEntry) * (size_t)kPcgStreamTableEntries));
+    pcg_stream_table_kernel<<<kPcgStreamTableEntries / 256, 256, 0, st>>>(static_cast<PcgStreamEntry*>(p), kPcgStreamTableEntries);
+    hipError_t err = hipGetLastError();
+    if (err == hipSuccess) err = hipStreamSynchronize(st);
+    if (err != hipSuccess) {
+      (void)hipFree(p);
+      WG_HIP_CHECK(err);
+    }
+    g_tables[dev] = device_table{static_cast<PcgStreamEntry*>(p), kPcgStreamTableEntries};
+  });
+}
+
+void wgamd_pcg_stream_table_limit(unsigned int entries)
+{
+  wgamd::g_limit.store(std::min(entries, wgamd::kPcgStreamTableEntries), std::memory_order_relaxed);
+}
+
+void wgamd_pcg_stream_table_entry(unsigned long long J, unsigned long long* a, unsigned long long* s)
+{
+  uint64_t acc_a = 1, acc_s = 0, cur_a = wgamd::Pcg32::kMult, cur_s = 1;
+  for (uint64_t n = J + 1; n; n >>= 1) {
+    if (n & 1u) {
+      acc_s = acc_s * cur_a + cur_s;
+      acc_a *= cur_a;
+    }
+    cur_s = cur_s * cur_a + cur_s;
+    cur_a *= cur_a;
+  }
+  if (a) *a = acc_a;
+  if (s) *s = acc_s * wgamd::Pcg32::kMult + 1;
+}
+
+}
diff --git a/cugraph-gnn_amd/csrc/wg_pcg_stream.hpp b/cugraph-gnn_amd/csrc/wg_pcg_stream.hpp
--- /dev/null
+++ b/cugraph-gnn_amd/csrc/wg_pcg_stream.hpp
@@ -0,0 +1,20 @@
+#pragma once
+#include <cstdint>
+
+namespace wgamd {
+
+struct alignas(16) PcgStreamEntry {
+  unsigned long long a;
+  unsigned long long s;
+};
+
+struct pcg_stream_table {
+  const PcgStreamEntry* entries = nullptr;
+  uint32_t limit                = 0;
+};
+
+constexpr uint32_t kPcgStreamTableEntries = 1u << 20;
+
+pcg_stream_table pcg_stream_table_current();
+
+}
diff --git a/cugraph-gnn_amd/csrc/wg_rng.hpp b/cugraph-gnn_amd/csrc/wg_rng.hpp
--- a/cugraph-gnn_amd/csrc/wg_rng.hpp
+++ b/cugraph-gnn_amd/csrc/wg_rng.hpp
@@ -2,6 +2,8 @@
 #include <hip/hip_runtime.h>
 
 #include <cstdint>
+
+#include "wg_pcg_stream.hpp"
 
 namespace wgamd {
 
@@ -89,11 +91,17 @@
   }
 
   struct table_tag {};
-  __device__ __forceinline__ Pcg32(uint64_t seed, uint32_t subsequence, table_tag, uint32_t extra_draws = 0)
+  __device__ __forceinline__ Pcg32(uint64_t seed, uint32_t subsequence, table_tag, pcg_stream_table tab, uint32_t extra_draws = 0)
   {
-    inc   = ((uint64_t)subsequence << 1u) | 1u;
-    state = (inc + seed) * kMult + inc;
-    jump_table(subsequence + extra_draws);
+    inc              = ((uint64_t)subsequence << 1u) | 1u;
+    const uint32_t J = subsequence + extra_draws;
+    if (J < tab.limit) {
+      const PcgStreamEntry e = tab.entries[J];
+      state                  = e.a * seed + inc * e.s;
+    } else {
+      state = (inc + seed) * kMult + inc;
+      jump_table(J);
+    }
   }
 
   __host__ __device__ __forceinline__ int32_t next_i31() { return (int32_t)(next_u32() & 0x7fffffffu); }
diff --git a/cugraph-gnn_amd/csrc/wg_sample.hip b/cugraph-gnn_amd/csrc/wg_sample.hip
--- a/cugraph-gnn_amd/csrc/wg_sample.hip
+++ b/cugraph-gnn_amd/csrc/wg_sample.hip
@@ -35,10 +35,10 @@
   return (uint64_t)(int64_t)(int32_t)(seed_index * B + lane);
 }
 
-__device__ __forceinline__ Pcg32 stream_generator(uint64_t random_seed, int64_t seed_index, int B, int lane)
+__device__ __forceinline__ Pcg32 stream_generator(uint64_t random_seed, int64_t seed_index, int B, int lane, pcg_stream_table tab)
 {
   const int64_t sid = seed_index * B + lane;
-  if (sid < (1ll << 31)) return Pcg32(random_seed, (uint32_t)sid, Pcg32::table_tag{});
+  if (sid < (1ll << 31)) return Pcg32(random_seed, (uint32_t)sid, Pcg32::table_tag{}, tab);
   return Pcg32(random_seed, stream_id(seed_index, B, lane));
 }
 
@@ -56,7 +56,10 @@
                                                            int list_cap            = 0,
                                                            int scratch_threshold   = 0,
                                                            int64_t* __restrict__ row_start = nullptr,
-                                                           int* __restrict__ row_deg       = nullptr)
+                                                           int* __restrict__ row_deg       = nullptr,
+                                                           int2* __restrict__ row_rng      = nullptr ,
+                                                           const int* __restrict__ target_batch = nullptr,
+                                                           const int* __restrict__ target_seg   = nullptr)
 {
   const int n_live = n_.get();
   if (lists == nullptr) {
@@ -70,6 +73,10 @@
         if (row_start) {
           row_start[i] = first;
           row_deg[i]   = deg;
+        }
+        if (row_rng) {
+          const int b = target_batch[i];
+          row_rng[i]  = make_int2(i - target_seg[b], b);
         }
         deg = (M > 0 && deg > M) ? M : deg;
       }
@@ -268,7 +275,7 @@
     } else
       rng.resolve(i, random_seed, i_local);
     if (i_local < (1 << 26)) {
-      Pcg32 g(random_seed, (uint32_t)(i_local * 32 + hl), Pcg32::table_tag{});
+      Pcg32 g(random_seed, (uint32_t)(i_local * 32 + hl), Pcg32::table_tag{}, rng.tab);
       r_draw = g.next_i31();
     } else {
       Pcg32 g(random_seed, stream_id(i_local, 32, hl));
@@ -325,7 +332,7 @@
 sample_uniform_multi_kernel(const ColT* __restrict__ col, dev_count n_, int M_rt, rng_plan rng, const int* __restrict__ offsets,
                             ColT* __restrict__ dst, int* __restrict__ src_lid, int64_t* __restrict__ edge_gid,
                             const int64_t* __restrict__ row_start, const int* __restrict__ row_deg,
-                            const loc_rec* __restrict__ recs)
+                            const loc_rec* __restrict__ recs, const int2* __restrict__ row_rng)
 {
   constexpr int kGPW    = 64 / GW;
   constexpr int kGroups = 4 * kGPW;
@@ -364,10 +371,15 @@
         start[k] = row_start[i[k]];
         N[k]     = row_deg[i[k]];
         base[k]  = offsets[i[k]];
-        if (rng.target_batch) batch[k] = rng.target_batch[i[k]];
-      }
-    }
-    if (rng.target_batch) {
+        if (row_rng) {
+          const int2 q = row_rng[i[k]];
+          i_local[k] = q.x, batch[k] = q.y;
+        } else if (rng.target_batch) {
+          batch[k] = rng.target_batch[i[k]];
+        }
+      }
+    }
+    if (rng.target_batch && !row_rng) {
 #pragma unroll
       for (int k = 0; k < K; k++)
         if (i[k] < n) i_local[k] = i[k] - rng.target_seg[batch[k]];
@@ -380,7 +392,7 @@
     if (i[k] < n && hl < M) {
       const uint64_t random_seed = rng.seeds_dev ? rng.seeds_dev[rng.target_batch ? batch[k] : 0] : rng.seed;
       if (i_local[k] < (1 << 26)) {
-        Pcg32 g(random_seed, (uint32_t)(i_local[k] * 32 + hl), Pcg32::table_tag{});
+        Pcg32 g(random_seed, (uint32_t)(i_local[k] * 32 + hl), Pcg32::table_tag{}, rng.tab);
         r_draw[k] = g.next_i31();
       } else {
         Pcg32 g(random_seed, stream_id(i_local[k], 32, hl));
@@ -653,7 +665,7 @@
     bool redrawn = false;
     if (m0 < m1) {
       const int64_t sid = (int64_t)i_rng * B + lane;
-      Pcg32 g = (sid < (1ll << 31)) ? Pcg32(random_seed, (uint32_t)sid, Pcg32::table_tag{}, 3u * (uint32_t)m0)
+      Pcg32 g = (sid < (1ll << 31)) ? Pcg32(random_seed, (uint32_t)sid, Pcg32::table_tag{}, rng.tab, 3u * (uint32_t)m0)
                                     : Pcg32(random_seed, stream_id(i_rng, B, lane));
       if (sid >= (1ll << 31)) g.skipahead(3u * (uint64_t)m0);
       for (int m = m0; m < m1; m++) {
@@ -666,7 +678,7 @@
   __syncthreads();
   if (T > B && sh_redo) {
     if (threadIdx.x < B) {
-      Pcg32 g = stream_generator(random_seed, i_rng, B, threadIdx.x);
+      Pcg32 g = stream_generator(random_seed, i_rng, B, threadIdx.x, rng.tab);
       for (int id = threadIdx.x; id < N; id += B) put(id, key_bits(ares_key((float)weight[start + id], g)));
     }
     __syncthreads();
@@ -783,7 +795,7 @@
     N                 = (int)(row_ptr[nid + 1] - start);
     base              = offsets[i];
     if (hl < N) {
-      Pcg32 g = stream_generator(random_seed, i_rng, 128, hl);
+      Pcg32 g = stream_generator(random_seed, i_rng, 128, hl, rng.tab);
       k       = key_bits(ares_key((float)weight[start + hl], g));
     }
   }
@@ -832,8 +844,8 @@
   const int64_t base  = offsets[i];
   uint32_t k[KMAX];
   {
-    Pcg32 ga = stream_generator(random_seed, i_rng, 128, lane);
-    Pcg32 gb = stream_generator(random_seed, i_rng, 128, lane + 64);
+    Pcg32 ga = stream_generator(random_seed, i_rng, 128, lane, rng.tab);
+    Pcg32 gb = stream_generator(random_seed, i_rng, 128, lane + 64, rng.tab);
 #pragma unroll
     for (int s = 0; s < KMAX; s++) {
       const int id = (s >> 1) * 128 + (s & 1) * 64 + lane;
@@ -989,8 +1001,8 @@
     float wv[KMAX];
 #pragma unroll
     for (int s = 0; s < KMAX; s++) wv[s] = (float)weight[start + min(s * 64 + lane, N - 1)];
-    KeyStream ga(stream_generator(random_seed, i_rng, 128, lane));
-    KeyStream gb(stream_generator(random_seed, i_rng, 128, lane + 64));
+    KeyStream ga(stream_generator(random_seed, i_rng, 128, lane, rng.tab));
+    KeyStream gb(stream_generator(random_seed, i_rng, 128, lane + 64, rng.tab));
 #pragma unroll
     for (int s = 0; s < KMAX; s++) {
       const int id = s * 64 + lane;
@@ -1310,7 +1322,7 @@
     const int m0 = part * share, m1 = min(L, m0 + share);
     const int rounds = (((N + B - 1) / B) + 3) / 4;
     const int64_t sid = (int64_t)i_rng * B + sl;
-    Pcg32 g0 = (sid < (1ll << 31)) ? Pcg32(random_seed, (uint32_t)sid, Pcg32::table_tag{}, 3u * (uint32_t)m0)
+    Pcg32 g0 = (sid < (1ll << 31)) ? Pcg32(random_seed, (uint32_t)sid, Pcg32::table_tag{}, rng.tab, 3u * (uint32_t)m0)
                                    : Pcg32(random_seed, stream_id(i_rng, B, sl));
     if (sid >= (1ll << 31)) g0.skipahead(3u * (uint64_t)m0);
     KeyStream g(g0);
@@ -1399,7 +1411,8 @@
 template <typename SeedT, typename ColT>
 void uniform_launch(const int64_t* row_ptr, const ColT* col, const SeedT* seeds, dev_count n, int M,
                     rng_plan random_seed, const int* offsets, ColT* dst, int* lid, int64_t* gid, hipStream_t stream,
-                    const int64_t* row_start = nullptr, const int* row_deg = nullptr, const sample_locality* loc = nullptr)
+                    const int64_t* row_start = nullptr, const int* row_deg = nullptr, const sample_locality* loc = nullptr,
+                    const int2* row_rng = nullptr)
 {
   const int cap = n.host;
   if (cap <= 0) return;
@@ -1420,7 +1433,7 @@
 #define WG_MULTI(GW, KK)                                                                                             \
   sample_uniform_multi_kernel<SeedT, ColT, GW, KK, WG_EXACT>                                                          \
     <<<(int)std::min<int64_t>((ceil_div((int64_t)cap, 4 * (64 / GW) * KK) + 15) / 8 * 8, kWalkGrid), 256, 0, stream>>>(           \
-      col, n, M, random_seed, offsets, dst, lid, gid, row_start, row_deg, recs)
+      col, n, M, random_seed, offsets, dst, lid, gid, row_start, row_deg, recs, recs ? nullptr : row_rng)
 #define WG_MULTI_K(GW)                                                                                               \
   do {                                                                                                               \
     if (K == 1) WG_MULTI(GW, 1); else if (K == 2) WG_MULTI(GW, 2); else WG_MULTI(GW, 4);                              \
@@ -1501,6 +1514,7 @@
                             int64_t slab_len, ColT* dst, int* lid, int64_t* gid, hipStream_t stream)
 {
   if (n.host <= 0) return;
+  rng.tab       = pcg_stream_table_current();
   const int cap = n.host;
   if (M <= 0 || M > 256) {
     sample_weighted_kernel<SeedT, ColT, WeightT, 256, 256><<<std::max(blocks, 1), 256, 0, stream>>>(
@@ -1761,15 +1775,17 @@
 }
 
 void sample_count_enqueue(const int64_t* row_ptr, const void* seeds, bool seeds64, dev_count n, int M, int* cnt,
-                          int* big_deg, hipStream_t stream, int64_t* row_start, int* row_deg)
+                          int* big_deg, hipStream_t stream, int64_t* row_start, int* row_deg, void* row_rng,
+                          const int* target_batch, const int* target_seg)
 {
   if (n.host <= 0) return;
+  int2* rr = target_batch && target_seg ? static_cast<int2*>(row_rng) : nullptr;
   if (seeds64)
     sample_count_kernel<int64_t><<<std::min(ceil_div(n.host, 256), kWalkGrid), 256, 0, stream>>>(
-      row_ptr, static_cast<const int64_t*>(seeds), n, M, cnt, big_deg, nullptr, 0, 0, row_start, row_deg);
+      row_ptr, static_cast<const int64_t*>(seeds), n, M, cnt, big_deg, nullptr, 0, 0, row_start, row_deg, rr, target_batch, target_seg);
   else
     sample_count_kernel<int32_t><<<std::min(ceil_div(n.host, 256), kWalkGrid), 256, 0, stream>>>(
-      row_ptr, static_cast<const int32_t*>(seeds), n, M, cnt, big_deg, nullptr, 0, 0, row_start, row_deg);
+      row_ptr, static_cast<const int32_t*>(seeds), n, M, cnt, big_deg, nullptr, 0, 0, row_start, row_deg, rr, target_batch, target_seg);
   WG_HIP_CHECK(hipGetLastError());
 }
 
@@ -1820,11 +1836,13 @@
 void uniform_sample_enqueue(const int64_t* row_ptr, const void* col, bool col64, const void* seeds, bool seeds64,
                             dev_count n, int M, rng_plan random_seed, const int* offsets, void* dst, int* src_lid,
                             int64_t* edge_gid, hipStream_t stream, const int64_t* row_start,
-                            const int* row_deg, const sample_locality* loc)
-{
+                            const int* row_deg, const sample_locality* loc, const void* row_rng)
+{
+  random_seed.tab = pcg_stream_table_current();
 #define WG_U(ST, CT)                                                                                               \
   uniform_launch<ST, CT>(row_ptr, static_cast<const CT*>(col), static_cast<const ST*>(seeds), n, M, random_seed, \
-                         offsets, static_cast<CT*>(dst), src_lid, edge_gid, stream, row_start, row_deg, loc)
+                         offsets, static_cast<CT*>(dst), src_lid, edge_gid, stream, row_start, row_deg, loc,      \
+                         static_cast<const int2*>(row_rng))
   if (seeds64 && col64) WG_U(int64_t, int64_t);
   else if (seeds64) WG_U(int64_t, int32_t);
   else if (col64) WG_U(int32_t, int64_t);
diff --git a/cugraph-gnn_amd/csrc/wg_sample_replace.hip b/cugraph-gnn_amd/csrc/wg_sample_replace.hip
--- a/cugraph-gnn_amd/csrc/wg_sample_replace.hip
+++ b/cugraph-gnn_amd/csrc/wg_sample_replace.hip
@@ -18,7 +18,7 @@
 template <typename SeedT, typename ColT>
 __global__ void __launch_bounds__(256)
 replace_sample_kernel(const int64_t* __restrict__ row_ptr, const ColT* __restrict__ col, const SeedT* __restrict__ seeds, int n,
-                      int M, uint64_t random_seed, const int* __restrict__ offsets, ColT* __restrict__ dst,
+                      int M, uint64_t random_seed, pcg_stream_table tab, const int* __restrict__ offsets, ColT* __restrict__ dst,
                       int* __restrict__ src_lid, int64_t* __restrict__ edge_gid)
 {
   const int64_t p = (int64_t)blockIdx.x * blockDim.x + threadIdx.x;
@@ -26,7 +26,7 @@
   const int i = (int)(p / M), t = (int)(p - (int64_t)i * M);
   int32_t r;
   if (p < (1ll << 31)) {
-    Pcg32 g(random_seed, (uint32_t)p, Pcg32::table_tag{});
+    Pcg32 g(random_seed, (uint32_t)p, Pcg32::table_tag{}, tab);
     r = g.next_i31();
   } else {
     Pcg32 g(random_seed, (uint64_t)p);
@@ -63,7 +63,7 @@
   auto* gid = gid_ctx ? static_cast<int64_t*>(output_alloc(env, gid_ctx, total, WHOLEMEMORY_DT_INT64)) : nullptr;
   if (n == 0 || total == 0) return;
   replace_sample_kernel<SeedT, ColT><<<ceil_div((int64_t)n * M, 256), 256, 0, stream>>>(row_ptr, col, seeds, n, M, random_seed,
-                                                                                       offsets, dst, lid, gid);
+                                                                                       pcg_stream_table_current(), offsets, dst, lid, gid);
   WG_HIP_CHECK(hipGetLastError());
   WG_HIP_CHECK(hipStreamSynchronize(stream));
 }
diff --git a/cugraph-gnn_amd/csrc/wg_unique.hip b/cugraph-gnn_amd/csrc/wg_unique.hip
--- a/cugraph-gnn_amd/csrc/wg_unique.hip
+++ b/cugraph-gnn_amd/csrc/wg_unique.hip
@@ -1,3 +1,5 @@
+#include <atomic>
+
 #include "wg_common.hpp"
 #include "wgamd_ext.h"
 
@@ -6,11 +8,13 @@
 
 template <typename IdT>
 __global__ void __launch_bounds__(256) unique_mark_kernel(const IdT* __restrict__ ids, int64_t n, int64_t bound, uint8_t* __restrict__ flags,
-                                                          int* __restrict__ bad, const int* __restrict__ n_live)
+                                                          int* __restrict__ bad, const int* __restrict__ n_live, int stage, int stages)
 {
   if (n_live) n = min(n, (int64_t)*n_live);
+  const int64_t lo = n * stage / stages;
+  n                = n * (stage + 1) / stages;
   const int64_t T = (int64_t)gridDim.x * blockDim.x;
-  for (int64_t i = (int64_t)blockIdx.x * blockDim.x + threadIdx.x; i < n; i += 4 * T) {
+  for (int64_t i = lo + (int64_t)blockIdx.x * blockDim.x + threadIdx.x; i < n; i += 4 * T) {
     int64_t id[4];
     uint8_t f[4];
 #pragma unroll
@@ -88,6 +92,20 @@
       if (i + k * T < n) inverse[i + k * T] = (int)r[k].y + __popc(r[k].x & ((1u << (id[k] & 31)) - 1u));
   }
 }
+
+constexpr int kMarkStages        = 1;
+constexpr int64_t kMarkStagedMin = 4096;
+inline bool mark_stages_ok(int v) { return v == 1 || v == 2 || v == 4 || v == 8; }
+std::atomic<int>& mark_stages_setting()
+{
+  static std::atomic<int> stages{[] {
+    const char* e = getenv("WGAMD_UNIQUE_MARK_STAGES");
+    const int v   = e ? atoi(e) : kMarkStages;
+    return mark_stages_ok(v) ? v : kMarkStages;
+  }()};
+  return stages;
+}
+int mark_stages(int64_t n) { return n < kMarkStagedMin ? 1 : mark_stages_setting().load(std::memory_order_relaxed); }
 
 struct unique_plan {
   size_t flags, bits, cnt, tmp, bad, total;
@@ -117,6 +135,11 @@
 }
 
 extern "C" {
+
+void wgamd_set_unique_mark_stages(int stages)
+{
+  wgamd::mark_stages_setting().store(wgamd::mark_stages_ok(stages) ? stages : wgamd::kMarkStages, std::memory_order_relaxed);
+}
 
 size_t wgamd_unique_bounded_workspace_bytes(int64_t id_bound)
 {
@@ -155,9 +178,14 @@
     WG_HIP_CHECK(hipMemsetAsync(flags, 0, (size_t)p.n_words * 32, st));
     WG_HIP_CHECK(hipMemsetAsync(bad, 0, sizeof(int), st));
     if (n > 0) {
-      const int grid = (int)std::min<int64_t>(ceil_div(n, 256), 256 * 32);
-      if (id_dtype == WHOLEMEMORY_DT_INT) unique_mark_kernel<int32_t><<<grid, 256, 0, st>>>(static_cast<const int32_t*>(ids), n, id_bound, flags, bad, n_live_dev);
-      else unique_mark_kernel<int64_t><<<grid, 256, 0, st>>>(static_cast<const int64_t*>(ids), n, id_bound, flags, bad, n_live_dev);
+      const int stages = mark_stages(n);
+      const int grid   = (int)std::min<int64_t>(ceil_div(ceil_div(n, stages), 256), stages > 1 ? 256 * 8 : 256 * 32);
+      for (int s = 0; s < stages; s++) {
+        if (id_dtype == WHOLEMEMORY_DT_INT)
+          unique_mark_kernel<int32_t><<<grid, 256, 0, st>>>(static_cast<const int32_t*>(ids), n, id_bound, flags, bad, n_live_dev, s, stages);
+        else
+          unique_mark_kernel<int64_t><<<grid, 256, 0, st>>>(static_cast<const int64_t*>(ids), n, id_bound, flags, bad, n_live_dev, s, stages);
+      }
       WG_HIP_CHECK(hipGetLastError());
     }
     unique_pack_kernel<<<(int)ceil_div(p.cnt_padded, 256), 256, 0, st>>>(flags, p.n_words, rank, cnt, p.cnt_padded);
diff --git a/cugraph-gnn_amd/wholegraph_amd/_lib.py b/cugraph-gnn_amd/wholegraph_amd/_lib.py
--- a/cugraph-gnn_amd/wholegraph_amd/_lib.py
+++ b/cugraph-gnn_amd/wholegraph_amd/_lib.py
@@ -356,6 +356,10 @@
                                      c_size_t, c_void_p]),
     "wgamd_unique_bounded_live": (c_int, [c_void_p, c_int, c_int64, c_void_p, c_int64, c_void_p, c_void_p, c_void_p, c_void_p,
                                           c_void_p, c_size_t, c_void_p]),
+    "wgamd_set_unique_mark_stages": (None, [c_int]),
+    "wgamd_pcg_stream_table_prepare": (c_int, [c_void_p]),
+    "wgamd_pcg_stream_table_limit": (None, [ctypes.c_uint]),
+    "wgamd_pcg_stream_table_entry": (None, [c_ulonglong, c_void_p, c_void_p]),
     "wgamd_sample_hop_batched_nosync_ex": (c_int, [c_void_p, c_void_p, c_int, c_void_p, c_void_p, c_void_p, c_int,
                                                    c_int64, c_int, c_void_p, c_void_p, c_void_p, c_void_p, c_void_p,
                                                    c_int64, c_void_p, c_void_p, c_void_p, c_void_p, c_void_p, c_size_t,
diff --git a/cugraph-gnn_amd/wholegraph_amd/fused.py b/cugraph-gnn_amd/wholegraph_amd/fused.py
--- a/cugraph-gnn_amd/wholegraph_amd/fused.py
+++ b/cugraph-gnn_amd/wholegraph_amd/fused.py
@@ -135,6 +135,13 @@
         for i in range(n_fields):
             merged[i][dest] = live[h][i]
     return merged, offs
+
+
+def prepare_pcg_stream_table(dev) -> None:
+    if torch.cuda.is_current_stream_capturing():
+        return
+    with torch.cuda.device(dev):
+        L.check(L.lib().wgamd_pcg_stream_table_prepare(get_stream()), "wgamd_pcg_stream_table_prepare")
 
 
 class NoSyncWalk:
@@ -169,6 +176,7 @@
         self.ws_off = (-self.workspace.data_ptr()) % 256
         self.ws_bytes = ws
         self.dev = dev
+        prepare_pcg_stream_table(dev)
         self.seed_seg = (torch.arange(self.G + 1, dtype=torch.int32, device=dev) * self.B).contiguous()
         self.seed_batch = torch.arange(self.G, dtype=torch.int32, device=dev).repeat_interleave(self.B).contiguous()
 
@@ -225,6 +233,7 @@
 
     def __init__(self, walk: NoSyncWalk):
         self.walk = walk
+        prepare_pcg_stream_table(walk.dev)
         self._graph = self._res = None
         hops = len(walk.fanouts)
         self._seeds = torch.zeros(walk.G * walk.B, dtype=walk.id_dtype, device=walk.dev)
@@ -411,6 +420,7 @@
             n, f = n + f * m, f * m
         assert n < (1 << 30), "call group too large: lower n_batches"
         lib = L.lib()
+        prepare_pcg_stream_table(csr_row_ptr.device)
         if self.weight is None:
             ws = max(lib.wgamd_sample_hop_workspace_bytes(max(nc, fc), ec, self.wm_dtype)
                      for nc, fc, ec in zip(self.node_caps, self.frontier_caps, self.edge_caps))
@@ -502,6 +512,7 @@
         self.wm_dtype = torch_dtype_to_wm(torch.int64)
         self._ws = None
         dev = self.dev
+        prepare_pcg_stream_table(dev)
         self.seed_seg = (torch.arange(self.G + 1, dtype=torch.int32, device=dev) * self.B).contiguous()
         self.seed_batch = torch.arange(self.G, dtype=torch.int32, device=dev).repeat_interleave(self.B).contiguous()
         self.zeros_g = torch.zeros(self.G, dtype=torch.int32, device=dev)
diff --git a/include/wgamd_ext.h b/include/wgamd_ext.h
--- a/include/wgamd_ext.h
+++ b/include/wgamd_ext.h
@@ -382,6 +382,12 @@
                                                    int64_t id_bound, int64_t* distinct, int* inverse, int* n_distinct_dev,
                                                    int* out_of_bound_dev, void* workspace, size_t workspace_bytes, void* stream);
 
+wholememory_error_code_t wgamd_pcg_stream_table_prepare(void* stream);
+void wgamd_pcg_stream_table_limit(unsigned int entries);
+void wgamd_pcg_stream_table_entry(unsigned long long J, unsigned long long* a, unsigned long long* s);
+
+void wgamd_set_unique_mark_stages(int stages);
+
 size_t wgamd_softmax_xent_state_bytes(int64_t n_rows);
 wholememory_error_code_t wgamd_softmax_xent_forward_f32(const float* logits, int64_t ld, int64_t n_rows, int n_classes,
                                                         const int64_t* target, const float* row_weight, float* lse, void* state,
```
